# srihari-humbarwadi/retinanet-tensorflow2.x

Measured on AMD Instinct MI355X. Metric: images/sec train, ResNet50-640 RetinaNet data-parallel step (encode + fwd + loss + bwd + clip + all-reduce + SGD/EMA); inference images/s under `infer`, higher is better.
Workload: dtype bf16; 1 GPU; ResNet50-640x640 bf16 training, 32 images/GPU (BASELINE configs[2] shard: global batch 32), resnet_initial frozen, single GPU; global_batch=32, parallelism=dp1, rccl_ranks=1, comm=torch, syncbn_messages=0

## Files before the change

### include/rnet_hip.h

```cpp
#ifndef RNET_HIP_H_
#define RNET_HIP_H_

#include <stddef.h>
#include <stdint.h>

#ifdef __cplusplus
extern "C" {
#endif
#if defined(__GNUC__)
#pragma GCC visibility push(default)
#endif

typedef enum {
  RN_OK = 0,
  RN_EINVAL = -1,
  RN_ENOMEM = -2,
  RN_EHIP = -3,
  RN_ECOMM = -4,
  RN_EUNSUPPORTED = -5
} rn_status;

enum { RN_DT_F32 = 0, RN_DT_BF16 = 1 };
enum { RN_ACT_NONE = 0, RN_ACT_RELU = 1, RN_ACT_RELU6 = 2, RN_ACT_SWISH = 3 };

// ... 16 lines not shown
size_t rn_loss_workspace_bytes(int B, int64_t A, int K);
int rn_retinanet_loss_fwd_bwd(const float* const* class_logits, const float* const* box_preds,
                              float* const* d_class_logits, float* const* d_box_preds,
                              const int64_t* level_offsets, int num_levels, int B, int K,
                              const float* class_targets, const float* box_targets, const float* normalizer,
                              float alpha, float gamma, float label_smoothing, float delta,
                              float box_loss_weight, float class_loss_weight, float grad_scale, float* losses,
                              void* workspace, size_t workspace_bytes, void* stream);
int rn_retinanet_loss_fwd_bwd_bf16(const float* const* class_logits, const float* const* box_preds,
                                   void* const* d_class_bf16, void* const* d_box_bf16, int class_pix_stride,
                                   int box_pix_stride, int anchors_per_location, const int64_t* level_offsets,
                                   int num_levels, int B, int K, const float* class_targets,
                                   const float* box_targets, const float* normalizer, float alpha, float gamma,
                                   float label_smoothing, float delta, float box_loss_weight,
                                   float class_loss_weight, float grad_scale, float* losses, void* workspace,
                                   size_t workspace_bytes, void* stream);

int rn_decode_boxes(const float* const* box_preds, const int64_t* level_offsets, int num_levels, int B,
                    const float* anchors, const float* box_variance, float input_h, float input_w,
                    float* boxes, void* stream);

int rn_sigmoid_scores(const float* const* class_logits, const int64_t* level_offsets, int num_levels, int B,
                      int K, float* scores, void* stream);

size_t rn_topk_workspace_bytes(int B, int64_t A, int K);
int rn_topk_per_class(const float* scores, int B, int64_t A, int K, int top_k, float* topk_scores,
                      int32_t* topk_indices, void* workspace, size_t workspace_bytes, void* stream);

size_t rn_detect_workspace_bytes(int B, int64_t A, int K, int max_det);
int rn_detect_per_class(const float* const* class_logits, const int64_t* level_offsets, int num_levels, int B,
                        int K, const float* boxes, int pre_nms_top_k, float iou_threshold,
                        float score_threshold, float soft_nms_sigma, int max_det, float* det_boxes,
                        float* det_scores, int32_t* det_classes, int32_t* valid, void* workspace,
                        size_t workspace_bytes, void* stream);

size_t rn_nms_workspace_bytes(int B, int n, int K, int max_det);
int rn_nms_per_class(const float* cand_scores, const float* cand_boxes, int B, int n, int K,
                     float iou_threshold, float score_threshold, float soft_nms_sigma, int max_det,
                     float* det_boxes, float* det_scores, int32_t* det_classes,
                     int32_t* det_index ,
                     int32_t* valid, void* workspace, size_t workspace_bytes, void* stream);

int rn_rowmax_argmax(const float* scores, int64_t rows, int K, float* max_out, int32_t* argmax_out, void* stream);

typedef struct {
  int32_t conv_tile;
  int32_t conv_no_halo;
  int32_t conv_big_min_tiles;
  int32_t max_workgroups;
  int32_t reserved_cus;
  int32_t wgrad_kernel;
  int32_t wgrad_target_blocks;
  int32_t ablate;
  int32_t splitk_target_blocks;
} rn_launch_opts;

typedef struct rn_handle rn_handle;
int rn_create(int device_id, rn_handle** out);
int rn_destroy(rn_handle* h);
int rn_handle_device(const rn_handle* h);
int rn_handle_num_cus(const rn_handle* h);
int rn_handle_set_launch_opts(rn_handle* h, const rn_launch_opts* opts);
int rn_handle_get_launch_opts(const rn_handle* h, rn_launch_opts* opts);
int rn_handle_comm_init(rn_handle* h, int slot, const void* unique_id , int rank, int world);
void* rn_handle_comm(const rn_handle* h, int slot);
int rn_handle_comm_destroy(rn_handle* h, int slot);

#define RN_CONV_MAX_SEGMENTS 10

typedef struct {
  const void* x;
  const void* w;
  void* y;
  const float* scale;
  const float* shift;
  const void* residual;
  int32_t N, H, W, Cin, pix_stride, Ho, Wo, Cout;
  float* bn_partial;
  const float* bias;
  int32_t w_terms;
  int32_t w_pair;
  const void* bn_bwd_y;
  const float* bn_bwd_fwd;
} rn_conv_segment;

typedef struct {
  int32_t R, S, stride_h, stride_w, pad_top, pad_left;
  int32_t act;
  int32_t out_dtype;
  int32_t num_segments;
  rn_conv_segment seg[RN_CONV_MAX_SEGMENTS];
  rn_launch_opts opts;
  void* splitk_ws;
  int64_t splitk_ws_bytes;
} rn_conv_problem;

int rn_conv2d_nhwc_fwd(const rn_conv_problem* problem , void* stream);
size_t rn_conv_splitk_workspace_bytes(const rn_conv_problem* problem );
size_t rn_conv_splitk_workspace_max_bytes(void);

int rn_conv_cout_pad(int Cout);
int rn_conv_tile_rows(const rn_conv_problem* problem);
int rn_conv_bn_row_blocks(const rn_conv_problem* problem, int segment);
int rn_conv_kernel_id(const rn_conv_problem* problem);
int rn_conv_cin_pad(int Cin);
int rn_pack_conv_weight(const float* w_hwio, int R, int S, int Cin, int Cout, int Cin_pad, void* w_packed,
                        void* stream);
int rn_pack_conv_weight_split(const float* w, int layout_ohwi, int R, int S, int Cin, int Cout, int Cin_pad, int terms,
                              void* w_packed, void* stream);
int rn_conv_pair_rows(int Cout);
int rn_pack_conv_weight_pair(const float* w, int layout_ohwi, int R, int S, int Cin, int Cout, int Cin_pad,
                             void* w_packed, void* stream);
int rn_pack_conv_weight_ohwi(const float* w_ohwi, int R, int S, int Cin, int Cout, int Cin_pad, void* w_packed,
                             void* stream);
int rn_pack_stem_weight(const float* w_hwio, int Cout, void* w_packed, void* stream);
int rn_stem_padded_width(int W);
int rn_pack_stem_input(const float* images, int N, int H, int W, void* packed, void* stream);
int rn_pack_stem_weight_rs(const float* w_hwio, int R, int S, int Cout, void* w_packed, void* stream);
int rn_pack_image_nhwc4(const float* images, int N, int H, int W, int pad_top, int pad_left, int Hp, int Wp,
                        void* packed, void* stream);

typedef struct {
  const void* x;
  const void* dy;
  int32_t N, H, W, Cin, Ho, Wo, Cout;
  int32_t dy_pix_stride;
  int32_t x_pix_stride;
} rn_wgrad_segment;

typedef struct {
  int32_t R, S, stride_h, stride_w, pad_top, pad_left;
  int32_t num_segments;
  rn_wgrad_segment seg[RN_CONV_MAX_SEGMENTS];
  rn_launch_opts opts;
} rn_wgrad_problem;

size_t rn_wgrad_workspace_bytes(const rn_wgrad_problem* problem );
int rn_wgrad_kernel_id(const rn_wgrad_problem* problem );
int rn_conv2d_nhwc_wgrad(const rn_wgrad_problem* problem , float* dw, float beta, void* workspace,
                         size_t workspace_bytes, void* stream);
size_t rn_wgrad_group_workspace_bytes(const rn_wgrad_problem* const* problems , int n);
int rn_wgrad_group_fused(const rn_wgrad_problem* const* problems , int n);
int rn_conv2d_nhwc_wgrad_group(const rn_wgrad_problem* const* problems , int n, float* const* dws ,
                               float beta, void* workspace, size_t workspace_bytes, void* stream);

int rn_pack_conv_weight_dgrad(const float* w_ohwi, int R, int S, int Cin, int Cout, int Cout_pad, void* w_packed,
                              void* stream);
#define RN_DGRAD_PACK_MAX 64
typedef struct {
  const float* w_ohwi;
  void* w_packed;
  int32_t R, S, Cin, Cout, Cout_pad;
  int32_t pad_;
} rn_dgrad_pack;
int rn_pack_conv_weight_dgrad_batch(const rn_dgrad_pack* items , int n, void* stream);
int rn_cast_pad_f32_to_bf16(const float* x, void* y, int64_t P, int C, int Cpad, void* stream);
int rn_reduce_rows_f32(const float* src, int rows, int64_t row_stride, int n, float add, float* dst, void* stream);
int rn_upsample_zero2x(const void* x, void* y, int N, int H, int W, int C, int Ho, int Wo, void* stream);
int rn_scatter_add2x(const void* x, void* y, int N, int H, int W, int C, int Ho, int Wo, int accumulate, void* stream);
int rn_depth_to_space2x(const void* x, void* y, int N, int H, int W, int C, int accumulate, void* stream);
int rn_cast_f32_to_bf16(const float* x, void* y, int64_t n, void* stream);
int rn_act_bwd(const void* dz, const void* z, void* dy, int64_t n, int act, void* stream);

typedef struct {
  const void* y;
  void* z;
  const void* residual;
  const void* dz;
  void* dy;
  void* dres;
  float* sums;
  float* fwd;
  float* bsums;
  const float* gamma;
  const float* beta;
  float* moving_mean;
  float* moving_var;
  float* dgamma;
  float* dbeta;
  int64_t P;
  int32_t C;
  int32_t dres_accumulate;
  const float* sample_scale;
  int64_t rows_per_sample;
  int32_t ext_chunks;
  int32_t ext_chunks_bwd;
  void* act_mask;
  float* dy_colsum_partial;
} rn_bn_segment;

typedef struct {
  int32_t num_segments;
  int32_t act;
  int32_t bessel;
  float eps;
  float momentum;
  float count_scale;
  rn_bn_segment seg[RN_CONV_MAX_SEGMENTS];
} rn_bn_problem;

size_t rn_bn_workspace_bytes(const rn_bn_problem* problem );
int rn_bn_workspace_init(const rn_bn_problem* problem, void* workspace, size_t workspace_bytes, void* stream);
size_t rn_bn_partial_offset_bytes(const rn_bn_problem* problem, int segment);
size_t rn_bn_bwd_partial_offset_bytes(const rn_bn_problem* problem, int segment);
int rn_bn_stats(const rn_bn_problem* problem, void* workspace, size_t workspace_bytes, void* stream);
int rn_bn_stats_finalize(const rn_bn_problem* problem, void* workspace, size_t workspace_bytes, void* stream);
int rn_bn_finalize(const rn_bn_problem* problem, void* stream);
int rn_bn_apply(const rn_bn_problem* problem, void* stream);
int rn_bn_bwd_reduce(const rn_bn_problem* problem, void* workspace, size_t workspace_bytes, void* stream);
int rn_bn_bwd_apply(const rn_bn_problem* problem, void* stream);
int rn_bn_bwd_colsum_chunks(const rn_bn_problem* problem, int segment);

int rn_maxpool2d_nhwc_bwd(const void* x, const void* dy, void* dx, int N, int H, int W, int C, int k, int stride,
                          int pad_top, int pad_left, int Ho, int Wo, int accumulate, void* stream);
int rn_fpn_topdown_bwd_level(const void* dout, const void* din_finer, const void* out, void* din, int N, int H,
                             int W, int C, int act, void* stream);
size_t rn_balance_features_bwd_scratch_bytes(int num_levels, int mid, int N, int H0, int W0, int C);
int rn_balance_features_bwd(void* const* dout, void* const* in, void* const* din, const void* avg,
                            void* davg_scratch, size_t scratch_bytes, int num_levels, int mid, int N, int H0, int W0,
                            int C, void* stream);

int rn_optim_chunk(void);
size_t rn_optim_workspace_bytes(int num_blocks, int num_segments);
int rn_optim_clip(float* grads, const float* params, const void* segs_dev, int num_segments,
                  const int32_t* block_seg_dev, int num_blocks, float wd_coeff, float wd_alpha, float grad_unscale,
                  float clipnorm, float* metrics, void* workspace, size_t workspace_bytes, void* stream);
int rn_optim_clip_prepare(float* grads, const float* params, const void* segs_dev, const int32_t* block_seg_dev,
                          int num_blocks, int block_begin, int block_count, float wd_coeff, float grad_unscale,
                          float* local_copy ,
                          void* workspace, size_t workspace_bytes, void* stream);
int rn_optim_clip_factors(const void* segs_dev, int num_segments, int num_blocks, float clipnorm, float wd_alpha,
                          float* metrics, float* flags, void* workspace, size_t workspace_bytes, void* stream);
int rn_optim_clip_apply(float* grads, float* correction, const void* segs_dev, const int32_t* block_seg_dev,
                        int num_blocks, void* workspace, size_t workspace_bytes, void* stream);
int rn_optim_sgd_step(float* params, const float* grads, float* momentum_buf, float* ema, void* params_bf16,
                      const void* segs_dev, const int32_t* block_seg_dev, int num_blocks, float lr, float momentum,
                      float ema_decay, int nesterov, const float* skip_flag, void* stream);

int rn_comm_available(void);
int rn_comm_unique_id_bytes(void);
int rn_comm_unique_id(void* out );
int rn_comm_init(const void* unique_id , int rank, int world, void** comm_out);
int rn_comm_destroy(void* comm);
int rn_allreduce_bucket(void* comm, void* ptr , int64_t count, int dtype, void* stream);
int rn_allreduce_small(void* comm, float* ptr , int count, void* stream);

long long rn_probe_mfma_flops(int iters);
int rn_probe_spin(int microseconds, void* stream);
int rn_probe_mfma(const float* table, float* out, int iters, unsigned long long* clocks, void* stream);

int rn_maxpool2d_nhwc(const void* x, void* y, int N, int H, int W, int C, int k, int stride, int pad_top,
                      int pad_left, int Ho, int Wo, void* stream);

int rn_stem_conv_bn_relu_pool(const void* x, const void* w_packed, const float* scale, const float* shift, void* y,
                              int N, int Hp, int Wp, int Hs, int Ws, int R, int Cout, int act, int pool_k,
                              int pool_stride, int pool_pad_top, int pool_pad_left, int Po, int Qo, void* stream);

typedef struct {
  const void* x;
  void* y;
  const void* w_packed;
  const float* affine;
  int32_t N, H, W, Cx;
  rn_launch_opts opts;
} rn_bottleneck64_problem;
int rn_bottleneck64_supported(int N, int H, int W, int Cx);
size_t rn_bottleneck64_packed_bytes(int Cx);
int rn_bottleneck64_pack(const float* wa_hwio, const float* wb_hwio, const float* wo_hwio, const float* wsc_hwio, int Cx,
                         void* packed, void* stream);
int rn_bottleneck64_fwd(const rn_bottleneck64_problem* problem, void* stream);

int rn_fpn_topdown(void* const* p_in , void* const* p_out, int num_levels,
                   int N, int H0, int W0, int C, int act, void* stream);

int rn_balance_features(void* const* p_in, void* const* p_out, int num_levels, int mid, int N, int H0, int W0,
                        int C, void* scratch, void* stream);

typedef struct {
  const void* x;
  const void* w;
  void* y;
  const float* scale;
  const float* shift;
  const void* residual;
  int32_t N, H, W, C, Ho, Wo;
} rn_dw_segment;

typedef struct {
  int32_t k, stride, pad_top, pad_left, act, num_segments;
  rn_dw_segment seg[RN_CONV_MAX_SEGMENTS];
} rn_dw_problem;

int rn_depthwise_conv2d_nhwc_fwd(const rn_dw_problem* problem , void* stream);
int rn_pack_depthwise_weight(const float* w_kkc1, int k, int C, void* w_packed, void* stream);
int rn_pack_depthwise_weight_flip(const float* w_kkc, int k, int C, void* w_packed, void* stream);
// ... 50 lines not shown
```

### retinanet-tensorflow2.x_amd/csrc/rn_conv.hip

```cpp
#include <map>
#include <mutex>
#include <tuple>

#include <algorithm>
#include "rn_conv_dev.h"

template <int BM, int BN, int BK, bool OUT_F32, int ABL = 0, int WM = 2, int WN = 2, int STAGES = 2, bool SPLIT = false>
__global__ void __launch_bounds__(64 * WM * WN, 2) conv_fwd_kernel(const ConvArgs args) {
  constexpr int NWAVES = WM * WN;
  constexpr int NTHREADS = 64 * NWAVES;
  constexpr int SLOTS = BK / 8;
  constexpr int RPI = 64 / SLOTS;
  constexpr int A_INSTR = BM / RPI / NWAVES;
  constexpr int B_INSTR = BN / RPI / NWAVES;
  constexpr int WTM = BM / WM, WTN = BN / WN;
  constexpr int TM = WTM / 32, TN = WTN / 32;
  constexpr int KSUB = BK / 16;
  constexpr int A_BYTES = BM * BK * 2, B_BYTES = BN * BK * 2;
  constexpr int STAGE_BYTES = A_BYTES + B_BYTES;
  static_assert(A_INSTR >= 1 && B_INSTR >= 1, "tile too small for the wave count");

  extern __shared__ __attribute__((aligned(16))) char smem[];

  int tile, part = 0;
// ... 741 lines not shown
  const int kid = conv_pick(p);
  return kid == 3 ? 512 : (kid ? 256 : 128);
}

extern "C" int rn_conv2d_nhwc_fwd(const rn_conv_problem* p, void* stream) {
  RN_CHECK_ARG(p != nullptr, "rn_conv2d_nhwc_fwd: null problem");
  RN_CHECK_ARG(p->num_segments >= 1 && p->num_segments <= RN_CONV_MAX_SEGMENTS,
               "rn_conv2d_nhwc_fwd: num_segments=%d", p->num_segments);
  RN_CHECK_ARG(p->R >= 1 && p->S >= 1 && p->R * p->S <= 32, "rn_conv2d_nhwc_fwd: R*S=%d > 32", p->R * p->S);
  RN_CHECK_ARG(p->stride_h >= 1 && p->stride_w >= 1, "rn_conv2d_nhwc_fwd: bad stride");
  RN_CHECK_ARG(p->out_dtype == RN_DT_BF16 || p->out_dtype == RN_DT_F32, "rn_conv2d_nhwc_fwd: bad out_dtype");
  if (const int orc = rn_validate_launch_opts(p->opts, "rn_conv2d_nhwc_fwd")) return orc;
  ConvArgs a;
  a.R = p->R; a.S = p->S; a.sh = p->stride_h; a.sw = p->stride_w; a.pt = p->pad_top; a.pl = p->pad_left;
  a.act = p->act; a.nseg = p->num_segments; a.pad_ = 0;
  const int cout_pad0 = rn_conv_cout_pad(seg_cols(p->seg[0]));
  int BN = cout_pad0 <= 64 ? 64 : 128;
  const int BK = conv128_bk(p);
  const int kid = conv_pick(p);
  const bool big = kid == 1 || kid == 2;
  const bool halo512 = kid == 3;
  const int BM = big ? 256 : (halo512 ? 512 : 128);
  if (!big && !halo512) {
    int bk_;
    conv128_shape(p, &BN, &bk_);
  }
  const int BNT = big ? 256 : BN;
  const int bal_rows = kid == 1 ? conv_big_balanced_rows(p) : 0;
  int tiles = 0;
  int order[RN_CONV_MAX_SEGMENTS];
  for (int i = 0; i < p->num_segments; ++i) order[i] = i;
  bool deal = false;
  if (kid == 1 && p->num_segments > 1) {
    long long dmin = 1ll << 60, dmax = 0;
    bool one_col = true;
    for (int i = 0; i < p->num_segments; ++i) {
      const long long depth = (long long)p->R * p->S * rn_conv_cin_pad(p->seg[i].Cin) * (p->seg[i].w_terms > 1 ? p->seg[i].w_terms : 1);
      dmin = depth < dmin ? depth : dmin;
      dmax = depth > dmax ? depth : dmax;
      one_col = one_col && rn_conv_cout_pad(seg_cols(p->seg[i])) <= 256;
    }
    deal = one_col && dmax >= 2 * dmin;
    if (deal)
      std::stable_sort(order, order + p->num_segments, [&](int x, int y) {
        return rn_conv_cin_pad(p->seg[x].Cin) * (p->seg[x].w_terms > 1 ? p->seg[x].w_terms : 1) >
               rn_conv_cin_pad(p->seg[y].Cin) * (p->seg[y].w_terms > 1 ? p->seg[y].w_terms : 1);
      });
  }
  for (int ii = 0; ii < p->num_segments; ++ii) {
    const int i = order[ii];
    const rn_conv_segment& s = p->seg[i];
    RN_CHECK_ARG(s.x && s.w && s.y, "rn_conv2d_nhwc_fwd: segment %d has a null tensor", i);
    RN_CHECK_ARG(s.N > 0 && s.H > 0 && s.W > 0 && s.Ho > 0 && s.Wo > 0 && s.Cout > 0 && s.Cin > 0,
                 "rn_conv2d_nhwc_fwd: segment %d bad shape", i);
    RN_CHECK_ARG(s.Cin % 8 == 0 && rn_conv_cin_pad(s.Cin) % BK == 0,
                 "rn_conv2d_nhwc_fwd: segment %d Cin=%d must be a multiple of 8 (K step %d)", i, s.Cin, BK);
    RN_CHECK_ARG(s.pix_stride % 4 == 0 && s.pix_stride > 0,
                 "rn_conv2d_nhwc_fwd: segment %d pix_stride=%d must be a positive multiple of 4", i, s.pix_stride);
    RN_CHECK_ARG(s.Cout % 4 == 0, "rn_conv2d_nhwc_fwd: segment %d Cout=%d not a multiple of 4", i, s.Cout);
    const int cp = rn_conv_cout_pad(seg_cols(s));
    RN_CHECK_ARG((cp <= 64) == (cout_pad0 <= 64), "rn_conv2d_nhwc_fwd: segments mix Cout tile widths");
    RN_CHECK_ARG(!s.w_pair || ((big || halo512) && p->out_dtype == RN_DT_F32 && s.w_terms <= 1 && !s.scale && !s.shift &&
                               !s.residual && !s.bn_partial),
                 "rn_conv2d_nhwc_fwd: segment %d: w_pair needs an f32 launch without scale / shift / residual that the 256- / "
                 "512-row kernels take (rn_conv_kernel_id() != 0)", i);
    RN_CHECK_ARG(((uintptr_t)s.x | (uintptr_t)s.w | (uintptr_t)s.y | (uintptr_t)s.residual) % 16 == 0,
                 "rn_conv2d_nhwc_fwd: segment %d tensors must be 16-byte aligned", i);
    const long long M = (long long)s.N * s.Ho * s.Wo;
    RN_CHECK_ARG(M < (1ll << 31) && (long long)s.N * s.H * s.W * s.pix_stride * 2 < (1ll << 31),
                 "rn_conv2d_nhwc_fwd: segment %d input exceeds the 2 GiB buffer-addressing limit", i);
    ConvSegDev& d = a.seg[ii];
    d.x = (const uint16_t*)s.x; d.w = (const uint16_t*)s.w; d.y = s.y;
    d.scale = s.scale; d.shift = s.shift; d.residual = (const uint16_t*)s.residual;
    d.bn_partial = s.bn_partial;
    d.bn_y = (const uint16_t*)s.bn_bwd_y;
    d.bn_fwd = s.bn_bwd_fwd;
    if (s.bn_bwd_y) {
      RN_CHECK_ARG(s.bn_partial && s.bn_bwd_fwd && p->out_dtype == RN_DT_BF16 && !s.scale && !s.shift && !s.bias &&
                       !s.residual && p->act == RN_ACT_NONE && s.Cout % 8 == 0 && (uintptr_t)s.bn_bwd_y % 16 == 0,
                   "rn_conv2d_nhwc_fwd: segment %d: bn_bwd_y needs bn_partial + bn_bwd_fwd on a plain bf16 launch", i);
    }
    RN_CHECK_ARG((s.bn_bwd_y != nullptr) == (p->seg[0].bn_bwd_y != nullptr),
                 "rn_conv2d_nhwc_fwd: bn_bwd_y must be set on all segments or none");
    d.bias = s.bias;
    d.N = s.N; d.H = s.H; d.W = s.W; d.Cin = s.Cin; d.pix_stride = s.pix_stride;
    d.Ho = s.Ho; d.Wo = s.Wo; d.Cout = seg_cols(s);
    d.pair_cout = s.w_pair ? s.Cout : 0;
    d.rows = kid == 1 ? bal_rows : 0;
    d.M = (int)M;
    d.tile_begin = tiles;
    d.n_tiles = (int)rn_cdiv(cp, BNT);
    const int terms = s.w_terms > 1 ? s.w_terms : 1;
    RN_CHECK_ARG(terms <= 3, "rn_conv2d_nhwc_fwd: segment %d w_terms=%d (1..3)", i, s.w_terms);
    d.cwrap = rn_conv_cin_pad(s.Cin);
    d.CinP = terms * d.cwrap;
    d.halo_pitch = s.W + 1;
    if (rn_conv_halo_patch_pixels(s.N, s.H, s.W, rn_conv_halo_pitch(s.W), halo512 ? 512 : 256) <= rn_conv_halo_capacity(halo512 ? 512 : 256))
      d.halo_pitch = rn_conv_halo_pitch(s.W);
    tiles += (int)rn_cdiv(M, d.rows ? d.rows : BM) * d.n_tiles;
  }
  a.total_tiles = tiles;
  a.split_f = a.vtotal = tiles; a.split_s = 1; a.pad2_ = 0; a.ws = nullptr;
  RN_CHECK_ARG(p->splitk_ws == nullptr || ((uintptr_t)p->splitk_ws % 16 == 0 && p->splitk_ws_bytes >= 0),
               "rn_conv2d_nhwc_fwd: splitk_ws must be 16-byte aligned");
  hipStream_t st = (hipStream_t)stream;
  const bool f32 = p->out_dtype == RN_DT_F32;
  if (p->opts.ablate && BM == 128 && BN == 128 && BK == 64 && !f32) {
    switch (p->opts.ablate) {
      case 1: return launch_ablate<1>(a, st);
      case 2: return launch_ablate<2>(a, st);
      case 3: return launch_ablate<3>(a, st);
      case 4: return launch_ablate<4>(a, st);
      case 5: return launch_ablate<5>(a, st);
      case 6: return launch_ablate<6>(a, st);
      case 7: return launch_ablate<7>(a, st);
      case 8: return launch_ablate<8>(a, st);
      case 16: return launch_ablate<16>(a, st);
      case 32: return launch_ablate<32>(a, st);
      case 48: return launch_ablate<48>(a, st);
      default: break;
    }
  }
  if (halo512) return rn_launch_conv_halo(a, f32, p->opts, st, 4);
  if (kid == 2) {
    rn_splitk_plan(a, conv_splitk_min_chunks(p), p->splitk_ws, p->splitk_ws_bytes, p->opts);
    return rn_launch_conv_halo(a, f32, p->opts, st);
  }
  if (big) {
    a.pad_ = 1;
    for (int i = 0; i < a.nseg; ++i)
      if (a.seg[i].M >= (1 << 22)) a.pad_ = 0;
    if (deal) a.pad_ |= 2;
    return rn_launch_conv_big(a, f32, p->opts, st);
  }
  a.pad_ = 1;
  for (int i = 0; i < a.nseg; ++i)
    if (a.seg[i].M >= (1 << 22)) a.pad_ = 0;
  const int S128 = conv128_split_parts(p, tiles, BN, BK);
  if (S128 >= 2) {
    a.split_s = S128; a.vtotal = tiles * S128; a.ws = (float*)p->splitk_ws;
    return launch_conv128<true>(a, BN, BK, f32, st);
  }
  return launch_conv128<false>(a, BN, BK, f32, st);
}

__global__ void pack_weight_kernel(const float* __restrict__ w, int R, int S, int Cin, int Cout, int Cin_pad,
                                   int Cout_pad, uint16_t* __restrict__ out) {
  const long long total = (long long)Cout_pad * R * S * Cin_pad;
  for (long long i = blockIdx.x * (long long)blockDim.x + threadIdx.x; i < total;
       i += (long long)gridDim.x * blockDim.x) {
    const int c = (int)(i % Cin_pad);
    long long t = i / Cin_pad;
    const int s = (int)(t % S);
    t /= S;
    const int r = (int)(t % R);
    const int o = (int)(t / R);
    float v = 0.0f;
    if (o < Cout && c < Cin) v = w[(((long long)r * S + s) * Cin + c) * Cout + o];
    out[i] = rn_f32_to_bf16(v);
  }
}

extern "C" int rn_pack_conv_weight(const float* w_hwio, int R, int S, int Cin, int Cout, int Cin_pad,
                                   void* w_packed, void* stream) {
  RN_CHECK_ARG(w_hwio && w_packed && R > 0 && S > 0 && Cin > 0 && Cout > 0 && Cin_pad >= Cin,
               "rn_pack_conv_weight: bad argument");
  const int Cout_pad = rn_conv_cout_pad(Cout);
  const long long total = (long long)Cout_pad * R * S * Cin_pad;
  int blocks = (int)(rn_cdiv(total, 256) < 4096 ? rn_cdiv(total, 256) : 4096);
  hipLaunchKernelGGL(pack_weight_kernel, dim3(blocks), dim3(256), 0, (hipStream_t)stream, w_hwio, R, S, Cin,
                     Cout, Cin_pad, Cout_pad, (uint16_t*)w_packed);
  RN_CHECK_LAUNCH();
  return RN_OK;
}

__global__ void pack_weight_ohwi_kernel(const float* __restrict__ w, int RS, int Cin, int Cout, int Cin_pad,
                                        int Cout_pad, uint16_t* __restrict__ out) {
  const long long total = (long long)Cout_pad * RS * Cin_pad;
  for (long long i = blockIdx.x * (long long)blockDim.x + threadIdx.x; i < total;
       i += (long long)gridDim.x * blockDim.x) {
    const int c = (int)(i % Cin_pad);
    const long long t = i / Cin_pad;
    float v = 0.0f;
    if (t < (long long)Cout * RS && c < Cin) v = w[t * Cin + c];
    out[i] = rn_f32_to_bf16(v);
  }
}

extern "C" int rn_pack_conv_weight_ohwi(const float* w_ohwi, int R, int S, int Cin, int Cout, int Cin_pad,
                                        void* w_packed, void* stream) {
  RN_CHECK_ARG(w_ohwi && w_packed && R > 0 && S > 0 && Cin > 0 && Cout > 0 && Cin_pad >= Cin,
               "rn_pack_conv_weight_ohwi: bad argument");
  const int Cout_pad = rn_conv_cout_pad(Cout);
  const long long total = (long long)Cout_pad * R * S * Cin_pad;
  int blocks = (int)(rn_cdiv(total, 256) < 4096 ? rn_cdiv(total, 256) : 4096);
  hipLaunchKernelGGL(pack_weight_ohwi_kernel, dim3(blocks), dim3(256), 0, (hipStream_t)stream, w_ohwi, R * S, Cin,
                     Cout, Cin_pad, Cout_pad, (uint16_t*)w_packed);
  RN_CHECK_LAUNCH();
  return RN_OK;
}

__global__ void pack_weight_split_kernel(const float* __restrict__ w, int ohwi, int RS, int Cin, int Cout, int Cin_pad,
                                         int Cout_pad, int terms, uint16_t* __restrict__ out) {
  const long long total = (long long)Cout_pad * RS * Cin_pad;
  for (long long i = blockIdx.x * (long long)blockDim.x + threadIdx.x; i < total;
       i += (long long)gridDim.x * blockDim.x) {
    const int c = (int)(i % Cin_pad);
    const long long t = i / Cin_pad;
    const int tap = (int)(t % RS), o = (int)(t / RS);
    float v = 0.0f;
    if (o < Cout && c < Cin) v = ohwi ? w[t * Cin + c] : w[((long long)tap * Cin + c) * Cout + o];
    uint16_t* dst = out + (t * terms) * Cin_pad + c;
    for (int k = 0; k < terms; ++k) {
      const uint16_t b = rn_f32_to_bf16(v);
      dst[(long long)k * Cin_pad] = b;
// ... 112 lines not shown
```

### retinanet-tensorflow2.x_amd/csrc/rn_conv_big.hip

```cpp
#include "rn_conv_big_epi.h"

namespace {

constexpr int BM = 256, BN = 256, BK = 32, NW = 8, STAGES = 4;
constexpr int A_BYTES = BM * BK * 2, STAGE_BYTES = (BM + BN) * BK * 2;
constexpr int RING_BYTES = STAGES * STAGE_BYTES, PATCH_BYTES = 4096;
constexpr int LDS_BYTES = RING_BYTES + NW * PATCH_BYTES;

template <bool OUT_F32, bool HAS_RES, bool BN_BWD = false>
__global__ void __launch_bounds__(512) conv_big_kernel(const ConvArgs args) {
  extern __shared__ __attribute__((aligned(16))) char smem[];
  const int total = args.total_tiles;
  const int G = gridDim.x;
  const int tid = threadIdx.x;
  const int lane = tid & 63;
  const int wave = __builtin_amdgcn_readfirstlane(tid >> 6);
  const int wave_m = wave >> 2, wave_n = wave & 3;
  const int R = args.R, S = args.S, RS = R * S;

  int i_v = blockIdx.x;
  int i_tap = 0, i_c0 = 0;
  int i_r = 0, i_s = 0;
  int g_iss = 0;
  int i_W = 0, i_PS = 0, i_Cin = 0, i_cw = 0;
  __amdgpu_buffer_rsrc_t rs_x, rs_w;
  unsigned a_off[2], a_mask[2], b_off[2];
  const int d_row = lane >> 2, d_pos = lane & 3;

#define BIG_SETUP_ISSUE()                                                                             \
  do {                                                                                                \
    const int tile__ = (args.pad_ & 2) ? i_v : tile_of(i_v, total);      \
    int si__ = 0;                                                                                     \
    _Pragma("unroll 1") for (int i = 1; i < args.nseg; ++i)                                           \
      if (tile__ >= args.seg[i].tile_begin) si__ = i;                                                 \
    const ConvSegDev& sg__ = args.seg[si__];                                                          \
    const int lt__ = tile__ - sg__.tile_begin;                                                        \
    const int mt__ = rn_fdiv(lt__, sg__.n_tiles, rn_rcp((float)sg__.n_tiles));   \
    const int rows_t__ = sg__.rows ? sg__.rows : BM;      \
    const int m0__ = mt__ * rows_t__, n0__ = (lt__ - mt__ * sg__.n_tiles) * BN;                       \
    const int mend__ = m0__ + rows_t__ < sg__.M ? m0__ + rows_t__ : sg__.M;                           \
    i_W = sg__.W; i_PS = sg__.pix_stride; i_Cin = sg__.CinP; i_cw = sg__.cwrap;                       \
    const int H__ = sg__.H, Ktot__ = RS * i_Cin;                                                      \
    const int rows__ = sg__.Cout <= 64 ? 64 : ((sg__.Cout + 127) / 128) * 128;  \
    rs_x = __builtin_amdgcn_make_buffer_rsrc((void*)sg__.x, 0,                                        \
                                             (int)((long long)sg__.N * H__ * i_W * i_PS * 2), 0x00020000); \
    rs_w = __builtin_amdgcn_make_buffer_rsrc((void*)sg__.w, 0, (int)((long long)rows__ * Ktot__ * 2), \
                                             0x00020000);                                             \
    const float rWo__ = rn_rcp((float)sg__.Wo), rHo__ = rn_rcp((float)sg__.Ho);                 \
    _Pragma("unroll") for (int j = 0; j < 2; ++j) {                                                   \
      const int row = (j * NW + wave) * 16 + d_row;                                                   \
      const int chunk = d_pos ^ lds_swz<BK>(row);                                                     \
      const int m = m0__ + row;                                                                       \
      const int mm = m < mend__ ? m : 0;                                                              \
      int ox, oy, n;                                                                                  \
      if (args.pad_ & 1) {    \
        const int t2 = rn_fdiv(mm, sg__.Wo, rWo__);                                                   \
        ox = mm - t2 * sg__.Wo;                                                                       \
        n = rn_fdiv(t2, sg__.Ho, rHo__);                                                              \
        oy = t2 - n * sg__.Ho;                                                                        \
      } else {                                                                                        \
        ox = mm % sg__.Wo;                                                                            \
        const int t2 = mm / sg__.Wo;                                                                  \
        oy = t2 % sg__.Ho;                                                                            \
        n = t2 / sg__.Ho;                                                                             \
      }                                                                                               \
      const int iy0 = oy * args.sh - args.pt, ix0 = ox * args.sw - args.pl;                           \
      a_off[j] = (unsigned)(((((long long)n * H__ + iy0) * i_W + ix0) * i_PS + chunk * 8) * 2);       \
      unsigned mask = 0;                                                                              \
      if (m < mend__) {                                                                               \
        for (int r = 0; r < R; ++r)                                                                   \
          for (int s = 0; s < S; ++s) {                                                               \
            const bool ok = (unsigned)(iy0 + r) < (unsigned)H__ && (unsigned)(ix0 + s) < (unsigned)i_W; \
            mask |= (ok ? 1u : 0u) << (r * S + s);                                                    \
          }                                                                                           \
      }                                                                                               \
      a_mask[j] = mask;                                                                               \
      const int nrow = n0__ + row;                                                                    \
      b_off[j] = nrow < rows__ ? (unsigned)(((long long)nrow * Ktot__ + chunk * 8) * 2) : RN_OOB;     \
    }                                                                                                 \
  } while (0)

#define BIG_ISSUE_STEP()                                                                              \
  do {                                                                                                \
    const int cw__ = i_c0 < i_cw ? i_c0 : (i_c0 < 2 * i_cw ? i_c0 - i_cw : i_c0 - 2 * i_cw);          \
    const unsigned tap_off__ = (unsigned)((((long long)i_r * i_W + i_s) * i_PS + cw__) * 2);          \
    const unsigned koff__ = (unsigned)(((long long)i_tap * i_Cin + i_c0) * 2);                        \
    char* st__ = smem + (g_iss & 3) * STAGE_BYTES;                                                    \
    _Pragma("unroll") for (int j = 0; j < 2; ++j) {                                                   \
      const unsigned v__ = ((a_mask[j] >> i_tap) & 1u) ? a_off[j] + tap_off__ : RN_OOB;               \
      dma16(rs_x, st__ + (j * NW + wave) * 1024, v__);                                                \
    }                                                                                                 \
    _Pragma("unroll") for (int j = 0; j < 2; ++j)                                                     \
// ... 10 lines not shown
      if (__builtin_expect(i_tap == RS, 0)) {                                                         \
        i_tap = i_r = i_s = 0;                                                                        \
        i_v += G;                                                                                     \
        if (i_v < total) BIG_SETUP_ISSUE();                                                           \
      }                                                                                               \
    }                                                                                                 \
  } while (0)

  int off_p0, off_w0;
  {
    const int fr = lane & 31, fh = lane >> 5;
    const int sw = (fr >> 2) & 3;
    off_p0 = (wave_m * 128 + fr) * 64 + ((0 + fh) ^ sw) * 16;
    off_w0 = A_BYTES + (wave_n * 64 + fr) * 64 + ((0 + fh) ^ sw) * 16;
  }

  f32x16_t acc[4][2];
#pragma unroll
  for (int i = 0; i < 4; ++i)
#pragma unroll
    for (int j = 0; j < 2; ++j)
#pragma unroll
      for (int r = 0; r < 16; ++r) acc[i][j][r] = 0.0f;

  bf16x8_t px0[4], wt0[2], px1[4], wt1[2];
#define BIG_READ(stage_)                                                                              \
  do {                                                                                                \
    const char* b__ = smem + (stage_) * STAGE_BYTES;                                                  \
    _Pragma("unroll") for (int j = 0; j < 2; ++j) wt0[j] = *(const bf16x8_t*)(b__ + off_w0 + j * 2048); \
    _Pragma("unroll") for (int i = 0; i < 4; ++i) px0[i] = *(const bf16x8_t*)(b__ + off_p0 + i * 2048); \
    _Pragma("unroll") for (int j = 0; j < 2; ++j) wt1[j] = *(const bf16x8_t*)(b__ + (off_w0 ^ 32) + j * 2048); \
    _Pragma("unroll") for (int i = 0; i < 4; ++i) px1[i] = *(const bf16x8_t*)(b__ + (off_p0 ^ 32) + i * 2048); \
  } while (0)
#define BIG_LOADSEG(stage_)                                                                           \
  do {                                                                                                \
    BIG_READ(stage_);                                                                                 \
    if (i_v < total) {                                                                                \
      BIG_ISSUE_STEP();                                                                               \
      asm volatile("s_waitcnt vmcnt(8)" ::: "memory");                                                \
    } else {                                                                                          \
      asm volatile("s_waitcnt vmcnt(0)" ::: "memory");                                                \
    }                                                                                                 \
    asm volatile("s_waitcnt lgkmcnt(0)" ::: "memory");                                                \
  } while (0)
#define BIG_COMPUTESEG()                                                                              \
  do {                                                                                                \
    __builtin_amdgcn_sched_barrier(0);                                                                \
    _Pragma("unroll") for (int i = 0; i < 4; ++i)                                                     \
      _Pragma("unroll") for (int j = 0; j < 2; ++j)                                                   \
        acc[i][j] = RN_MFMA_32x32x16(wt0[j], px0[i], acc[i][j], 0, 0, 0);      \
    _Pragma("unroll") for (int i = 0; i < 4; ++i)                                                     \
      _Pragma("unroll") for (int j = 0; j < 2; ++j)                                                   \
        acc[i][j] = RN_MFMA_32x32x16(wt1[j], px1[i], acc[i][j], 0, 0, 0);      \
    __builtin_amdgcn_sched_barrier(0);                                                                \
  } while (0)
#define BIG_BARRIER()                       \
  do {                                      \
    __builtin_amdgcn_s_barrier();           \
    asm volatile("" ::: "memory");          \
  } while (0)

  int c_v = blockIdx.x;
  int c_k = 0;
  int c_ksteps, c_m0, c_n0, c_si, c_mend, c_chunk0;
#define BIG_SETUP_COMPUTE()                                                                           \
  do {                                                                                                \
    const int tile__ = (args.pad_ & 2) ? c_v : tile_of(c_v, total);                                   \
    c_si = 0;                                                                                         \
    _Pragma("unroll 1") for (int i = 1; i < args.nseg; ++i)                                           \
      if (tile__ >= args.seg[i].tile_begin) c_si = i;                                                 \
    const ConvSegDev& sg__ = args.seg[c_si];                                                          \
    const int lt__ = tile__ - sg__.tile_begin;                                                        \
    const int mt__ = rn_fdiv(lt__, sg__.n_tiles, rn_rcp((float)sg__.n_tiles));   \
    const int rows_t__ = sg__.rows ? sg__.rows : BM;                                                  \
    c_m0 = mt__ * rows_t__;                                                                           \
    c_mend = c_m0 + rows_t__ < sg__.M ? c_m0 + rows_t__ : sg__.M;                                     \
    c_chunk0 = mt__ * 2;                                                                              \
    c_n0 = (lt__ - mt__ * sg__.n_tiles) * BN;                                                         \
    c_ksteps = RS * (sg__.CinP / BK);                                                                 \
    c_k = 0;                                                                                          \
  } while (0)

  auto epilogue = [&]() __attribute__((always_inline)) {
    big_epilogue<OUT_F32, HAS_RES, BN_BWD>(acc, args, c_si, c_m0, c_n0, wave, smem + RING_BYTES + wave * PATCH_BYTES,
                                           BigEpiSrc(), c_mend, c_chunk0);
  };

  BIG_SETUP_ISSUE();
  BIG_SETUP_COMPUTE();
  big_acc_init<OUT_F32, HAS_RES>(acc, args, c_si, c_n0, wave);
#pragma unroll 1
  for (int t = 0; t < 3 && i_v < total; ++t) BIG_ISSUE_STEP();
  if (g_iss >= 3) asm volatile("s_waitcnt vmcnt(4)" ::: "memory");
  else asm volatile("s_waitcnt vmcnt(0)" ::: "memory");
  BIG_BARRIER();
  BIG_LOADSEG(0);
  if (wave_m == 1) BIG_BARRIER();

#define BIG_TILE_END()                                       \
  if (__builtin_expect(c_k == c_ksteps, 0)) {               \
    epilogue();                                             \
    if (c_v + G >= total) break;                            \
    c_v += G;                                               \
    BIG_SETUP_COMPUTE();                                    \
    big_acc_init<OUT_F32, HAS_RES>(acc, args, c_si, c_n0, wave); \
  }
  int g = 0;
#pragma unroll 1
  while (true) {
    BIG_COMPUTESEG();
    ++c_k;
    if (wave_m == 0) BIG_BARRIER();
    BIG_TILE_END();
    if (wave_m == 1) BIG_BARRIER();
    ++g;
    BIG_LOADSEG(g & 3);
    BIG_BARRIER();
  }
#undef BIG_TILE_END
#undef BIG_SETUP_COMPUTE
#undef BIG_BARRIER
#undef BIG_COMPUTESEG
#undef BIG_LOADSEG
#undef BIG_READ
#undef BIG_ISSUE_STEP
#undef BIG_SETUP_ISSUE
}

}

int rn_launch_conv_big(const ConvArgs& a, bool out_f32, const rn_launch_opts& opts, hipStream_t st) {
  static unsigned long long attr_set = 0;
  if (RN_ATTRS_NEEDED(attr_set)) {
    RN_CHECK_HIP(hipFuncSetAttribute((const void*)conv_big_kernel<false, false>,
                                     hipFuncAttributeMaxDynamicSharedMemorySize, LDS_BYTES));
    RN_CHECK_HIP(hipFuncSetAttribute((const void*)conv_big_kernel<false, true>,
                                     hipFuncAttributeMaxDynamicSharedMemorySize, LDS_BYTES));
    RN_CHECK_HIP(hipFuncSetAttribute((const void*)conv_big_kernel<true, false>,
                                     hipFuncAttributeMaxDynamicSharedMemorySize, LDS_BYTES));
    RN_CHECK_HIP(hipFuncSetAttribute((const void*)conv_big_kernel<true, true>,
                                     hipFuncAttributeMaxDynamicSharedMemorySize, LDS_BYTES));
    RN_CHECK_HIP(hipFuncSetAttribute((const void*)conv_big_kernel<false, false, true>,
                                     hipFuncAttributeMaxDynamicSharedMemorySize, LDS_BYTES));
    RN_ATTRS_DONE(attr_set);
  }
  const int grid = rn_persistent_grid(a.total_tiles, rn_num_cus(), opts);
  bool has_res = false;
  for (int i = 0; i < a.nseg; ++i) has_res = has_res || a.seg[i].residual != nullptr;
  const dim3 g3(grid), b3(512);
  if (a.seg[0].bn_y) {
    hipLaunchKernelGGL((conv_big_kernel<false, false, true>), g3, b3, LDS_BYTES, st, a);
  } else if (out_f32) {
    if (has_res) hipLaunchKernelGGL((conv_big_kernel<true, true>), g3, b3, LDS_BYTES, st, a);
    else hipLaunchKernelGGL((conv_big_kernel<true, false>), g3, b3, LDS_BYTES, st, a);
  } else {
    if (has_res) hipLaunchKernelGGL((conv_big_kernel<false, true>), g3, b3, LDS_BYTES, st, a);
    else hipLaunchKernelGGL((conv_big_kernel<false, false>), g3, b3, LDS_BYTES, st, a);
  }
  RN_CHECK_LAUNCH();
  return RN_OK;
}
```

### retinanet-tensorflow2.x_amd/csrc/rn_conv_big_epi.h

```cpp
#ifndef RN_CONV_BIG_EPI_H_
#define RN_CONV_BIG_EPI_H_
#include <type_traits>

#include "rn_conv_dev.h"

#ifdef HALO_PROF
__device__ unsigned long long g_halo_clk[48];
#define EPI_STAMP(k_) if (blockIdx.x == 0 && threadIdx.x == 0) g_halo_clk[k_] = clock64();
#else
#define EPI_STAMP(k_)
#endif

#ifdef HALO_ABLATE
#define EPI_ABLATE HALO_ABLATE
#else
#define EPI_ABLATE 0
#endif

typedef rn_h16 bf16x2_t __attribute__((ext_vector_type(2)));
typedef float f32x2_t __attribute__((ext_vector_type(2)));

__device__ __forceinline__ uint32_t pack2(float lo, float hi) {
  f32x2_t v = {lo, hi};
  bf16x2_t b = __builtin_convertvector(v, bf16x2_t);
// ... 28 lines not shown
    typedef const float __attribute__((address_space(4))) cfloat;
    const cfloat* b = (const cfloat*)(unsigned long long)sg.bias;
    const int cw0 = (c_n0 + (wave % (8 / WM)) * 64) >> 1;
    const int C = sg.pair_cout;
    const int lane = (int)__builtin_amdgcn_mbcnt_hi(~0u, __builtin_amdgcn_mbcnt_lo(~0u, 0u));
    const bool hi = lane >= 32;
#pragma unroll
    for (int g = 0; g < 4; ++g)
#pragma unroll
      for (int q = 0; q < 4; ++q) {
        const int ca = cw0 + g * 8 + q, cb = ca + 4;
        const float lo_v = b[ca < C ? ca : 0], hi_v = b[cb < C ? cb : 0];
        const float v = hi ? hi_v : lo_v;
#pragma unroll
        for (int i = 0; i < 4; ++i) { acc[i][0][g * 4 + q] = v; acc[i][1][g * 4 + q] = 0.0f; }
      }
    return;
  }
  if (with_bias && big_bias_in_acc<OUT_F32, HAS_RES>(args, sg)) {
    typedef const float __attribute__((address_space(4))) cfloat;
    const cfloat* b = (const cfloat*)(unsigned long long)sg.bias;
    const int nw0 = c_n0 + (wave % (8 / WM)) * 64;
    const int Cout = sg.Cout;
    const int lane = (int)__builtin_amdgcn_mbcnt_hi(~0u, __builtin_amdgcn_mbcnt_lo(~0u, 0u));
    const bool hi = lane >= 32;
#pragma unroll
    for (int j = 0; j < 2; ++j)
#pragma unroll
      for (int g = 0; g < 4; ++g) {
        int c0 = nw0 + j * 32 + g * 8;
        c0 = c0 + 8 <= Cout ? c0 : Cout - 8;
        c0 = c0 < 0 ? 0 : c0;
#pragma unroll
        for (int q = 0; q < 4; ++q) {
          const float lo_v = b[c0 + q], hi_v = b[c0 + 4 + q];
          const float v = hi ? hi_v : lo_v;
#pragma unroll
          for (int i = 0; i < 4; ++i) acc[i][j][g * 4 + q] = v;
        }
      }
  } else {
#pragma unroll
    for (int i = 0; i < 4; ++i)
#pragma unroll
      for (int j = 0; j < 2; ++j)
#pragma unroll
        for (int r = 0; r < 16; ++r) acc[i][j][r] = 0.0f;
  }
}

struct BigEpiSrc {
  const char* slots;
  int nparts, voff;
};
template <int NJ>
__device__ __forceinline__ void big_epi_rebuild(f32x16_t* t, const BigEpiSrc& src, int i, int j0) {
  typedef unsigned u32x4_t_ __attribute__((ext_vector_type(4)));
  const __amdgpu_buffer_rsrc_t rs = __builtin_amdgcn_make_buffer_rsrc(
      (void*)src.slots, 0, src.nparts * RN_SPLITK_SLOT_BYTES, 0x00020000);
  u32x4_t_ v[4][NJ][4];
#pragma unroll
  for (int p = 0; p < 4; ++p)
#pragma unroll
    for (int j = 0; j < NJ; ++j)
#pragma unroll
      for (int q = 0; q < 4; ++q)
        v[p][j][q] = __builtin_amdgcn_raw_buffer_load_b128(rs, src.voff + p * RN_SPLITK_SLOT_BYTES,
                                                           ((i * 2 + j0 + j) * 4 + q) * 1024, 16);
#pragma unroll
  for (int j = 0; j < NJ; ++j)
#pragma unroll
    for (int q = 0; q < 4; ++q) {
      float a0 = __uint_as_float(v[0][j][q].x), a1 = __uint_as_float(v[0][j][q].y);
      float a2 = __uint_as_float(v[0][j][q].z), a3 = __uint_as_float(v[0][j][q].w);
#pragma unroll
      for (int p = 1; p < 4; ++p) {
        a0 += __uint_as_float(v[p][j][q].x); a1 += __uint_as_float(v[p][j][q].y);
        a2 += __uint_as_float(v[p][j][q].z); a3 += __uint_as_float(v[p][j][q].w);
      }
      t[j][q * 4] = a0; t[j][q * 4 + 1] = a1; t[j][q * 4 + 2] = a2; t[j][q * 4 + 3] = a3;
    }
}

template <bool OUT_F32, bool HAS_RES, bool BN_BWD = false, bool FROM_WS = false, int WM = 2>
__device__ __forceinline__ void big_epilogue(f32x16_t (&acc)[4][2], const ConvArgs& args, int c_si, int c_m0,
                                             int c_n0, int wave, char* patch, const BigEpiSrc src = BigEpiSrc(),
                                             int m_end = -1, int chunk0 = -1) {
  static_assert(!(BN_BWD && (OUT_F32 || HAS_RES)), "BN_BWD: plain bf16 launches only");
  constexpr bool LOADS = HAS_RES || BN_BWD;
  const int wave_m = wave / (8 / WM), wave_n = wave % (8 / WM);
  const ConvSegDev& sg = args.seg[c_si];
  const int Cout = sg.Cout, M = m_end >= 0 ? m_end : sg.M;
  const int nw0 = c_n0 + wave_n * 64;
  const int mw0 = c_m0 + wave_m * 128;
  const int elane = (int)__builtin_amdgcn_mbcnt_hi(~0u, __builtin_amdgcn_mbcnt_lo(~0u, 0u));
  const int fr = elane & 31, fh = elane >> 5;
  const int rrow = elane >> 3, ru = elane & 7;
  if (!OUT_F32) {
    const int nr = nw0 + ru * 8;
    const bool nok = nr < Cout;
    float sc[8], sf[8];
#pragma unroll
    for (int q = 0; q < 8; ++q) { sc[q] = 1.0f; sf[q] = 0.0f; }
    if (nok && sg.scale) {
      const float4 a = *(const float4*)(sg.scale + nr), b = *(const float4*)(sg.scale + nr + 4);
      sc[0] = a.x; sc[1] = a.y; sc[2] = a.z; sc[3] = a.w; sc[4] = b.x; sc[5] = b.y; sc[6] = b.z; sc[7] = b.w;
    }
    if (nok && sg.shift) {
      const float4 a = *(const float4*)(sg.shift + nr), b = *(const float4*)(sg.shift + nr + 4);
      sf[0] = a.x; sf[1] = a.y; sf[2] = a.z; sf[3] = a.w; sf[4] = b.x; sf[5] = b.y; sf[6] = b.z; sf[7] = b.w;
    }
    float mu[BN_BWD ? 8 : 1], is[BN_BWD ? 8 : 1];
    if (BN_BWD) {
#pragma unroll
      for (int q = 0; q < 8; ++q) { mu[q] = 0.0f; is[q] = 0.0f; }
    }
    if (BN_BWD && nok) {
      const float* f0 = sg.bn_fwd + nr;
      const float* f1 = sg.bn_fwd + Cout + nr;
      {
        const float4 a = *(const float4*)f0, b = *(const float4*)(f0 + 4), c = *(const float4*)f1, d = *(const float4*)(f1 + 4);
        mu[0] = a.x; mu[1] = a.y; mu[2] = a.z; mu[3] = a.w; mu[4] = b.x; mu[5] = b.y; mu[6] = b.z; mu[7] = b.w;
        is[0] = c.x; is[1] = c.y; is[2] = c.z; is[3] = c.w; is[4] = d.x; is[5] = d.y; is[6] = d.z; is[7] = d.w;
      }
      const float* f2 = sg.bn_fwd + 2 * Cout + nr;
      const float* f3 = sg.bn_fwd + 3 * Cout + nr;
      const float4 a = *(const float4*)f2, b = *(const float4*)(f2 + 4), c = *(const float4*)f3, d = *(const float4*)(f3 + 4);
      sc[0] = a.x; sc[1] = a.y; sc[2] = a.z; sc[3] = a.w; sc[4] = b.x; sc[5] = b.y; sc[6] = b.z; sc[7] = b.w;
      sf[0] = c.x; sf[1] = c.y; sf[2] = c.z; sf[3] = c.w; sf[4] = d.x; sf[5] = d.y; sf[6] = d.z; sf[7] = d.w;
    }
#pragma unroll
    for (int q = 0; q < 8; ++q) asm volatile("" : "+v"(sc[q]), "+v"(sf[q]));
    if (BN_BWD) {
#pragma unroll
      for (int q = 0; q < 8; ++q) asm volatile("" : "+v"(mu[q]), "+v"(is[q]));
    }
    EPI_STAMP(12);
    const bool has_res = HAS_RES && sg.residual != nullptr;
    const uint16_t* const side = BN_BWD ? sg.bn_y : sg.residual;
    const bool has_side = BN_BWD ? true : has_res;
    const bool stats = sg.bn_partial != nullptr;
    float st0[8], st1[8];
#pragma unroll
    for (int q = 0; q < 8; ++q) st0[q] = st1[q] = 0.0f;
    char* const ybase = (char*)sg.y + ((long long)(mw0 + rrow) * Cout + nr) * 2;
    const long long row_bytes = (long long)Cout * 2;
    const int act = args.act;
    const bool clamp_lo = act == RN_ACT_RELU || act == RN_ACT_RELU6, clamp_hi = act == RN_ACT_RELU6;
    const bool affine = !BN_BWD && (sg.scale != nullptr || sg.shift != nullptr);
    const bool plain = BN_BWD || (!affine && !has_res && act != RN_ACT_SWISH);
    const bool round2 = affine && has_res;
    uint4 rv[2][LOADS ? 4 : 1];
#define BIG_RES_PREFETCH(buf_, i_)                                                                    \
_Pragma("unroll") for (int pass = 0; pass < (LOADS ? 4 : 0); ++pass) {                              \
  const int m = mw0 + (i_) * 32 + pass * 8 + rrow;                                                  \
  rv[buf_][pass] = make_uint4(0u, 0u, 0u, 0u);                                                      \
  if (has_side && nok && m < M) rv[buf_][pass] = *(const uint4*)(side + (long long)m * Cout + nr);  \
}
    const uint32_t lo2 = clamp_lo ? 0u : 0x80008000u, hi2 = clamp_hi ? RN_SIX_X2 : 0x7fff7fffu;
    auto blocks = [&](auto plain_c, auto stats_c, auto round2_c, auto swish_c) __attribute__((always_inline)) {
      constexpr bool PLAIN = decltype(plain_c)::value;
      constexpr int STATS = decltype(stats_c)::value, ROUND2 = decltype(round2_c)::value, SWISH = decltype(swish_c)::value;
      BIG_RES_PREFETCH(0, 0);
#pragma unroll
      for (int i = 0; i < 4; ++i) {
        EPI_STAMP(13 + 2 * i);
        if (i + 1 < 4) BIG_RES_PREFETCH((i + 1) & 1, i + 1);
        if (FROM_WS) big_epi_rebuild<2>(&acc[i][0], src, i, 0);
#pragma unroll
        for (int j = 0; j < 2; ++j)
#pragma unroll
          for (int g = 0; g < 4; ++g) {
            const int nl = j * 32 + g * 8 + fh * 4;
            uint2 pk;
            pk.x = pack2(acc[i][j][g * 4 + 0], acc[i][j][g * 4 + 1]);
            pk.y = pack2(acc[i][j][g * 4 + 2], acc[i][j][g * 4 + 3]);
            *(uint2*)(patch + fr * 128 + (((nl >> 3) ^ (fr & 7)) << 4) + ((((nl >> 2) ^ (fr >> 3)) & 1) << 3)) = pk;
          }
        EPI_STAMP(14 + 2 * i);
        uint4 vb[4];
#pragma unroll
        for (int pass = 0; pass < 4; ++pass) {
          const int row = pass * 8 + rrow;
          const uint4 t = *(const uint4*)(patch + row * 128 + ((ru ^ (row & 7)) << 4));
          vb[pass] = (pass & 1) ? make_uint4(t.z, t.w, t.x, t.y) : t;
        }
#pragma unroll
        for (int pass = 0; pass < 4; ++pass) {
          const int row = pass * 8 + rrow;
          const uint4 v = vb[pass];
          const int m = mw0 + i * 32 + row;
          if (m < M && nok) {
            uint4 ov;
            if (PLAIN) {
              ov.x = pk_min_i16(pk_max_i16(v.x, lo2), hi2); ov.y = pk_min_i16(pk_max_i16(v.y, lo2), hi2);
              ov.z = pk_min_i16(pk_max_i16(v.z, lo2), hi2); ov.w = pk_min_i16(pk_max_i16(v.w, lo2), hi2);
            } else {
              const uint4 r4 = HAS_RES ? rv[i & 1][LOADS ? pass : 0] : make_uint4(0u, 0u, 0u, 0u);
              float f[8] = {bf_lo(v.x), bf_hi(v.x), bf_lo(v.y), bf_hi(v.y), bf_lo(v.z), bf_hi(v.z), bf_lo(v.w), bf_hi(v.w)};
              const float rr[8] = {bf_lo(r4.x), bf_hi(r4.x), bf_lo(r4.y), bf_hi(r4.y),
                                   bf_lo(r4.z), bf_hi(r4.z), bf_lo(r4.w), bf_hi(r4.w)};
#pragma unroll
              for (int q = 0; q < 8; ++q) f[q] = f[q] * sc[q] + sf[q];
              if (ROUND2 == 1 || (ROUND2 == 2 && round2)) {
#pragma unroll
                for (int q = 0; q < 8; q += 2) {
                  const uint32_t pq = pack2(f[q], f[q + 1]);
                  f[q] = bf_lo(pq); f[q + 1] = bf_hi(pq);
                }
              }
#pragma unroll
              for (int q = 0; q < 8; ++q) f[q] += rr[q];
              if (SWISH == 1 || (SWISH == 2 && act == RN_ACT_SWISH)) {
#pragma unroll
                for (int q = 0; q < 8; ++q) f[q] = rn_swish(rn_rb(f[q]));
              }
              ov.x = pack2(f[0], f[1]); ov.y = pack2(f[2], f[3]); ov.z = pack2(f[4], f[5]); ov.w = pack2(f[6], f[7]);
              ov.x = pk_min_i16(pk_max_i16(ov.x, lo2), hi2); ov.y = pk_min_i16(pk_max_i16(ov.y, lo2), hi2);
              ov.z = pk_min_i16(pk_max_i16(ov.z, lo2), hi2); ov.w = pk_min_i16(pk_max_i16(ov.w, lo2), hi2);
            }
            if (!(EPI_ABLATE & 16) || ov.x == 0x12345678u) *(uint4*)(ybase + (long long)(i * 32 + pass * 8) * row_bytes) = ov;
            if (STATS == 1 || (STATS == 2 && stats)) {
              const float w[8] = {bf_lo(ov.x), bf_hi(ov.x), bf_lo(ov.y), bf_hi(ov.y),
                                  bf_lo(ov.z), bf_hi(ov.z), bf_lo(ov.w), bf_hi(ov.w)};
              if (BN_BWD) {
                const uint4 y4 = rv[i & 1][LOADS ? pass : 0];
                const float yy[8] = {bf_lo(y4.x), bf_hi(y4.x), bf_lo(y4.y), bf_hi(y4.y),
                                     bf_lo(y4.z), bf_hi(y4.z), bf_lo(y4.w), bf_hi(y4.w)};
#pragma unroll
                for (int q = 0; q < 8; ++q) {
                  const float g = (yy[q] * sc[q] + sf[q]) > 0.0f ? w[q] : 0.0f;
                  st0[q] += g;
                  st1[q] += g * ((yy[q] - mu[BN_BWD ? q : 0]) * is[BN_BWD ? q : 0]);
                }
              } else {
#pragma unroll
                for (int q = 0; q < 8; ++q) { st0[q] += w[q]; st1[q] += w[q] * w[q]; }
              }
            }
          }
        }
      }
    };
    typedef std::integral_constant<int, 0> off_t;
    typedef std::integral_constant<int, 1> on_t;
    typedef std::integral_constant<int, 2> runtime_t;
    if constexpr (BN_BWD) {
      blocks(std::true_type{}, on_t{}, off_t{}, off_t{});
    } else if (plain) {
      if (stats) blocks(std::true_type{}, on_t{}, off_t{}, off_t{});
      else blocks(std::true_type{}, off_t{}, off_t{}, off_t{});
    } else if (!stats && act != RN_ACT_SWISH) {
      if (round2) blocks(std::false_type{}, off_t{}, on_t{}, off_t{});
      else blocks(std::false_type{}, off_t{}, off_t{}, off_t{});
    } else {
      blocks(std::false_type{}, runtime_t{}, runtime_t{}, runtime_t{});
    }
    EPI_STAMP(21);
    if (stats) {
#pragma unroll
      for (int q = 0; q < 8; ++q) {
#pragma unroll
        for (int o = 8; o < 64; o <<= 1) {
          st0[q] += __shfl_xor(st0[q], o, 64);
          st1[q] += __shfl_xor(st1[q], o, 64);
        }
      }
      if (rrow == 0 && nok) {
        float* dst = sg.bn_partial + ((long long)(chunk0 >= 0 ? chunk0 : c_m0 / 128) + wave_m) * 2 * Cout + nr;
        *(float4*)(dst) = make_float4(st0[0], st0[1], st0[2], st0[3]);
        *(float4*)(dst + 4) = make_float4(st0[4], st0[5], st0[6], st0[7]);
        *(float4*)(dst + Cout) = make_float4(st1[0], st1[1], st1[2], st1[3]);
        *(float4*)(dst + Cout + 4) = make_float4(st1[4], st1[5], st1[6], st1[7]);
      }
    }
#undef BIG_RES_PREFETCH
  } else {
    const int pairC = sg.pair_cout;
    const int CoutY = pairC ? pairC : Cout;
    auto half = [&](auto j_c) __attribute__((always_inline)) {
      constexpr int j = decltype(j_c)::value;
      const int nr = (pairC ? (nw0 >> 1) : nw0 + j * 32) + ru * 4;
      const bool nok = nr < CoutY;
      float4 sc = make_float4(1.f, 1.f, 1.f, 1.f), sf = make_float4(0.f, 0.f, 0.f, 0.f);
      if (nok && sg.scale) sc = *(const float4*)(sg.scale + nr);
      if (nok && sg.shift) sf = *(const float4*)(sg.shift + nr);
      asm volatile("" : "+v"(sc.x), "+v"(sc.y), "+v"(sc.z), "+v"(sc.w), "+v"(sf.x), "+v"(sf.y), "+v"(sf.z), "+v"(sf.w));
#pragma unroll
      for (int i = 0; i < 4; ++i) {
        if (FROM_WS) big_epi_rebuild<1>(&acc[i][j], src, i, j);
        if (j == 0 && pairC) {
          if (FROM_WS) big_epi_rebuild<1>(&acc[i][1], src, i, 1);
#pragma unroll
          for (int r = 0; r < 16; ++r) acc[i][0][r] += acc[i][1][r];
        }
#pragma unroll
        for (int g = 0; g < 4; ++g) {
          float4 v;
          v.x = acc[i][j][g * 4 + 0]; v.y = acc[i][j][g * 4 + 1]; v.z = acc[i][j][g * 4 + 2]; v.w = acc[i][j][g * 4 + 3];
          *(float4*)(patch + fr * 128 + (((g * 2 + fh) ^ (fr & 7)) << 4)) = v;
        }
#pragma unroll
        for (int pass = 0; pass < 4; ++pass) {
          const int row = pass * 8 + rrow;
          float4 v = *(const float4*)(patch + row * 128 + ((ru ^ (row & 7)) << 4));
          const int m = mw0 + i * 32 + row;
          if (m < M && nok) {
            const long long o = (long long)m * CoutY + nr;
            v.x = v.x * sc.x + sf.x; v.y = v.y * sc.y + sf.y; v.z = v.z * sc.z + sf.z; v.w = v.w * sc.w + sf.w;
            if (sg.residual) {
              const uint2 r2 = *(const uint2*)(sg.residual + o);
              v.x += bf_lo(r2.x); v.y += bf_hi(r2.x); v.z += bf_lo(r2.y); v.w += bf_hi(r2.y);
            }
            {
              float f4[4] = {v.x, v.y, v.z, v.w};
              rn_apply_act_n<4>(f4, args.act);
              v = make_float4(f4[0], f4[1], f4[2], f4[3]);
            }
            *(float4*)((float*)sg.y + o) = v;
          }
        }
      }
    };
    half(std::integral_constant<int, 0>{});
    if (!pairC) half(std::integral_constant<int, 1>{});
  }
}
#endif
```

### retinanet-tensorflow2.x_amd/csrc/rn_core.hip

```cpp
#include "rn_common.h"
#include <string.h>
#include <new>

static thread_local char g_rn_err[512] = "";

void rn_set_error(const char* fmt, ...) {
  va_list ap;
  va_start(ap, fmt);
  vsnprintf(g_rn_err, sizeof(g_rn_err), fmt, ap);
  va_end(ap);
}

extern "C" const char* rn_last_error(void) { return g_rn_err; }

extern "C" int rn_abi_version(void) { return 8; }

extern "C" int rn_storage_dtype(void) {
#ifdef RN_F16
  return 1;
#else
  return 0;
#endif
}

extern "C" int rn_device_ok(void) {
  int n = 0;
  if (hipGetDeviceCount(&n) != hipSuccess || n <= 0) {
    (void)hipGetLastError();
    return 0;
  }
  hipDeviceProp_t p;
  if (hipGetDeviceProperties(&p, 0) != hipSuccess) return 0;
  return strncmp(p.gcnArchName, "gfx950", 6) == 0 ? 1 : 0;
}

struct rn_handle {
  int device;
  int num_cus;
  rn_launch_opts opts;
  void* comm[4];
};

static int rn_check_opts(const rn_launch_opts& o, const char* who) {
  RN_CHECK_ARG(o.conv_tile >= 0 && o.conv_tile <= 3, "%s: conv_tile=%d (0..3)", who, o.conv_tile);
  RN_CHECK_ARG(o.wgrad_kernel >= 0 && o.wgrad_kernel <= 3, "%s: wgrad_kernel=%d (0..3)", who, o.wgrad_kernel);
  RN_CHECK_ARG(o.reserved_cus >= 0 && o.reserved_cus <= 128, "%s: reserved_cus=%d out of range (0..128)", who,
               o.reserved_cus);
  RN_CHECK_ARG(o.max_workgroups >= 0 && o.conv_big_min_tiles >= 0 && o.wgrad_target_blocks >= 0 && o.splitk_target_blocks >= 0,
               "%s: negative max_workgroups / conv_big_min_tiles / wgrad_target_blocks / splitk_target_blocks", who);
  return RN_OK;
}
int rn_validate_launch_opts(const rn_launch_opts& o, const char* who) { return rn_check_opts(o, who); }

extern "C" int rn_create(int device_id, rn_handle** out) {
  RN_CHECK_ARG(out != nullptr, "rn_create: null out");
  *out = nullptr;
  int n = 0;
  RN_CHECK_HIP(hipGetDeviceCount(&n));
  RN_CHECK_ARG(device_id >= 0 && device_id < n, "rn_create: device %d of %d", device_id, n);
  hipDeviceProp_t p;
  RN_CHECK_HIP(hipGetDeviceProperties(&p, device_id));
  RN_CHECK_ARG(strncmp(p.gcnArchName, "gfx950", 6) == 0, "rn_create: device %d is %s, this library is gfx950 only",
               device_id, p.gcnArchName);
  rn_handle* h = new (std::nothrow) rn_handle();
  if (!h) {
    rn_set_error("rn_create: out of host memory");
    return RN_ENOMEM;
  }
  h->device = device_id;
  h->num_cus = p.multiProcessorCount;
  memset(&h->opts, 0, sizeof(h->opts));
  for (auto& c : h->comm) c = nullptr;
  *out = h;
  return RN_OK;
}

extern "C" int rn_destroy(rn_handle* h) {
  if (!h) return RN_OK;
  int rc = RN_OK;
  for (auto& c : h->comm)
    if (c) {
      const int r = rn_comm_destroy(c);
      if (r != RN_OK) rc = r;
      c = nullptr;
    }
  delete h;
  return rc;
}

extern "C" int rn_handle_device(const rn_handle* h) { return h ? h->device : RN_EINVAL; }
extern "C" int rn_handle_num_cus(const rn_handle* h) { return h ? h->num_cus : RN_EINVAL; }

extern "C" int rn_handle_set_launch_opts(rn_handle* h, const rn_launch_opts* opts) {
  RN_CHECK_ARG(h && opts, "rn_handle_set_launch_opts: null argument");
  const int rc = rn_check_opts(*opts, "rn_handle_set_launch_opts");
  if (rc != RN_OK) return rc;
  h->opts = *opts;
  return RN_OK;
// ... 51 lines not shown
```

### retinanet-tensorflow2.x_amd/csrc/rn_optim.hip

```cpp
#include "rn_common.h"

#define OPT_THREADS 256
#define OPT_CHUNK 8192

struct OptSeg { long long offset, size; int wd, block_begin, nblocks, pad_; long long bf16_offset; };

__global__ void __launch_bounds__(OPT_THREADS)
optim_sqnorm_kernel(float* __restrict__ g, const float* __restrict__ w, const OptSeg* __restrict__ segs,
                    const int* __restrict__ block_seg, int block0, float wdc, float unscale,
                    double* __restrict__ partial, double* __restrict__ partial_w, float* __restrict__ local_copy) {
  const int blk = block0 + blockIdx.x;
  const int si = block_seg[blk];
  const OptSeg s = segs[si];
  const long long b0 = (long long)(blk - s.block_begin) * OPT_CHUNK;
  long long b1 = b0 + OPT_CHUNK;
  if (b1 > s.size) b1 = s.size;
  float acc = 0.0f, accw = 0.0f;
  const bool touch = s.wd || unscale != 1.0f;
#define SQNORM_ELEM(gv_, wv_)                 \
  do {                                        \
    float v__ = (gv_) * unscale;              \
    if (s.wd) {                               \
      v__ += wdc * (wv_);                     \
      accw += (wv_) * (wv_);                  \
// ... 210 lines not shown
                                     float wd_alpha, float* metrics, float* flags, void* workspace,
                                     size_t workspace_bytes, void* stream) {
  RN_CHECK_ARG(segs_dev && metrics && num_segments > 0 && num_blocks > 0, "rn_optim_clip_factors: bad argument");
  if (!workspace || workspace_bytes < rn_optim_workspace_bytes(num_blocks, num_segments)) {
    rn_set_error("rn_optim_clip_factors: workspace too small");
    return RN_ENOMEM;
  }
  const OptWs w = opt_ws(workspace, num_blocks);
  hipLaunchKernelGGL(optim_factors_kernel, dim3(1), dim3(256), 0, (hipStream_t)stream, (const OptSeg*)segs_dev,
                     num_segments, w.partial, w.partial_w, clipnorm, wd_alpha, w.factor, metrics, flags);
  RN_CHECK_LAUNCH();
  return RN_OK;
}

extern "C" int rn_optim_clip_apply(float* grads, float* correction, const void* segs_dev,
                                   const int32_t* block_seg_dev, int num_blocks, void* workspace,
                                   size_t workspace_bytes, void* stream) {
  RN_CHECK_ARG(grads && segs_dev && block_seg_dev && num_blocks > 0 && workspace, "rn_optim_clip_apply: bad argument");
  const OptWs w = opt_ws(workspace, num_blocks);
  hipLaunchKernelGGL(optim_scale_kernel, dim3(num_blocks), dim3(OPT_THREADS), 0, (hipStream_t)stream, grads, correction,
                     (const OptSeg*)segs_dev, block_seg_dev, w.factor);
  RN_CHECK_LAUNCH();
  return RN_OK;
}

extern "C" int rn_optim_clip(float* grads, const float* params, const void* segs_dev, int num_segments,
                             const int32_t* block_seg_dev, int num_blocks, float wd_coeff, float wd_alpha,
                             float grad_unscale, float clipnorm, float* metrics , void* workspace,
                             size_t workspace_bytes, void* stream) {
  RN_CHECK_ARG(grads && params && segs_dev && block_seg_dev && metrics && num_segments > 0 && num_blocks > 0,
               "rn_optim_clip: bad argument");
  int rc = rn_optim_clip_prepare(grads, params, segs_dev, block_seg_dev, num_blocks, 0, num_blocks, wd_coeff,
                                 grad_unscale, nullptr, workspace, workspace_bytes, stream);
  if (rc) return rc;
  rc = rn_optim_clip_factors(segs_dev, num_segments, num_blocks, clipnorm, wd_alpha, metrics, nullptr, workspace,
                             workspace_bytes, stream);
  if (rc) return rc;
  return rn_optim_clip_apply(grads, nullptr, segs_dev, block_seg_dev, num_blocks, workspace, workspace_bytes, stream);
}

extern "C" int rn_optim_sgd_step(float* params, const float* grads, float* momentum_buf, float* ema,
                                 void* params_bf16, const void* segs_dev, const int32_t* block_seg_dev,
                                 int num_blocks, float lr, float momentum, float ema_decay, int nesterov,
                                 const float* skip_flag, void* stream) {
  RN_CHECK_ARG(params && grads && momentum_buf && segs_dev && block_seg_dev && num_blocks > 0,
               "rn_optim_sgd_step: bad argument");
  hipLaunchKernelGGL(optim_sgd_kernel, dim3(num_blocks), dim3(OPT_THREADS), 0, (hipStream_t)stream, params, grads,
                     momentum_buf, ema, (uint16_t*)params_bf16, (const OptSeg*)segs_dev, block_seg_dev, lr, momentum,
                     ema_decay, ema ? 1 : 0, nesterov, skip_flag);
  RN_CHECK_LAUNCH();
  return RN_OK;
}

__global__ void __launch_bounds__(256)
pack_dgrad_kernel(const float* __restrict__ w, int R, int S, int Cin, int Cout, int Cin_pad, int Cout_pad,
                  uint16_t* __restrict__ out) {
  const long long total = (long long)Cin_pad * R * S * Cout_pad;
  for (long long i = blockIdx.x * (long long)blockDim.x + threadIdx.x; i < total;
       i += (long long)gridDim.x * blockDim.x) {
    const int co = (int)(i % Cout_pad);
    long long t = i / Cout_pad;
    const int s = (int)(t % S);
    t /= S;
    const int r = (int)(t % R);
    const int ci = (int)(t / R);
    float v = 0.0f;
    if (ci < Cin && co < Cout) v = w[(((long long)co * R + (R - 1 - r)) * S + (S - 1 - s)) * Cin + ci];
    out[i] = rn_f32_to_bf16(v);
  }
}
struct DgradPackArgs {
  int n;
  rn_dgrad_pack item[RN_DGRAD_PACK_MAX];
};
__device__ __forceinline__ float dgrad_s2_weight(const float* __restrict__ w, int Cin, int Cout, int n, int u, int v, int co) {
  if (n >= 4 * Cin || co >= Cout) return 0.0f;
  const int ph = n / Cin, ci = n - ph * Cin, a = ph >> 1, b = ph & 1;
  const int r = a == 0 ? (u == 0 ? 1 : -1) : (u == 0 ? 2 : 0);
  const int s = b == 0 ? (v == 0 ? 1 : -1) : (v == 0 ? 2 : 0);
  if (r < 0 || s < 0) return 0.0f;
  return w[(((long long)co * 3 + r) * 3 + s) * Cin + ci];
}

__global__ void __launch_bounds__(256) pack_dgrad_batch_kernel(const DgradPackArgs a) {
  const rn_dgrad_pack& it = a.item[blockIdx.y];
  if (it.pad_ == 1) {
    const int Cin = it.Cin, Cout = it.Cout, Cout_pad = it.Cout_pad;
    const int rows = 4 * Cin <= 64 ? 64 : ((4 * Cin + 127) / 128) * 128;
    const long long total = (long long)rows * 4 * Cout_pad;
    uint16_t* __restrict__ out = (uint16_t*)it.w_packed;
    for (long long i = blockIdx.x * (long long)blockDim.x + threadIdx.x; i < total;
         i += (long long)gridDim.x * blockDim.x) {
      const int co = (int)(i % Cout_pad);
      const long long t = i / Cout_pad;
      const int v = (int)(t & 1), u = (int)((t >> 1) & 1), n = (int)(t >> 2);
      out[i] = rn_f32_to_bf16(dgrad_s2_weight(it.w_ohwi, Cin, Cout, n, u, v, co));
    }
    return;
  }
  const int R = it.R, S = it.S, Cin = it.Cin, Cout = it.Cout, Cout_pad = it.Cout_pad;
  const int Cin_pad = Cin <= 64 ? 64 : ((Cin + 127) / 128) * 128;
  const long long total = (long long)Cin_pad * R * S * Cout_pad;
  const float* __restrict__ w = it.w_ohwi;
  uint16_t* __restrict__ out = (uint16_t*)it.w_packed;
  for (long long i = blockIdx.x * (long long)blockDim.x + threadIdx.x; i < total;
       i += (long long)gridDim.x * blockDim.x) {
    const int co = (int)(i % Cout_pad);
    long long t = i / Cout_pad;
    const int s = (int)(t % S);
    t /= S;
    const int r = (int)(t % R);
    const int ci = (int)(t / R);
    float v = 0.0f;
    if (ci < Cin && co < Cout) v = w[(((long long)co * R + (R - 1 - r)) * S + (S - 1 - s)) * Cin + ci];
    out[i] = rn_f32_to_bf16(v);
  }
}
extern "C" int rn_pack_conv_weight_dgrad_batch(const rn_dgrad_pack* items, int n, void* stream) {
  RN_CHECK_ARG(items && n >= 0, "rn_pack_conv_weight_dgrad_batch: bad argument");
  for (int base = 0; base < n; base += RN_DGRAD_PACK_MAX) {
    DgradPackArgs a;
    a.n = n - base < RN_DGRAD_PACK_MAX ? n - base : RN_DGRAD_PACK_MAX;
    long long most = 0;
    for (int i = 0; i < a.n; ++i) {
      const rn_dgrad_pack& it = items[base + i];
      RN_CHECK_ARG(it.w_ohwi && it.w_packed && it.R > 0 && it.S > 0 && it.Cin > 0 && it.Cout > 0 &&
                       it.Cout_pad >= it.Cout, "rn_pack_conv_weight_dgrad_batch: bad item %d", base + i);
      RN_CHECK_ARG(it.pad_ == 0 || (it.pad_ == 1 && it.R == 3 && it.S == 3),
                   "rn_pack_conv_weight_dgrad_batch: item %d: the sub-pixel form is for 3x3 kernels", base + i);
      a.item[i] = it;
      const long long total = it.pad_ == 1 ? (long long)rn_conv_cout_pad(4 * it.Cin) * 4 * it.Cout_pad
                                           : (long long)rn_conv_cout_pad(it.Cin) * it.R * it.S * it.Cout_pad;
      if (total > most) most = total;
    }
    const int bx = (int)(rn_cdiv(most, 256) < 256 ? rn_cdiv(most, 256) : 256);
    hipLaunchKernelGGL(pack_dgrad_batch_kernel, dim3(bx, a.n), dim3(256), 0, (hipStream_t)stream, a);
    RN_CHECK_LAUNCH();
  }
  return RN_OK;
}

extern "C" int rn_pack_conv_weight_dgrad(const float* w_ohwi, int R, int S, int Cin, int Cout, int Cout_pad,
                                         void* out, void* stream) {
  RN_CHECK_ARG(w_ohwi && out && R > 0 && S > 0 && Cin > 0 && Cout > 0 && Cout_pad >= Cout,
               "rn_pack_conv_weight_dgrad: bad argument");
  const int Cin_pad = rn_conv_cout_pad(Cin);
  const long long total = (long long)Cin_pad * R * S * Cout_pad;
  int blocks = (int)(rn_cdiv(total, 256) < 4096 ? rn_cdiv(total, 256) : 4096);
  hipLaunchKernelGGL(pack_dgrad_kernel, dim3(blocks), dim3(256), 0, (hipStream_t)stream, w_ohwi, R, S, Cin, Cout,
                     Cin_pad, Cout_pad, (uint16_t*)out);
  RN_CHECK_LAUNCH();
  return RN_OK;
}
```

### retinanet-tensorflow2.x_amd/csrc/rn_train.hip

```cpp
#include "rn_common.h"

#define TR_THREADS 256

struct bf8 { float v[8]; };
__device__ __forceinline__ bf8 unpack8(uint4 u) {
  bf8 r;
  r.v[0] = rn_bf16_to_f32((uint16_t)(u.x & 0xffffu)); r.v[1] = rn_bf16_to_f32((uint16_t)(u.x >> 16));
  r.v[2] = rn_bf16_to_f32((uint16_t)(u.y & 0xffffu)); r.v[3] = rn_bf16_to_f32((uint16_t)(u.y >> 16));
  r.v[4] = rn_bf16_to_f32((uint16_t)(u.z & 0xffffu)); r.v[5] = rn_bf16_to_f32((uint16_t)(u.z >> 16));
  r.v[6] = rn_bf16_to_f32((uint16_t)(u.w & 0xffffu)); r.v[7] = rn_bf16_to_f32((uint16_t)(u.w >> 16));
  return r;
}
__device__ __forceinline__ uint4 pack8(const bf8& r) {
  uint4 u;
  u.x = rn_pack_bf16x2(r.v[0], r.v[1]); u.y = rn_pack_bf16x2(r.v[2], r.v[3]);
  u.z = rn_pack_bf16x2(r.v[4], r.v[5]); u.w = rn_pack_bf16x2(r.v[6], r.v[7]);
  return u;
}
__device__ __forceinline__ float act_mask(float z, int act) {
  if (act == RN_ACT_RELU) return z > 0.0f ? 1.0f : 0.0f;
  if (act == RN_ACT_RELU6) return (z > 0.0f && z < 6.0f) ? 1.0f : 0.0f;
  return 1.0f;
}
__device__ __forceinline__ float act_mask_u(float u, int act) {
  if (act == RN_ACT_RELU) return u > 0.0f ? 1.0f : 0.0f;
  if (act == RN_ACT_RELU6) {
    const float ub = rn_rb(u);
    return (ub > 0.0f && ub < 6.0f) ? 1.0f : 0.0f;
  }
  return 1.0f;
}
__device__ __forceinline__ float act_deriv(float z, float u, int act) {
  if (act == RN_ACT_SWISH) {
    const float sg = 1.0f / (1.0f + __expf(-u));
    return sg + u * sg * (1.0f - sg);
  }
  return act_mask(z, act);
}

enum { G_GENERIC = 0, G_NONE = 1, G_U_RELU = 2, G_U_RELU6 = 3, G_Z_RELU = 4, G_Z_RELU6 = 5, G_SWISH = 6, G_MASK = 7 };
template <int G>
__device__ __forceinline__ float grad_gate(float dz, float z, float u, int act, bool from_u) {
  if (G == G_NONE || G == G_MASK) return dz;
  if (G == G_U_RELU) return u > 0.0f ? dz : 0.0f;
  if (G == G_U_RELU6) {
    const float ub = rn_rb(u);
    return (ub > 0.0f && ub < 6.0f) ? dz : 0.0f;
  }
  if (G == G_Z_RELU) return z > 0.0f ? dz : 0.0f;
  if (G == G_Z_RELU6) return (z > 0.0f && z < 6.0f) ? dz : 0.0f;
  if (G == G_SWISH) {
    const float sg = __builtin_amdgcn_rcpf(1.0f + __expf(-u));
    return dz * (sg + u * sg * (1.0f - sg));
  }
  return act == RN_ACT_NONE ? dz : dz * (from_u ? act_mask_u(u, act) : act_deriv(z, u, act));
}
static int bn_gate_mode(const rn_bn_problem* p) {
  if (p->act == RN_ACT_NONE) return G_NONE;
  if (p->act == RN_ACT_SWISH) return G_SWISH;
  int with_res = 0;
  for (int i = 0; i < p->num_segments; ++i) with_res += p->seg[i].residual ? 1 : 0;
  if (with_res != 0 && with_res != p->num_segments) return G_GENERIC;
  if (with_res == 0) return p->act == RN_ACT_RELU ? G_U_RELU : (p->act == RN_ACT_RELU6 ? G_U_RELU6 : G_GENERIC);
  int with_mask = 0;
  for (int i = 0; i < p->num_segments; ++i) with_mask += p->seg[i].act_mask ? 1 : 0;
  if (with_mask == p->num_segments && (p->act == RN_ACT_RELU || p->act == RN_ACT_RELU6)) return G_MASK;
  return p->act == RN_ACT_RELU ? G_Z_RELU : (p->act == RN_ACT_RELU6 ? G_Z_RELU6 : G_GENERIC);
}
#define BN_DISPATCH_GATE(mode_, CALL_)                  \
  switch (mode_) {                                      \
    case G_NONE: CALL_(G_NONE); break;                  \
    case G_U_RELU: CALL_(G_U_RELU); break;              \
    case G_U_RELU6: CALL_(G_U_RELU6); break;            \
    case G_Z_RELU: CALL_(G_Z_RELU); break;              \
    case G_Z_RELU6: CALL_(G_Z_RELU6); break;            \
    case G_SWISH: CALL_(G_SWISH); break;                \
    case G_MASK: CALL_(G_MASK); break;                  \
    default: CALL_(G_GENERIC); break;                   \
  }

static int tr_blocks(long long items, int cap = 8192) {
  long long b = rn_cdiv(items, TR_THREADS);
  if (b > cap) b = cap;
// ... 67 lines not shown
        const bool from_u = !s.residual && (a.act == RN_ACT_RELU || a.act == RN_ACT_RELU6);
        constexpr bool need_z = G == G_Z_RELU || G == G_Z_RELU6 || G == G_GENERIC;
        bf8 z;
        if (need_z && (G != G_GENERIC || (a.act != RN_ACT_NONE && !from_u))) z = unpack8(s.z[o]);
        unsigned bits = 0xffu;
        if (G == G_MASK) bits = s.mask[o];
        float m = 1.0f;
        if (s.sample_scale) m = s.sample_scale[(int)r / (int)s.rows_per_sample];
#pragma unroll
        for (int q = 0; q < 8; ++q) {
          const float u = y.v[q] * scq[q] + shq[q];
          float g = grad_gate<G < 0 ? 0 : G>(dz.v[q], z.v[q], u, a.act, from_u) * m;
          if (G == G_MASK) g = ((bits >> q) & 1u) ? g : 0.0f;
          s0[q] += g;
          s1[q] += g * ((y.v[q] - mean[q]) * istd[q]);
        }
      }
    }
  }
  __shared__ float red[SGT == 8 ? 2 * 32 * 65 : 2 * (TR_THREADS * 8 + TR_THREADS)];
  const int W = SG * 8 + 1;
  if (rl < RL) {
#pragma unroll
    for (int q = 0; q < 8; ++q) {
      red[rl * W + cg * 8 + q] = s0[q];
      red[RL * W + rl * W + cg * 8 + q] = s1[q];
    }
  }
  __syncthreads();
  for (int t = threadIdx.x; t < 2 * SG * 8; t += TR_THREADS) {
    const int which = t >= SG * 8 ? 1 : 0, c = t - which * SG * 8;
    float v = 0.0f;
    for (int r = 0; r < RL; ++r) v += red[which * RL * W + r * W + c];
    const int ch = slab * SG * 8 + c;
    if (ch < s.C) a.ws[a.ws_off[blockIdx.z] + ((long long)chunk * 2 + which) * s.C + ch] = v;
  }
}

static void bn_slab_plan(int C8, int chunks, int* slab_groups, int* nslab) {
  const int old_n = (C8 + 7) / 8;
  auto score = [&](int n) {
    const int g = (C8 + n - 1) / n;
    return (double)C8 * (TR_THREADS / g) / ((double)n * TR_THREADS);
  };
  *slab_groups = C8 < 8 ? C8 : 8;
  *nslab = old_n;
  if (C8 >= 8 && (double)C8 / (8.0 * old_n) >= 0.95) return;
  double best = 0.0;
  for (int n = 1; n <= old_n; ++n) {
    const int g = (C8 + n - 1) / n;
    if (g > 64 || (g < 8 && n > 1)) continue;
    if (score(n) > best) best = score(n);
  }
  for (int n = 1; n <= old_n; ++n) {
    const int g = (C8 + n - 1) / n;
    if (g > 64 || (g < 8 && n > 1) || score(n) < best - 0.01) continue;
    if ((long long)chunks * n >= 512 || C8 < 8) {
      *slab_groups = g;
      *nslab = n;
      return;
    }
  }
}

__device__ __forceinline__ void bn_finalize_channel(const BnArgs& a, const BnSegDev& s, int c, double sum, double sumsq) {
  const double n = (double)s.P * (double)a.count_scale;
  const double mean = sum / n;
  double var = sumsq / n - mean * mean;
  if (var < 0.0) var = 0.0;
  const float istd = (float)(1.0 / sqrt(var + (double)a.eps));
  const float sc = s.gamma[c] * istd;
  s.fwd[0 * s.C + c] = (float)mean;
  s.fwd[1 * s.C + c] = istd;
  s.fwd[2 * s.C + c] = sc;
  s.fwd[3 * s.C + c] = s.beta[c] - (float)mean * sc;
  if (s.moving_mean) {
    const double vm = a.bessel && n > 1.0 ? var * n / (n - 1.0) : var;
    s.moving_mean[c] = s.moving_mean[c] * a.momentum + (float)mean * (1.0f - a.momentum);
    s.moving_var[c] = s.moving_var[c] * a.momentum + (float)vm * (1.0f - a.momentum);
  }
}

template <int CH>
__global__ void __launch_bounds__(1024) bn_colreduce_final_kernel(const BnArgs a) {
  constexpr int LANES = 1024 / CH, PER = LANES / 16;
  const BnSegDev& s = a.seg[blockIdx.y];
  __shared__ double red[2][LANES][CH + 1];
  __shared__ double red2[2][16][CH + 1];
  const int cl = threadIdx.x & (CH - 1), lane = threadIdx.x / CH;
  const int c = blockIdx.x * CH + cl;
  double t0 = 0.0, t1 = 0.0;
  if (c < s.C) {
    const float* p = a.ws + a.ws_off[blockIdx.y];
#pragma unroll 8
    for (int k = lane; k < s.chunks; k += LANES) {
      t0 += (double)p[((long long)k * 2 + 0) * s.C + c];
      t1 += (double)p[((long long)k * 2 + 1) * s.C + c];
    }
  }
  red[0][lane][cl] = t0;
  red[1][lane][cl] = t1;
  __syncthreads();
  if (threadIdx.x < 2 * 16 * CH) {
    const int which = threadIdx.x / (16 * CH), rem = threadIdx.x - which * (16 * CH);
    const int grp = rem / CH, ch = rem - grp * CH;
    double t = 0.0;
#pragma unroll
    for (int j = 0; j < PER; ++j) t += red[which][grp * PER + j][ch];
    red2[which][grp][ch] = t;
  }
  __syncthreads();
  if (threadIdx.x < 2 * CH) {
    const int which = threadIdx.x / CH, ch = threadIdx.x - which * CH;
    const int cc = blockIdx.x * CH + ch;
    if (cc < s.C) {
      double t = 0.0;
#pragma unroll
      for (int j = 0; j < 16; ++j) t += red2[which][j][ch];
      float* out = a.mode == 0 ? s.sums : s.bsums;
      out[which * s.C + cc] = (float)t;
      if (a.mode == 1) {
        float* gp = which == 0 ? s.dbeta : s.dgamma;
        if (gp) gp[cc] = (float)t;
      }
      red2[which][0][ch] = (double)(float)t;
    }
  }
  if (a.fuse_finalize) {
    __syncthreads();
    if (threadIdx.x < CH && c < s.C) bn_finalize_channel(a, s, c, red2[0][0][cl], red2[1][0][cl]);
  }
}

typedef unsigned bn_u32x2_t __attribute__((ext_vector_type(2)));
__global__ void __launch_bounds__(1024) bn_colreduce_final_split_kernel(const BnArgs a) {
  const BnSegDev& s = a.seg[blockIdx.y];
  const int ks = a.ks[blockIdx.y], part = blockIdx.z;
  if (part >= ks || (int)blockIdx.x * 16 >= s.C) return;
  __shared__ double red[16][2][16];
  __shared__ unsigned s_old;
  const int col = threadIdx.x & 3, lane = threadIdx.x >> 2, wave = threadIdx.x >> 6;
  const int c = blockIdx.x * 16 + col * 4;
  double t[8];
#pragma unroll
  for (int q = 0; q < 8; ++q) t[q] = 0.0;
  if (c < s.C) {
    const float* p = a.ws + a.ws_off[blockIdx.y] + c;
    const int per = (s.chunks + ks - 1) / ks;
    const int k1 = (part + 1) * per < s.chunks ? (part + 1) * per : s.chunks;
#pragma unroll 2
    for (int k = part * per + lane; k < k1; k += 256) {
      const float4 v0 = *(const float4*)(p + ((long long)k * 2 + 0) * s.C);
      const float4 v1 = *(const float4*)(p + ((long long)k * 2 + 1) * s.C);
      t[0] += (double)v0.x; t[1] += (double)v0.y; t[2] += (double)v0.z; t[3] += (double)v0.w;
      t[4] += (double)v1.x; t[5] += (double)v1.y; t[6] += (double)v1.z; t[7] += (double)v1.w;
    }
  }
#pragma unroll
  for (int m = 4; m < 64; m <<= 1)
#pragma unroll
    for (int q = 0; q < 8; ++q) t[q] += __shfl_xor(t[q], m, 64);
  if ((threadIdx.x & 63) < 4) {
#pragma unroll
    for (int q = 0; q < 8; ++q) red[wave][q >> 2][col * 4 + (q & 3)] = t[q];
  }
  __syncthreads();
  const int which = (threadIdx.x >> 4) & 1, ch = threadIdx.x & 15;
  double r = 0.0;
  if (threadIdx.x < 32) {
#pragma unroll
    for (int j = 0; j < 16; ++j) r += red[j][which][ch];
  }
  if (ks > 1) {
    char* const slots = (char*)a.ws + a.slot_off[blockIdx.y] + (size_t)blockIdx.x * ks * 256;
    if (threadIdx.x < 64) {
      if (threadIdx.x < 32) {
        const __amdgpu_buffer_rsrc_t rs = __builtin_amdgcn_make_buffer_rsrc((void*)(slots + part * 256), 0, 256, 0x00020000);
        const unsigned long long bits = __builtin_bit_cast(unsigned long long, r);
        __builtin_amdgcn_raw_buffer_store_b64(bn_u32x2_t{(unsigned)bits, (unsigned)(bits >> 32)}, rs, threadIdx.x * 8, 0, 16);
      }
      asm volatile("s_waitcnt vmcnt(0)" ::: "memory");
      if (threadIdx.x == 0) {
        unsigned* const cnt = (unsigned*)((char*)a.ws + a.cnt_off[blockIdx.y]) + blockIdx.x;
        const unsigned old = __hip_atomic_fetch_add(cnt, 1u, __ATOMIC_RELAXED, __HIP_MEMORY_SCOPE_AGENT);
        if (old == (unsigned)(ks - 1)) __hip_atomic_store(cnt, 0u, __ATOMIC_RELAXED, __HIP_MEMORY_SCOPE_AGENT);
        s_old = old;
      }
    }
    __syncthreads();
    if (s_old != (unsigned)(ks - 1)) return;
    if (threadIdx.x < 32) {
      const __amdgpu_buffer_rsrc_t rs = __builtin_amdgcn_make_buffer_rsrc((void*)slots, 0, ks * 256, 0x00020000);
      bn_u32x2_t pv[BN_KS_MAX];
#pragma unroll
      for (int j = 0; j < BN_KS_MAX; ++j) pv[j] = __builtin_amdgcn_raw_buffer_load_b64(rs, j * 256 + threadIdx.x * 8, 0, 16);
      r = 0.0;
#pragma unroll
      for (int j = 0; j < BN_KS_MAX; ++j)
        r += __builtin_bit_cast(double, ((unsigned long long)pv[j].y << 32) | pv[j].x);
    }
  }
  if (threadIdx.x < 32) {
    const int cc = blockIdx.x * 16 + ch;
    if (cc < s.C) {
      float* out = a.mode == 0 ? s.sums : s.bsums;
      out[which * s.C + cc] = (float)r;
      if (a.mode == 1) {
        float* gp = which == 0 ? s.dbeta : s.dgamma;
        if (gp) gp[cc] = (float)r;
      }
    }
    red[0][which][ch] = (double)(float)r;
  }
  if (a.fuse_finalize) {
    __syncthreads();
    const int cc = blockIdx.x * 16 + threadIdx.x;
    if (threadIdx.x < 16 && cc < s.C) bn_finalize_channel(a, s, cc, red[0][0][threadIdx.x], red[0][1][threadIdx.x]);
  }
}

__global__ void bn_finalize_kernel(const BnArgs a) {
  const BnSegDev& s = a.seg[blockIdx.y];
  const int c = blockIdx.x * blockDim.x + threadIdx.x;
  if (c >= s.C) return;
  bn_finalize_channel(a, s, c, (double)s.sums[c], (double)s.sums[s.C + c]);
}

#define BN_ELEMENTWISE_RANGE() BN_ELEMENTWISE_RANGE_(false)
#define BN_ELEMENTWISE_RANGE_(keep_)                                                                  \
  long long first, last, step;                                                                        \
  if (a.chunk_u > 0) {                                                                                \
    const long long span = 256ll * a.chunk_u;                                                         \
    first = blockIdx.x * span + threadIdx.x;                                                          \
    last = (blockIdx.x + 1) * span < total ? (blockIdx.x + 1) * span : total;                         \
    step = 256;                                                                                       \
    if (first >= last) {                                                                              \
      if (!(keep_) || blockIdx.x * span >= total) return;    \
      first = last;                                                                                   \
    }                                                                                                 \
  } else {                                                                                            \
    const long long nthreads = (long long)gridDim.x * blockDim.x;                                     \
    step = nthreads / C8 * C8;                                                                        \
    first = blockIdx.x * (long long)blockDim.x + threadIdx.x;                                         \
    last = total;                                                                                     \
    if (first >= step) return;                                                                        \
  }

__global__ void __launch_bounds__(TR_THREADS) bn_apply_kernel(const BnArgs a) {
  const BnSegDev& s = a.seg[blockIdx.y];
  const int C8 = s.C >> 3;
  const long long total = s.P * C8;
  BN_ELEMENTWISE_RANGE();
  const int c8 = (int)(first % C8);
  float sc[8], sh[8];
#pragma unroll
  for (int q = 0; q < 8; ++q) {
    sc[q] = s.fwd[2 * s.C + c8 * 8 + q];
    sh[q] = s.fwd[3 * s.C + c8 * 8 + q];
  }
  for (long long i = first; i < last; i += step) {
    const bf8 y = unpack8(s.y[i]);
    bf8 o;
    bf8 res;
    if (s.residual) res = unpack8(s.residual[i]);
    const float m = s.sample_scale ? s.sample_scale[(int)(i / C8) / (int)s.rows_per_sample] : 1.0f;
    const bool swish = a.act == RN_ACT_SWISH;
#pragma unroll
    for (int q = 0; q < 8; ++q) o.v[q] = y.v[q] * sc[q] + sh[q];
    if (s.residual != nullptr || s.sample_scale != nullptr || swish) {
#pragma unroll
      for (int q = 0; q < 8; ++q) o.v[q] = rn_rb(o.v[q]);
    }
    if (s.sample_scale) {
#pragma unroll
      for (int q = 0; q < 8; ++q) o.v[q] = rn_rb(o.v[q] * m);
    }
    if (s.residual) {
#pragma unroll
      for (int q = 0; q < 8; ++q) o.v[q] += res.v[q];
      if (swish) {
#pragma unroll
        for (int q = 0; q < 8; ++q) o.v[q] = rn_rb(o.v[q]);
      }
    }
    rn_apply_act_n<8>(o.v, a.act);
    const uint4 zp = pack8(o);
    s.z[i] = zp;
    if (s.mask) {
      const bf8 zs = unpack8(zp);
      unsigned bits = 0u;
      if (a.act == RN_ACT_RELU) {
#pragma unroll
        for (int q = 0; q < 8; ++q) bits |= (zs.v[q] > 0.0f ? 1u : 0u) << q;
      } else if (a.act == RN_ACT_RELU6) {
#pragma unroll
        for (int q = 0; q < 8; ++q) bits |= ((zs.v[q] > 0.0f && zs.v[q] < 6.0f) ? 1u : 0u) << q;
      } else {
        bits = 0xffu;
      }
      s.mask[i] = (unsigned char)bits;
    }
// ... 89 lines not shown
}

static int bn_fill(const rn_bn_problem* p, BnArgs& a, int need_ws, int mode = 1) {
  if (!p || p->num_segments < 1 || p->num_segments > RN_CONV_MAX_SEGMENTS) return -1;
  a.nseg = p->num_segments; a.act = p->act; a.bessel = p->bessel; a.mode = 0; a.fuse_finalize = 0; a.chunk_u = 0;
  a.eps = p->eps; a.momentum = p->momentum; a.count_scale = p->count_scale > 0 ? p->count_scale : 1.0f;
  long long off = 0;
  for (int i = 0; i < p->num_segments; ++i) {
    const rn_bn_segment& s = p->seg[i];
    if (s.P <= 0 || s.C <= 0 || (s.C % 8)) return -1;
    BnSegDev& d = a.seg[i];
    d.y = (const uint4*)s.y; d.z = (uint4*)s.z; d.residual = (const uint4*)s.residual;
    d.dz = (const uint4*)s.dz; d.dy = (uint4*)s.dy; d.dres = (uint4*)s.dres;
    d.sums = s.sums; d.fwd = s.fwd; d.bsums = s.bsums; d.gamma = s.gamma; d.beta = s.beta;
    d.moving_mean = s.moving_mean; d.moving_var = s.moving_var; d.dgamma = s.dgamma; d.dbeta = s.dbeta;
    d.P = s.P; d.C = s.C; d.dres_accumulate = s.dres_accumulate;
    d.sample_scale = s.sample_scale; d.rows_per_sample = s.rows_per_sample > 0 ? s.rows_per_sample : 1;
    d.mask = (unsigned char*)s.act_mask;
    d.colsum = s.dy_colsum_partial;
    if (s.sample_scale && p->act == RN_ACT_SWISH) return -1;
    d.chunks = bn_chunks_of(s, mode, &d.rows_per_chunk);
    bn_slab_plan(s.C / 8, d.chunks, &d.slab_groups, &d.nslab);
    a.ws_off[i] = off;
    off += (long long)d.chunks * 2 * s.C;
  }
  long long other = 0;
  for (int i = 0; i < p->num_segments; ++i) other += (long long)bn_chunks_of(p->seg[i], 1 - mode, nullptr) * 2 * p->seg[i].C;
  long long tail = ((off > other ? off : other) * 4 + 255) / 256 * 256;
  for (int i = 0; i < p->num_segments; ++i) {
    a.cnt_off[i] = tail;
    tail += rn_cdiv(p->seg[i].C, 16) * 4;
  }
  tail = (tail + 255) / 256 * 256;
  for (int i = 0; i < p->num_segments; ++i) {
    const int ch = a.seg[i].chunks;
    int ks = ch > BN_KS_CHUNKS ? (int)rn_cdiv(ch, 256) : 1;
    if (ks > BN_KS_MAX) ks = BN_KS_MAX;
    a.ks[i] = ks;
    a.slot_off[i] = tail;
    if (ks > 1) tail += rn_cdiv(p->seg[i].C, 16) * ks * 256;
  }
  a.total_bytes = tail;
  (void)need_ws;
  return 0;
}

extern "C" size_t rn_bn_workspace_bytes(const rn_bn_problem* p) {
  size_t need = 0;
  for (int mode = 0; mode < 2; ++mode) {
    BnArgs a;
    if (bn_fill(p, a, 1, mode)) return 0;
    if ((size_t)a.total_bytes > need) need = (size_t)a.total_bytes;
  }
  return need;
}

extern "C" int rn_bn_workspace_init(const rn_bn_problem* p, void* ws, size_t ws_bytes, void* stream) {
  BnArgs a;
  RN_CHECK_ARG(p && bn_fill(p, a, 1, 0) == 0, "rn_bn_workspace_init: bad problem (C %% 8 == 0, 1..10 segments)");
  const size_t need = rn_bn_workspace_bytes(p);
  if (!ws || ws_bytes < need) {
    rn_set_error("rn_bn_workspace_init: workspace too small (%zu < %zu)", ws_bytes, need);
    return RN_ENOMEM;
  }
  const long long begin = a.cnt_off[0];
  long long end = begin;
  for (int i = 0; i < p->num_segments; ++i) end = a.cnt_off[i] + rn_cdiv(p->seg[i].C, 16) * 4;
  RN_CHECK_HIP(hipMemsetAsync((char*)ws + begin, 0, (size_t)(end - begin), (hipStream_t)stream));
  return RN_OK;
}

extern "C" size_t rn_bn_partial_offset_bytes(const rn_bn_problem* p, int segment) {
  BnArgs a;
  if (bn_fill(p, a, 1, 0) || segment < 0 || segment >= a.nseg) return 0;
  return (size_t)a.ws_off[segment] * sizeof(float);
}

extern "C" size_t rn_bn_bwd_partial_offset_bytes(const rn_bn_problem* p, int segment) {
  BnArgs a;
  if (bn_fill(p, a, 1, 1) || segment < 0 || segment >= a.nseg) return 0;
  return (size_t)a.ws_off[segment] * sizeof(float);
}

static int bn_colreduce(const rn_bn_problem* p, int mode, void* ws, size_t ws_bytes, hipStream_t st,
                        const char* fn, int fuse_finalize = 0) {
  BnArgs a;
  RN_CHECK_ARG(bn_fill(p, a, 1, mode) == 0, "%s: bad problem (C %% 8 == 0, 1..10 segments)", fn);
  int n_ext = 0;
  for (int i = 0; i < p->num_segments; ++i)
    n_ext += ((mode == 0 && p->seg[i].ext_chunks > 0) || (mode == 1 && p->seg[i].ext_chunks_bwd > 0)) ? 1 : 0;
  RN_CHECK_ARG(n_ext == 0 || n_ext == p->num_segments, "%s: ext_chunks must be set on all segments or none", fn);
  if (mode == 1 && n_ext) {
    RN_CHECK_ARG(bn_gate_mode(p) == G_U_RELU, "%s: ext_chunks_bwd needs act = relu without residual inputs", fn);
    for (int i = 0; i < p->num_segments; ++i)
      RN_CHECK_ARG(!p->seg[i].sample_scale, "%s: ext_chunks_bwd with sample_scale", fn);
  }
  if (!ws || ws_bytes < rn_bn_workspace_bytes(p)) {
    rn_set_error("%s: workspace too small", fn);
    return RN_ENOMEM;
  }
  a.mode = mode;
  a.fuse_finalize = fuse_finalize;
  if (fuse_finalize)
    for (int i = 0; i < a.nseg; ++i)
      RN_CHECK_ARG(a.seg[i].fwd && a.seg[i].gamma && a.seg[i].beta, "%s: null tensor", fn);
  a.ws = (float*)ws;
  int max_chunks = 0, max_slabs = 0, max_c = 0;
  for (int i = 0; i < a.nseg; ++i) {
    const BnSegDev& s = a.seg[i];
    RN_CHECK_ARG(s.y && (mode == 0 ? s.sums != nullptr : (s.dz && s.bsums && s.fwd)), "%s: null tensor", fn);
    RN_CHECK_ARG(mode == 0 || a.act == RN_ACT_NONE || s.z || s.mask, "%s: z needed for the activation mask", fn);
    if (s.chunks > max_chunks) max_chunks = s.chunks;
    if (s.nslab > max_slabs) max_slabs = s.nslab;
    if (s.C > max_c) max_c = s.C;
  }
  if (n_ext == 0) {
    const dim3 grid(max_chunks, max_slabs, a.nseg), block(TR_THREADS);
    bool all8 = true;
    for (int i = 0; i < a.nseg; ++i) all8 = all8 && a.seg[i].slab_groups == 8;
    if (mode == 0) {
      if (all8) hipLaunchKernelGGL((bn_colreduce_kernel<-1, 8>), grid, block, 0, st, a);
      else hipLaunchKernelGGL((bn_colreduce_kernel<-1, 0>), grid, block, 0, st, a);
    } else {
#define BN_CALL_(G_)                                                                       \
  if (all8) hipLaunchKernelGGL((bn_colreduce_kernel<G_, 8>), grid, block, 0, st, a);       \
  else hipLaunchKernelGGL((bn_colreduce_kernel<G_, 0>), grid, block, 0, st, a)
      BN_DISPATCH_GATE(bn_gate_mode(p), BN_CALL_)
#undef BN_CALL_
    }
    RN_CHECK_LAUNCH();
  }
  int max_ks = 1;
  for (int i = 0; i < a.nseg; ++i) max_ks = a.ks[i] > max_ks ? a.ks[i] : max_ks;
  static const int final_form = getenv("RNET_BN_FINAL") ? atoi(getenv("RNET_BN_FINAL")) : 0;
  if (max_ks > 1 && final_form != 1 && (((uintptr_t)a.ws) & 15) == 0)
    hipLaunchKernelGGL(bn_colreduce_final_split_kernel, dim3((max_c + 15) / 16, a.nseg, max_ks), dim3(1024), 0, st, a);
  else
    hipLaunchKernelGGL(bn_colreduce_final_kernel<16>, dim3((max_c + 15) / 16, a.nseg), dim3(1024), 0, st, a);
  RN_CHECK_LAUNCH();
  return RN_OK;
}

extern "C" int rn_bn_stats(const rn_bn_problem* p, void* ws, size_t ws_bytes, void* stream) {
  return bn_colreduce(p, 0, ws, ws_bytes, (hipStream_t)stream, "rn_bn_stats");
}
extern "C" int rn_bn_stats_finalize(const rn_bn_problem* p, void* ws, size_t ws_bytes, void* stream) {
  return bn_colreduce(p, 0, ws, ws_bytes, (hipStream_t)stream, "rn_bn_stats_finalize", 1);
}
extern "C" int rn_bn_bwd_reduce(const rn_bn_problem* p, void* ws, size_t ws_bytes, void* stream) {
  return bn_colreduce(p, 1, ws, ws_bytes, (hipStream_t)stream, "rn_bn_bwd_reduce");
}

extern "C" int rn_bn_finalize(const rn_bn_problem* p, void* stream) {
  BnArgs a;
  RN_CHECK_ARG(bn_fill(p, a, 0) == 0, "rn_bn_finalize: bad problem");
  int max_c = 0;
  for (int i = 0; i < a.nseg; ++i) {
    RN_CHECK_ARG(a.seg[i].sums && a.seg[i].fwd && a.seg[i].gamma && a.seg[i].beta, "rn_bn_finalize: null tensor");
    if (a.seg[i].C > max_c) max_c = a.seg[i].C;
  }
  hipLaunchKernelGGL(bn_finalize_kernel, dim3((max_c + 255) / 256, a.nseg), dim3(256), 0, (hipStream_t)stream, a);
  RN_CHECK_LAUNCH();
  return RN_OK;
}

#ifndef RN_BN_CHUNK_U
#define RN_BN_CHUNK_U 8
#endif
static int bn_elementwise_grid(BnArgs& a, long long max_units) {
  static_assert(TR_THREADS == 256, "BN_ELEMENTWISE_RANGE assumes 256 threads");
  bool chunk = RN_BN_CHUNK_U > 0;
  for (int i = 0; i < a.nseg; ++i) chunk = chunk && 256 % (a.seg[i].C >> 3) == 0;
  const long long blocks = rn_cdiv(max_units, 256ll * (RN_BN_CHUNK_U > 0 ? RN_BN_CHUNK_U : 1));
  if (chunk && blocks < (1ll << 31)) {
    a.chunk_u = RN_BN_CHUNK_U;
    return (int)blocks;
  }
  a.chunk_u = 0;
  return tr_blocks(max_units, 4096);
}

extern "C" int rn_bn_apply(const rn_bn_problem* p, void* stream) {
  BnArgs a;
  RN_CHECK_ARG(bn_fill(p, a, 0) == 0, "rn_bn_apply: bad problem");
  long long mx = 0;
  for (int i = 0; i < a.nseg; ++i) {
    RN_CHECK_ARG(a.seg[i].y && a.seg[i].z && a.seg[i].fwd, "rn_bn_apply: null tensor");
    const long long t = a.seg[i].P * (a.seg[i].C / 8);
    if (t > mx) mx = t;
  }
  hipLaunchKernelGGL(bn_apply_kernel, dim3(bn_elementwise_grid(a, mx), a.nseg), dim3(TR_THREADS), 0, (hipStream_t)stream, a);
  RN_CHECK_LAUNCH();
  return RN_OK;
}

extern "C" int rn_bn_bwd_colsum_chunks(const rn_bn_problem* p, int segment) {
  BnArgs a;
  if (bn_fill(p, a, 0) || segment < 0 || segment >= a.nseg) return 0;
  long long mx = 0;
  for (int i = 0; i < a.nseg; ++i) {
    const long long t = a.seg[i].P * (a.seg[i].C / 8);
    if (t > mx) mx = t;
  }
  bn_elementwise_grid(a, mx);
  if (a.chunk_u <= 0) return 0;
  return (int)rn_cdiv(a.seg[segment].P * (a.seg[segment].C / 8), 256ll * a.chunk_u);
}

extern "C" int rn_bn_bwd_apply(const rn_bn_problem* p, void* stream) {
  BnArgs a;
  RN_CHECK_ARG(bn_fill(p, a, 0) == 0, "rn_bn_bwd_apply: bad problem");
  long long mx = 0;
  for (int i = 0; i < a.nseg; ++i) {
    RN_CHECK_ARG(a.seg[i].y && a.seg[i].dz && a.seg[i].dy && a.seg[i].fwd && a.seg[i].bsums,
                 "rn_bn_bwd_apply: null tensor");
    RN_CHECK_ARG(a.act == RN_ACT_NONE || a.seg[i].z || a.seg[i].mask, "rn_bn_bwd_apply: z needed for the activation mask");
    const long long t = a.seg[i].P * (a.seg[i].C / 8);
    if (t > mx) mx = t;
  }
  {
    const dim3 grid(bn_elementwise_grid(a, mx), a.nseg), block(TR_THREADS);
    for (int i = 0; i < a.nseg; ++i)
      RN_CHECK_ARG(!a.seg[i].colsum || a.chunk_u > 0,
                   "rn_bn_bwd_apply: dy_colsum_partial needs the chunked form (rn_bn_bwd_colsum_chunks() > 0)");
#define BN_CALL_(G_) hipLaunchKernelGGL(bn_bwd_apply_kernel<G_>, grid, block, 0, (hipStream_t)stream, a)
    BN_DISPATCH_GATE(bn_gate_mode(p), BN_CALL_)
#undef BN_CALL_
  }
  RN_CHECK_LAUNCH();
  return RN_OK;
}

__global__ void __launch_bounds__(TR_THREADS)
act_bwd_kernel(const uint4* __restrict__ dz, const uint4* __restrict__ z, uint4* __restrict__ dy, long long n8,
               int act) {
  for (long long i = blockIdx.x * (long long)blockDim.x + threadIdx.x; i < n8;
       i += (long long)gridDim.x * blockDim.x) {
    bf8 g = unpack8(dz[i]);
    const bf8 zz = unpack8(z[i]);
#pragma unroll
    for (int q = 0; q < 8; ++q) g.v[q] *= act_mask(zz.v[q], act);
    dy[i] = pack8(g);
  }
}

__global__ void __launch_bounds__(TR_THREADS)
cast_f32_bf16_kernel(const float4* __restrict__ x, uint2* __restrict__ y, long long n4) {
  for (long long i = blockIdx.x * (long long)blockDim.x + threadIdx.x; i < n4;
       i += (long long)gridDim.x * blockDim.x) {
    const float4 v = x[i];
    uint2 o;
    o.x = rn_pack_bf16x2(v.x, v.y);
    o.y = rn_pack_bf16x2(v.z, v.w);
    y[i] = o;
  }
}
__global__ void __launch_bounds__(TR_THREADS)
cast_pad_kernel(const float* __restrict__ x, uint2* __restrict__ y, long long P, int C, int Cpad) {
  const int q = Cpad / 4;
  const long long total = P * q;
  for (long long i = blockIdx.x * (long long)blockDim.x + threadIdx.x; i < total;
       i += (long long)gridDim.x * blockDim.x) {
    const long long r = i / q;
    const int c = (int)(i - r * q) * 4;
    float v[4];
#pragma unroll
    for (int u = 0; u < 4; ++u) v[u] = (c + u) < C ? x[r * C + c + u] : 0.0f;
    uint2 o;
    o.x = rn_pack_bf16x2(v[0], v[1]);
    o.y = rn_pack_bf16x2(v[2], v[3]);
    y[i] = o;
  }
}
extern "C" int rn_cast_pad_f32_to_bf16(const float* x, void* y, int64_t P, int C, int Cpad, void* stream) {
  RN_CHECK_ARG(x && y && P > 0 && C > 0 && Cpad >= C && Cpad % 4 == 0, "rn_cast_pad_f32_to_bf16: bad argument");
  hipLaunchKernelGGL(cast_pad_kernel, dim3(tr_blocks(P * (Cpad / 4))), dim3(TR_THREADS), 0, (hipStream_t)stream, x,
                     (uint2*)y, (long long)P, C, Cpad);
  RN_CHECK_LAUNCH();
  return RN_OK;
}
extern "C" int rn_cast_f32_to_bf16(const float* x, void* y, int64_t n, void* stream) {
  RN_CHECK_ARG(x && y && n > 0 && n % 4 == 0, "rn_cast_f32_to_bf16: bad argument (n %% 4 == 0)");
  hipLaunchKernelGGL(cast_f32_bf16_kernel, dim3(tr_blocks(n / 4)), dim3(TR_THREADS), 0, (hipStream_t)stream,
                     (const float4*)x, (uint2*)y, (long long)(n / 4));
  RN_CHECK_LAUNCH();
  return RN_OK;
}

__global__ void __launch_bounds__(TR_THREADS)
reduce_rows_kernel(const float* __restrict__ src, int rows, long long row_stride, int n, float add, float* __restrict__ dst) {
  const int c = blockIdx.x * blockDim.x + threadIdx.x;
  if (c >= n) return;
  float s = 0.0f;
  for (int r = 0; r < rows; ++r) s += src[r * row_stride + c];
  dst[c] = s + add;
}
extern "C" int rn_reduce_rows_f32(const float* src, int rows, int64_t row_stride, int n, float add, float* dst, void* stream) {
  RN_CHECK_ARG(src && dst && rows > 0 && n > 0 && row_stride >= 0, "rn_reduce_rows_f32: bad argument");
  hipLaunchKernelGGL(reduce_rows_kernel, dim3((n + TR_THREADS - 1) / TR_THREADS), dim3(TR_THREADS), 0, (hipStream_t)stream,
                     src, rows, (long long)row_stride, n, add, dst);
  RN_CHECK_LAUNCH();
  return RN_OK;
}

__global__ void __launch_bounds__(TR_THREADS)
upsample_zero_kernel(const uint4* __restrict__ x, uint4* __restrict__ y, int N, int H, int W, int C8, int Ho,
                     int Wo) {
  const long long total = (long long)N * Ho * Wo * C8;
  for (long long i = blockIdx.x * (long long)blockDim.x + threadIdx.x; i < total;
       i += (long long)gridDim.x * blockDim.x) {
    const RnIdx4 d_ = rn_decode4(i, C8, Wo, Ho, rn_decode_mode(total, C8));
    const int c = d_.c, ox = d_.x, oy = d_.y, n = d_.n;
    uint4 v = make_uint4(0u, 0u, 0u, 0u);
    if (!(ox & 1) && !(oy & 1) && (oy >> 1) < H && (ox >> 1) < W)
      v = x[(((long long)n * H + (oy >> 1)) * W + (ox >> 1)) * C8 + c];
    y[i] = v;
  }
}
extern "C" int rn_upsample_zero2x(const void* x, void* y, int N, int H, int W, int C, int Ho, int Wo,
                                  void* stream) {
  RN_CHECK_ARG(x && y && N > 0 && H > 0 && W > 0 && C % 8 == 0 && Ho >= 2 * H - 1 && Wo >= 2 * W - 1,
               "rn_upsample_zero2x: bad argument");
  hipLaunchKernelGGL(upsample_zero_kernel, dim3(tr_blocks((long long)N * Ho * Wo * (C / 8))), dim3(TR_THREADS), 0,
                     (hipStream_t)stream, (const uint4*)x, (uint4*)y, N, H, W, C / 8, Ho, Wo);
  RN_CHECK_LAUNCH();
  return RN_OK;
}

__global__ void __launch_bounds__(TR_THREADS)
scatter_add2x_kernel(const uint4* __restrict__ x, uint4* __restrict__ y, int N, int H, int W, int C8, int Ho, int Wo) {
  const long long total = (long long)N * H * W * C8;
  for (long long i = blockIdx.x * (long long)blockDim.x + threadIdx.x; i < total;
       i += (long long)gridDim.x * blockDim.x) {
    const RnIdx4 d_ = rn_decode4(i, C8, W, H, rn_decode_mode(total, C8));
    const int c = d_.c, w = d_.x, h = d_.y, n = d_.n;
    if (2 * h >= Ho || 2 * w >= Wo) continue;
    const long long o = (((long long)n * Ho + 2 * h) * Wo + 2 * w) * C8 + c;
    const bf8 a = unpack8(x[i]), b = unpack8(y[o]);
    bf8 r;
#pragma unroll
    for (int q = 0; q < 8; ++q) r.v[q] = a.v[q] + b.v[q];
    y[o] = pack8(r);
  }
}
extern "C" int rn_scatter_add2x(const void* x, void* y, int N, int H, int W, int C, int Ho, int Wo, int accumulate,
                                void* stream) {
  RN_CHECK_ARG(x && y && N > 0 && H > 0 && W > 0 && C % 8 == 0 && Ho >= 2 * H - 1 && Wo >= 2 * W - 1,
               "rn_scatter_add2x: bad argument");
  if (!accumulate) return rn_upsample_zero2x(x, y, N, H, W, C, Ho, Wo, stream);
  hipLaunchKernelGGL(scatter_add2x_kernel, dim3(tr_blocks((long long)N * H * W * (C / 8))), dim3(TR_THREADS), 0,
                     (hipStream_t)stream, (const uint4*)x, (uint4*)y, N, H, W, C / 8, Ho, Wo);
  RN_CHECK_LAUNCH();
  return RN_OK;
}

__global__ void __launch_bounds__(TR_THREADS)
depth_to_space2x_kernel(const uint4* __restrict__ x, uint4* __restrict__ y, int N, int H, int W, int C8, int accumulate) {
  const long long total = (long long)N * H * W * 4 * C8;
  for (long long i = blockIdx.x * (long long)blockDim.x + threadIdx.x; i < total;
       i += (long long)gridDim.x * blockDim.x) {
    const RnIdx4 d_ = rn_decode4(i, C8, 4 * W, H, rn_decode_mode(total, C8));
    const int c = d_.c, ph = d_.x & 3, w = d_.x >> 2, h = d_.y, n = d_.n;
    const long long o = (((long long)n * 2 * H + 2 * h + (ph >> 1)) * 2 * W + 2 * w + (ph & 1)) * C8 + c;
    uint4 v = x[i];
    if (accumulate) {
      const bf8 a = unpack8(v), b = unpack8(y[o]);
      bf8 r;
#pragma unroll
      for (int q = 0; q < 8; ++q) r.v[q] = a.v[q] + b.v[q];
      v = pack8(r);
    }
    y[o] = v;
  }
}
extern "C" int rn_depth_to_space2x(const void* x, void* y, int N, int H, int W, int C, int accumulate, void* stream) {
  RN_CHECK_ARG(x && y && N > 0 && H > 0 && W > 0 && C > 0 && C % 8 == 0, "rn_depth_to_space2x: bad argument");
  hipLaunchKernelGGL(depth_to_space2x_kernel, dim3(tr_blocks((long long)N * H * W * 4 * (C / 8))), dim3(TR_THREADS), 0,
                     (hipStream_t)stream, (const uint4*)x, (uint4*)y, N, H, W, C / 8, accumulate);
  RN_CHECK_LAUNCH();
  return RN_OK;
}

extern "C" int rn_act_bwd(const void* dz, const void* z, void* dy, int64_t n, int act, void* stream) {
// ... 319 lines not shown
```

### retinanet-tensorflow2.x_amd/retinanet/_C.py

```python
from __future__ import annotations

import ctypes
import logging
import os
from ctypes import (POINTER, Structure, c_char_p, c_float, c_int, c_int32, c_int64, c_longlong, c_size_t, c_uint32,
                    c_uint64, c_void_p)

_HERE = os.path.dirname(os.path.abspath(__file__))
LIB_PATH = os.environ.get("RNET_HIP_LIB") or os.path.join(_HERE, "librnet_hip.so")
LIB_PATH_F16 = os.environ.get("RNET_HIP_LIB_F16") or os.path.join(_HERE, "librnet_hip_f16.so")

RN_DT_F32, RN_DT_BF16 = 0, 1
RN_OK, RN_EINVAL, RN_ENOMEM, RN_EHIP, RN_ECOMM, RN_EUNSUPPORTED = 0, -1, -2, -3, -4, -5
RN_ACT_NONE, RN_ACT_RELU, RN_ACT_RELU6, RN_ACT_SWISH = 0, 1, 2, 3
RN_CONV_MAX_SEGMENTS = 10
ABI_VERSION = 8
PRED_W_TERMS = int(os.environ.get("RNET_PRED_W_TERMS", "2"))
ACT_IDS = {None: RN_ACT_NONE, "none": RN_ACT_NONE, "relu": RN_ACT_RELU, "relu6": RN_ACT_RELU6,
           "swish": RN_ACT_SWISH}


class RnetError(RuntimeError):
    pass


class DgradPack(Structure):
    _fields_ = [("w_ohwi", c_void_p), ("w_packed", c_void_p), ("R", c_int32), ("S", c_int32), ("Cin", c_int32),
                ("Cout", c_int32), ("Cout_pad", c_int32), ("pad_", c_int32)]


class ExampleInfo(Structure):
    _fields_ = [("image_offset", c_uint64), ("image_length", c_uint64), ("image_id", c_int64),
                ("n_xmins", c_int32), ("n_ymins", c_int32), ("n_xmaxs", c_int32), ("n_ymaxs", c_int32),
                ("n_classes", c_int32), ("pad_", c_int32)]


class LaunchOpts(Structure):
    _fields_ = [("conv_tile", c_int32), ("conv_no_halo", c_int32), ("conv_big_min_tiles", c_int32),
                ("max_workgroups", c_int32), ("reserved_cus", c_int32), ("wgrad_kernel", c_int32),
                ("wgrad_target_blocks", c_int32), ("ablate", c_int32), ("splitk_target_blocks", c_int32)]

    def __init__(self, **kw):
        super().__init__()
        for k, v in kw.items():
            if k not in dict(self._fields_):
                raise TypeError(f"rn_launch_opts has no field {k!r}")
            setattr(self, k, int(v))

    def copy(self, **kw):
        o = LaunchOpts(**{k: getattr(self, k) for k, _ in self._fields_})
        for k, v in kw.items():
            setattr(o, k, int(v))
        return o


class Bottleneck64Problem(Structure):
    _fields_ = [("x", c_void_p), ("y", c_void_p), ("w_packed", c_void_p), ("affine", c_void_p), ("N", c_int32), ("H", c_int32),
                ("W", c_int32), ("Cx", c_int32), ("opts", LaunchOpts)]


class ConvSegment(Structure):
    _fields_ = [("x", c_void_p), ("w", c_void_p), ("y", c_void_p), ("scale", c_void_p), ("shift", c_void_p),
                ("residual", c_void_p), ("N", c_int32), ("H", c_int32), ("W", c_int32), ("Cin", c_int32),
                ("pix_stride", c_int32), ("Ho", c_int32), ("Wo", c_int32), ("Cout", c_int32), ("bn_partial", c_void_p),
                ("bias", c_void_p), ("w_terms", c_int32), ("w_pair", c_int32), ("bn_bwd_y", c_void_p),
                ("bn_bwd_fwd", c_void_p)]


class ConvProblem(Structure):
    _fields_ = [("R", c_int32), ("S", c_int32), ("stride_h", c_int32), ("stride_w", c_int32),
                ("pad_top", c_int32), ("pad_left", c_int32), ("act", c_int32), ("out_dtype", c_int32),
                ("num_segments", c_int32), ("seg", ConvSegment * RN_CONV_MAX_SEGMENTS), ("opts", LaunchOpts),
                ("splitk_ws", c_void_p), ("splitk_ws_bytes", c_int64)]


class WgradSegment(Structure):
    _fields_ = [("x", c_void_p), ("dy", c_void_p), ("N", c_int32), ("H", c_int32), ("W", c_int32),
                ("Cin", c_int32), ("Ho", c_int32), ("Wo", c_int32), ("Cout", c_int32),
                ("dy_pix_stride", c_int32), ("x_pix_stride", c_int32)]


class WgradProblem(Structure):
    _fields_ = [("R", c_int32), ("S", c_int32), ("stride_h", c_int32), ("stride_w", c_int32),
                ("pad_top", c_int32), ("pad_left", c_int32), ("num_segments", c_int32),
                ("seg", WgradSegment * RN_CONV_MAX_SEGMENTS), ("opts", LaunchOpts)]


class DwSegment(Structure):
    _fields_ = [("x", c_void_p), ("w", c_void_p), ("y", c_void_p), ("scale", c_void_p), ("shift", c_void_p),
                ("residual", c_void_p),
                ("N", c_int32), ("H", c_int32), ("W", c_int32), ("C", c_int32), ("Ho", c_int32), ("Wo", c_int32)]


class DwProblem(Structure):
    _fields_ = [("k", c_int32), ("stride", c_int32), ("pad_top", c_int32), ("pad_left", c_int32), ("act", c_int32),
                ("num_segments", c_int32), ("seg", DwSegment * RN_CONV_MAX_SEGMENTS)]


class BnSegment(Structure):
    _fields_ = [("y", c_void_p), ("z", c_void_p), ("residual", c_void_p), ("dz", c_void_p), ("dy", c_void_p),
                ("dres", c_void_p), ("sums", c_void_p), ("fwd", c_void_p), ("bsums", c_void_p),
                ("gamma", c_void_p), ("beta", c_void_p), ("moving_mean", c_void_p), ("moving_var", c_void_p),
                ("dgamma", c_void_p), ("dbeta", c_void_p), ("P", c_int64), ("C", c_int32),
                ("dres_accumulate", c_int32), ("sample_scale", c_void_p), ("rows_per_sample", c_int64),
                ("ext_chunks", c_int32), ("ext_chunks_bwd", c_int32), ("act_mask", c_void_p),
                ("dy_colsum_partial", c_void_p)]


class BnProblem(Structure):
    _fields_ = [("num_segments", c_int32), ("act", c_int32), ("bessel", c_int32), ("eps", c_float),
                ("momentum", c_float), ("count_scale", c_float), ("seg", BnSegment * RN_CONV_MAX_SEGMENTS)]


_PP = POINTER(c_void_p)
_SIGNATURES = {
    "rn_last_error": (c_char_p, []),
    "rn_abi_version": (c_int, []),
    "rn_storage_dtype": (c_int, []),
    "rn_device_ok": (c_int, []),
    "rn_anchors_generate": (c_int, [c_void_p, c_int64, c_int, c_int, c_int, c_int, POINTER(c_float),
                                    POINTER(c_float), c_int, POINTER(c_float), c_int, POINTER(c_int64),
                                    c_void_p]),
    "rn_match_workspace_bytes": (c_size_t, [c_int, c_int]),
    "rn_anchor_match_encode": (c_int, [c_void_p, c_int64, c_void_p, c_void_p, c_void_p, c_int, c_int, c_float,
                                       c_float, POINTER(c_float), c_void_p, c_void_p, c_void_p, c_void_p,
                                       c_void_p, c_size_t, c_void_p]),
    "rn_loss_workspace_bytes": (c_size_t, [c_int, c_int64, c_int]),
    "rn_retinanet_loss_fwd_bwd": (c_int, [_PP, _PP, _PP, _PP, POINTER(c_int64), c_int, c_int, c_int, c_void_p,
                                          c_void_p, c_void_p, c_float, c_float, c_float, c_float, c_float,
                                          c_float, c_float, c_void_p, c_void_p, c_size_t, c_void_p]),
    "rn_retinanet_loss_fwd_bwd_bf16": (c_int, [_PP, _PP, _PP, _PP, c_int, c_int, c_int, POINTER(c_int64), c_int, c_int,
                                               c_int, c_void_p, c_void_p, c_void_p, c_float, c_float, c_float, c_float,
                                               c_float, c_float, c_float, c_void_p, c_void_p, c_size_t, c_void_p]),
    "rn_decode_boxes": (c_int, [_PP, POINTER(c_int64), c_int, c_int, c_void_p, POINTER(c_float), c_float,
                                c_float, c_void_p, c_void_p]),
    "rn_sigmoid_scores": (c_int, [_PP, POINTER(c_int64), c_int, c_int, c_int, c_void_p, c_void_p]),
    "rn_topk_workspace_bytes": (c_size_t, [c_int, c_int64, c_int]),
    "rn_topk_per_class": (c_int, [c_void_p, c_int, c_int64, c_int, c_int, c_void_p, c_void_p, c_void_p,
                                  c_size_t, c_void_p]),
    "rn_detect_workspace_bytes": (c_size_t, [c_int, c_int64, c_int, c_int]),
    "rn_detect_per_class": (c_int, [_PP, POINTER(c_int64), c_int, c_int, c_int, c_void_p, c_int, c_float,
                                    c_float, c_float, c_int, c_void_p, c_void_p, c_void_p, c_void_p, c_void_p,
                                    c_size_t, c_void_p]),
    "rn_nms_workspace_bytes": (c_size_t, [c_int, c_int, c_int, c_int]),
    "rn_nms_per_class": (c_int, [c_void_p, c_void_p, c_int, c_int, c_int, c_float, c_float, c_float, c_int,
                                 c_void_p, c_void_p, c_void_p, c_void_p, c_void_p, c_void_p, c_size_t, c_void_p]),
    "rn_rowmax_argmax": (c_int, [c_void_p, c_int64, c_int, c_void_p, c_void_p, c_void_p]),
    "rn_conv2d_nhwc_fwd": (c_int, [POINTER(ConvProblem), c_void_p]),
    "rn_conv_cout_pad": (c_int, [c_int]),
    "rn_conv_tile_rows": (c_int, [POINTER(ConvProblem)]),
    "rn_conv_bn_row_blocks": (c_int, [POINTER(ConvProblem), c_int]),
    "rn_probe_spin": (c_int, [c_int, c_void_p]),
    "rn_conv_kernel_id": (c_int, [POINTER(ConvProblem)]),
    "rn_conv_splitk_workspace_bytes": (c_size_t, [POINTER(ConvProblem)]),
    "rn_conv_splitk_workspace_max_bytes": (c_size_t, []),
    "rn_conv_cin_pad": (c_int, [c_int]),
    "rn_depthwise_conv2d_nhwc_fwd": (c_int, [POINTER(DwProblem), c_void_p]),
    "rn_pack_depthwise_weight": (c_int, [c_void_p, c_int, c_int, c_void_p, c_void_p]),
    "rn_pack_depthwise_weight_flip": (c_int, [c_void_p, c_int, c_int, c_void_p, c_void_p]),
    "rn_depthwise_wgrad_workspace_bytes": (c_size_t, [POINTER(DwProblem)]),
    "rn_depthwise_conv2d_nhwc_wgrad": (c_int, [POINTER(DwProblem), c_void_p, c_void_p, c_size_t, c_void_p]),
    "rn_squeeze_excite_fwd": (c_int, [c_void_p, c_void_p, c_int, c_int, c_int, c_void_p, c_void_p, c_void_p, c_void_p,
                                      c_int, c_void_p, c_size_t, c_void_p]),
    "rn_squeeze_excite_bwd": (c_int, [c_void_p, c_void_p, c_void_p, c_int, c_int, c_int, c_void_p, c_void_p, c_int,
                                      c_void_p, c_void_p, c_void_p, c_void_p, c_void_p, c_void_p, c_size_t, c_void_p]),
    "rn_coco_accumulate": (c_int, [c_void_p, c_void_p, c_void_p, c_void_p, c_float, c_float, c_void_p, c_int, c_int, c_int,
                                   c_int, c_void_p, c_void_p, c_void_p]),
    "rn_pack_conv_weight_ohwi": (c_int, [c_void_p, c_int, c_int, c_int, c_int, c_int, c_void_p, c_void_p]),
    "rn_se_workspace_bytes": (c_size_t, [c_int, c_int]),
    "rn_squeeze_excite_inplace": (c_int, [c_void_p, c_int, c_int, c_int, c_void_p, c_void_p, c_void_p, c_void_p,
                                          c_int, c_void_p, c_size_t, c_void_p]),
    "rn_pack_conv_weight": (c_int, [c_void_p, c_int, c_int, c_int, c_int, c_int, c_void_p, c_void_p]),
    "rn_conv_pair_rows": (c_int, [c_int]),
    "rn_pack_conv_weight_pair": (c_int, [c_void_p, c_int, c_int, c_int, c_int, c_int, c_int, c_void_p, c_void_p]),
    "rn_pack_conv_weight_split": (c_int, [c_void_p, c_int, c_int, c_int, c_int, c_int, c_int, c_int, c_void_p,
                                          c_void_p]),
    "rn_pack_stem_weight": (c_int, [c_void_p, c_int, c_void_p, c_void_p]),
    "rn_stem_padded_width": (c_int, [c_int]),
    "rn_pack_stem_input": (c_int, [c_void_p, c_int, c_int, c_int, c_void_p, c_void_p]),
    "rn_pack_stem_weight_rs": (c_int, [c_void_p, c_int, c_int, c_int, c_void_p, c_void_p]),
    "rn_pack_image_nhwc4": (c_int, [c_void_p, c_int, c_int, c_int, c_int, c_int, c_int, c_int, c_void_p, c_void_p]),
    "rn_wgrad_workspace_bytes": (c_size_t, [POINTER(WgradProblem)]),
    "rn_wgrad_kernel_id": (c_int, [POINTER(WgradProblem)]),
    "rn_conv2d_nhwc_wgrad": (c_int, [POINTER(WgradProblem), c_void_p, c_float, c_void_p, c_size_t, c_void_p]),
    "rn_wgrad_group_workspace_bytes": (c_size_t, [POINTER(POINTER(WgradProblem)), c_int]),
    "rn_wgrad_group_fused": (c_int, [POINTER(POINTER(WgradProblem)), c_int]),
    "rn_conv2d_nhwc_wgrad_group": (c_int, [POINTER(POINTER(WgradProblem)), c_int, _PP, c_float, c_void_p, c_size_t,
                                           c_void_p]),
    "rn_pack_conv_weight_dgrad": (c_int, [c_void_p, c_int, c_int, c_int, c_int, c_int, c_void_p, c_void_p]),
    "rn_pack_conv_weight_dgrad_batch": (c_int, [POINTER(DgradPack), c_int, c_void_p]),
    "rn_cast_pad_f32_to_bf16": (c_int, [c_void_p, c_void_p, c_int64, c_int, c_int, c_void_p]),
    "rn_reduce_rows_f32": (c_int, [c_void_p, c_int, c_int64, c_int, c_float, c_void_p, c_void_p]),
    "rn_upsample_zero2x": (c_int, [c_void_p, c_void_p, c_int, c_int, c_int, c_int, c_int, c_int, c_void_p]),
    "rn_scatter_add2x": (c_int, [c_void_p, c_void_p, c_int, c_int, c_int, c_int, c_int, c_int, c_int, c_void_p]),
    "rn_depth_to_space2x": (c_int, [c_void_p, c_void_p, c_int, c_int, c_int, c_int, c_int, c_void_p]),
    "rn_cast_f32_to_bf16": (c_int, [c_void_p, c_void_p, c_int64, c_void_p]),
    "rn_act_bwd": (c_int, [c_void_p, c_void_p, c_void_p, c_int64, c_int, c_void_p]),
    "rn_bn_workspace_bytes": (c_size_t, [POINTER(BnProblem)]),
    "rn_bn_workspace_init": (c_int, [POINTER(BnProblem), c_void_p, c_size_t, c_void_p]),
    "rn_bn_partial_offset_bytes": (c_size_t, [POINTER(BnProblem), c_int]),
    "rn_bn_bwd_partial_offset_bytes": (c_size_t, [POINTER(BnProblem), c_int]),
    "rn_bn_stats": (c_int, [POINTER(BnProblem), c_void_p, c_size_t, c_void_p]),
    "rn_bn_stats_finalize": (c_int, [POINTER(BnProblem), c_void_p, c_size_t, c_void_p]),
    "rn_bn_finalize": (c_int, [POINTER(BnProblem), c_void_p]),
    "rn_bn_apply": (c_int, [POINTER(BnProblem), c_void_p]),
    "rn_bn_bwd_reduce": (c_int, [POINTER(BnProblem), c_void_p, c_size_t, c_void_p]),
    "rn_bn_bwd_apply": (c_int, [POINTER(BnProblem), c_void_p]),
    "rn_bn_bwd_colsum_chunks": (c_int, [POINTER(BnProblem), c_int]),
    "rn_maxpool2d_nhwc_bwd": (c_int, [c_void_p, c_void_p, c_void_p, c_int, c_int, c_int, c_int, c_int, c_int,
                                      c_int, c_int, c_int, c_int, c_int, c_void_p]),
    "rn_fpn_topdown_bwd_level": (c_int, [c_void_p, c_void_p, c_void_p, c_void_p, c_int, c_int, c_int, c_int,
                                         c_int, c_void_p]),
    "rn_balance_features_bwd_scratch_bytes": (c_size_t, [c_int, c_int, c_int, c_int, c_int, c_int]),
    "rn_balance_features_bwd": (c_int, [_PP, _PP, _PP, c_void_p, c_void_p, c_size_t, c_int, c_int, c_int, c_int, c_int,
                                        c_int, c_void_p]),
    "rn_optim_chunk": (c_int, []),
    "rn_optim_workspace_bytes": (c_size_t, [c_int, c_int]),
    "rn_optim_clip": (c_int, [c_void_p, c_void_p, c_void_p, c_int, c_void_p, c_int, c_float, c_float, c_float, c_float,
                              c_void_p, c_void_p, c_size_t, c_void_p]),
    "rn_optim_clip_prepare": (c_int, [c_void_p, c_void_p, c_void_p, c_void_p, c_int, c_int, c_int, c_float, c_float,
                                      c_void_p, c_void_p, c_size_t, c_void_p]),
    "rn_optim_clip_factors": (c_int, [c_void_p, c_int, c_int, c_float, c_float, c_void_p, c_void_p, c_void_p, c_size_t,
                                      c_void_p]),
    "rn_optim_clip_apply": (c_int, [c_void_p, c_void_p, c_void_p, c_void_p, c_int, c_void_p, c_size_t, c_void_p]),
    "rn_optim_sgd_step": (c_int, [c_void_p, c_void_p, c_void_p, c_void_p, c_void_p, c_void_p, c_void_p, c_int,
                                  c_float, c_float, c_float, c_int, c_void_p, c_void_p]),
    "rn_prepare_image": (c_int, [c_void_p, c_int, c_int, c_int, c_int, c_void_p, c_int, c_int, POINTER(c_float),
                                 POINTER(c_float), c_float, c_void_p]),
    "rn_bottleneck64_supported": (c_int, [c_int, c_int, c_int, c_int]),
    "rn_bottleneck64_packed_bytes": (c_size_t, [c_int]),
    "rn_bottleneck64_pack": (c_int, [c_void_p, c_void_p, c_void_p, c_void_p, c_int, c_void_p, c_void_p]),
# ... 45 lines not shown
def lib(f16=False):
    f16 = bool(f16)
    if f16 not in _libs:
        path = LIB_PATH_F16 if f16 else LIB_PATH
        if not os.path.exists(path):
            raise RnetError(
                f"{path} is missing: build it with `python -c 'import __graft_entry__ as g; g.build()'` "
                "(hipcc --offload-arch=gfx950).  There is no CPU fallback.")
        import torch
        handle = ctypes.CDLL(path)
        for name, (res, args) in _SIGNATURES.items():
            fn = getattr(handle, name)
            fn.restype = res
            fn.argtypes = args
        if handle.rn_abi_version() != ABI_VERSION:
            raise RnetError(f"{path}: ABI version {handle.rn_abi_version()}, this binding needs {ABI_VERSION}: rebuild")
        if handle.rn_storage_dtype() != (1 if f16 else 0):
            raise RnetError(f"{path}: built for the other 16-bit storage type: rebuild")
        _libs[f16] = handle
    return _libs[f16]


class Handle:

    def __init__(self, library, device_id, opts=None):
        self.lib = library
        self.h = c_void_p()
        check(library.rn_create(int(device_id), ctypes.byref(self.h)), "rn_create")
        if opts is not None:
            self.set_launch_opts(opts)

    def set_launch_opts(self, opts):
        check(self.lib.rn_handle_set_launch_opts(self.h, ctypes.byref(opts)), "rn_handle_set_launch_opts")

    def launch_opts(self):
        o = LaunchOpts()
        check(self.lib.rn_handle_get_launch_opts(self.h, ctypes.byref(o)), "rn_handle_get_launch_opts")
        return o

    @property
    def device(self):
        return self.lib.rn_handle_device(self.h)

    @property
    def num_cus(self):
        return self.lib.rn_handle_num_cus(self.h)

    def comm_init(self, slot, unique_id, rank, world):
        check(self.lib.rn_handle_comm_init(self.h, int(slot), unique_id, int(rank), int(world)), "rn_handle_comm_init")
        return c_void_p(self.lib.rn_handle_comm(self.h, int(slot)))

    def close(self):
        if self.h:
            self.lib.rn_destroy(self.h)
            self.h = c_void_p()

    def __del__(self):
        try:
            self.close()
        except Exception:
            pass


def check(status: int, what: str = ""):
    if status != 0:
        msgs = [h.rn_last_error() for h in _libs.values()]
        msg = b" | ".join(m for m in msgs if m)
        raise RnetError(f"{what} failed with status {status}: {msg.decode() if msg else ''}")


def ptr(t):
    return None if t is None else c_void_p(t.data_ptr())


def ptr_array(tensors):
    if tensors is None:
        return None
    arr = (c_void_p * len(tensors))()
    for i, t in enumerate(tensors):
        arr[i] = None if t is None else t.data_ptr()
    return ctypes.cast(arr, _PP)


def f32_array(values):
    if values is None:
        return None
    return (c_float * len(values))(*[float(v) for v in values])


def i64_array(values):
    return (c_int64 * len(values))(*[int(v) for v in values])


def current_stream():
    import torch
    return c_void_p(torch.cuda.current_stream().cuda_stream)


def wait_blocks(lib_, a, probe, main, helper, spin_us=600, pre=None):
    import time
    import torch
    t0 = time.perf_counter()
    if pre is not None:
        pre()
    probe()
    host_us = (time.perf_counter() - t0) * 1e6
    torch.cuda.synchronize(a.device)
    t0 = time.perf_counter()
    if pre is not None:
        pre()
    probe()
    host_us = min(host_us, (time.perf_counter() - t0) * 1e6)
    spin_us = int(min(max(spin_us, 8.0 * host_us), 20000))
    torch.cuda.synchronize(a.device)
    gate = torch.cuda.Event()
    check(lib_.rn_probe_spin(int(spin_us), c_void_p(helper.cuda_stream)), "rn_probe_spin")
    gate.record(helper)
    e0, e1 = torch.cuda.Event(enable_timing=True), torch.cuda.Event(enable_timing=True)
    e0.record(main)
    a.wait_event(gate)
    if pre is not None:
        pre()
    probe()
    e1.record(main)
    torch.cuda.synchronize(a.device)
    took_us = e0.elapsed_time(e1) * 1e3
    blocked = took_us > 0.5 * spin_us
    logging.getLogger("retinanet").debug("wait_blocks: spin %d us, host enqueue %.0f us, probe took %.0f us -> %s",
                                         spin_us, host_us, took_us, "blocked" if blocked else "free")
    return blocked


def concurrent_stream(lib_, device, others, attempts=12, probes=(), agree=None):
    import torch
    if os.environ.get("RNET_STREAM_PROBE", "1") == "0" or not others:
        return torch.cuda.Stream(device), None
    held, s = [], None
    with torch.cuda.device(device):
        helper = torch.cuda.Stream(device)
        held.append(helper)
        main = others[0]
        for _ in range(attempts):
            s = torch.cuda.Stream(device)
            ok = True
            for o in others:
                kern_o = lambda o=o: check(lib_.rn_probe_spin(1, c_void_p(o.cuda_stream)), "rn_probe_spin")
                kern_s = lambda s=s: check(lib_.rn_probe_spin(1, c_void_p(s.cuda_stream)), "rn_probe_spin")
                ok = ok and not wait_blocks(lib_, s, kern_o, o, helper) and not wait_blocks(lib_, o, kern_s, s, helper)
                if not ok:
                    break
            for pr in probes:
                blocked = wait_blocks(lib_, s, pr, main, helper)
                ok = ok and not blocked
            if agree is not None:
                ok = bool(agree(ok))
            if ok:
                return s, True
            held.append(s)
    return s, False


def new_splitk_workspace(lib_, device, default_on=False):
    import torch
    on = os.environ.get("RNET_SPLITK", "1" if default_on else "0") == "1"
    if not on:
        return None
# ... 25 lines not shown
```

### retinanet-tensorflow2.x_amd/retinanet/model/train_engine.py

```python
from __future__ import annotations

import ctypes
import os
from typing import NamedTuple

import numpy as np
import torch

from retinanet import _C
from .bottleneck import Bottleneck64, fused_blocks
from .forward import (FoldedConvs, conv_launch_name, conv_problem, dw_problem, half_activations, maxpool_step, split_by_depth,
                      stem_input, stem_pool_partner, stem_pool_step, stem_problem, tensor_readers, topdown_step)

_DT = {"bf16": torch.bfloat16, "f32": torch.float32}
_SEG_DTYPE = np.dtype([("offset", "<i8"), ("size", "<i8"), ("wd", "<i4"), ("bb", "<i4"), ("nb", "<i4"),
                       ("pad", "<i4"), ("bf", "<i8")])


def _hwio_to_ohwi(w):
    return w.permute(3, 0, 1, 2).contiguous()


def _ohwi_to_hwio(w):
    return w.permute(1, 2, 3, 0).contiguous()


class BnGroup(NamedTuple):
    problem: _C.BnProblem
    sums: torch.Tensor
    bsums: torch.Tensor
    ws: torch.Tensor
    dys: list
    ops: list


class TrainEngine:
    def __init__(self, model, batch_size, frozen_regexes=(), process_group=None, world_size=None, frozen_names=(),
                 launch_opts=None, wide_pred_terms=None, force_dp=None):
        self.model = model
        self.g = model.graph
        self.params_cfg = model.params
        self.B = int(batch_size)
        self.dev = model.device
        env = os.environ.get
        if force_dp is None:
            force_dp = env("RNET_FORCE_DP", "0") == "1"
        if wide_pred_terms is None:
            wide_pred_terms = env("RNET_TRAIN_PRED_W_TERMS") or \
                getattr(getattr(model.params, "training", None), "prediction_weight_planes", None) or 2
        comm_cus = int(env("RNET_COMM_CUS", "8"))
        self.fuse_bn_stats = env("RNET_FUSE_BN_STATS", "1") != "0"
        self.fuse_bn_bwd = env("RNET_FUSE_BN_BWD", "1") != "0"
        self.fuse_bn_bwd_groups = env("RNET_FUSE_BN_BWD", "1") == "2"
        self.side_stream_on = env("RNET_WGRAD_STREAM", "1") != "0"
        cus = env("RNET_WGRAD_CUS", "160,208")
        self._wgrad_cap = tuple(int(v) for v in cus.split(",")) if cus not in ("0", "") else None
        if not self.side_stream_on:
            self._wgrad_cap = None
        if self._wgrad_cap and len(self._wgrad_cap) == 1:
            self._wgrad_cap = (self._wgrad_cap[0], 2 * self._wgrad_cap[0])
        self._wgrad_group_mode = env("RNET_WGRAD_GROUP", "halo")
        self._ab_workspaces = env("RNET_AB_WORKSPACES") == "1"
        self._stream_probe = env("RNET_STREAM_PROBE", "1") != "0"
        self._bucket_bytes = int(env("RNET_C1_BUCKET_MB", "25")) << 20
        self.f16 = half_activations(model.params)
        self.h16 = torch.float16 if self.f16 else torch.bfloat16
        self._DT = {"bf16": self.h16, "f32": torch.float32}
        self.lib = _C.lib(self.f16)
        self.pg = process_group
        if world_size is None:
            import torch.distributed as dist
            world_size = dist.get_world_size(process_group) if dist.is_available() and dist.is_initialized() else 1
        self.world = int(world_size)
        bn = self.params_cfg.architecture.batch_norm
        self.eps, self.momentum_bn = float(bn.epsilon), float(bn.momentum)
        self.dp_active = self.world > 1 or bool(force_dp)
        self.sync_bn = bool(bn.use_sync) and self.dp_active
        if isinstance(launch_opts, dict):
            launch_opts = _C.LaunchOpts(**launch_opts)
        self.launch_opts = launch_opts.copy() if launch_opts is not None else _C.LaunchOpts()
        if self.dp_active and not self.launch_opts.reserved_cus:
            self.launch_opts.reserved_cus = comm_cus
        self.handle = _C.Handle(self.lib, self.dev.index if self.dev.index is not None else torch.cuda.current_device(),
                                self.launch_opts)
        self.wide_pred_terms = max(1, min(int(wide_pred_terms), _C.PRED_W_TERMS))
        self.frozen = set(frozen_names)
        for k in model.variables:
            if any(rx.search(k) for rx in frozen_regexes):
                self.frozen.add(k)
        self._keep = []
        self._algo = {}
        self.conv_launches = []
        self._launch_names = {}
        self.wgrad_launches = []
        self.dw_launches = []
        self.dw_wgrad_launches = []
        self.se_launches = []
        self._wgrad_capped = []
        self.stem_packed = None
        self._bn_of_tensor = {}
        self.bn_bwd_ws = {}
        self._bn_bwd_pending = {}
        self.bn_bwd_fused = []
        self.dy_of = {}
        self._loss_dy = None
        self._dgrad_pack_items = None
        self.drop_connect = True
        self.dc_masks = {}
        self.dc_all = self.dc_p = None
        self.dc_generator = torch.Generator(device=self.dev)
        self.dc_generator.manual_seed(1337)
        self.step_count = 0
        self.loss_scale = None
        self._ls_host = self._ls_event = None
        self._ls_pending = False
        self._train_step_active = False
        self._images_ref = None
        self._step_args = dict(wdc=0.0, alpha=0.0, unscale=1.0, clip=0.0)
        self._side_stream = None
        self._side_events = []
        self.side_stream_probed = None
        self._dgrad_prepacked = False
        self.conv_profile = None
        self.wgrad_profile = None
        self.layer_profile = None
        self.hbm_profile = None
        self._c2_local, self._c2_sent, self.c2_normalizer = None, False, None
        self.native_comm = None
        self.native_comm_buckets = None
        self._small_msgs = 0
        self.syncbn_messages_per_step = None
        self._overlap_on = False
        self._overlap_done = 0
        self._overlap_works = []
        self._buckets = None
        self._bucket_at = {}
        self._comm_events = []
        self._bucket_stream = None
        self._overlap_last_event = None
        self.L = None
        self.pg_c1 = None
        self._probe_bucket_group = False
        self._overlap_unsafe = False
        self._flag_host = self._flag_event = None
        self.clip_fired = False
        self.bucket_host_ms = 0.0
        self.price_without_flag_read = False
        self._prepare_graph()
        with torch.cuda.device(self.dev):
            self.splitk_ws = _C.new_splitk_workspace(self.lib, self.dev)
            self.folded = FoldedConvs(self.lib, self.g, self.B, self.dev, self.h16, self.launch_opts, self.splitk_ws,
                                      self.eps, eligible=self._inference_form)
            self._analyse()
            self._alloc_params()
            self._alloc_tensors()
            self._fold_frozen()
            self._build_forward()
            self._build_backward()
            self._group_wgrad_steps()
            for name, cp in self.conv_launches:
                marks = {bool(cp.seg[i].bn_bwd_y) for i in range(cp.num_segments)}
                if name.startswith("dgrad:") and len(marks) != 1:
                    raise RuntimeError(f"{name}: BatchNorm backward fusion covers only part of the launch's segments")

    def _prepare_graph(self):
        g = self.g
        self.tensors = dict(g.tensors)
        self.ops = []
        alias = {}
        for op in g.ops:
            o = dict(op)
            for key in ("inp", "residual"):
                if o.get(key) in alias:
                    o[key] = alias[o[key]]
            if o["op"] == "se":
                t = o["tensor"]
                o["inp"], o["out"] = alias.get(t, t), t + ":se"
                self.tensors[o["out"]] = g.tensors[t]
                alias[t] = o["out"]
            if o["op"] in ("topdown",):
                o["ins"] = [alias.get(n, n) for n in o["ins"]]
            self.ops.append(o)
        self.readers = tensor_readers(self.ops)
        self.var_kind = {}
        for cname, c in g.convs.items():
            self.var_kind[c.get("kvar", cname + "/kernel")] = ("conv", cname)
        for dname, d in getattr(g, "dws", {}).items():
            self.var_kind[d["kvar"]] = ("dw", dname)
        for sname in getattr(g, "ses", {}):
            self.var_kind[sname + "/conv2d/kernel"] = ("se1", sname)
            self.var_kind[sname + "/conv2d_1/kernel"] = ("se2", sname)

    def _kvar(self, op):
        if op["op"] == "dwconv":
            return self.g.dws[op["dw"]]["kvar"]
        c = self.g.convs[op["conv"]]
        return c.get("kvar", op["conv"] + "/kernel")

    def _conv_trainable(self, op):
        return self._kvar(op) not in self.frozen

    def _bn_trainable(self, op):
        return op.get("bn") and (op["bn"] + "/gamma") not in self.frozen

    def _inference_form(self, op):
        return not self._conv_trainable(op) and not self._bn_trainable(op) and not self.requires.get(op["inp"])

    def _analyse(self):
        self.requires = {"images": False}
        for op in self.ops:
            kind = op["op"]
            if kind in ("conv", "stem"):
                tr = self._conv_trainable(op) or bool(self._bn_trainable(op))
                ins = [op["inp"]] + ([op["residual"]] if op.get("residual") else [])
                self.requires[op["out"]] = tr or any(self.requires[i] for i in ins)
            elif kind == "maxpool":
                self.requires[op["out"]] = self.requires[op["inp"]]
            elif kind == "topdown":
                r = any(self.requires[i] for i in op["ins"])
                for o in op["outs"]:
                    self.requires[o] = r or self.requires.get(o, False)
            elif kind == "balance":
                pass
            elif kind == "dwconv":
                if not self._conv_trainable(op):
                    raise NotImplementedError("frozen depthwise layers are not a shipped configuration")
                self.requires[op["out"]] = True
            elif kind == "se":
                if any((op["se"] + sfx) in self.frozen for sfx in ("/conv2d/kernel", "/conv2d_1/kernel")):
                    raise NotImplementedError("frozen squeeze-excite layers are not a shipped configuration")
                self.requires[op["out"]] = True
            else:
                raise NotImplementedError(f"training through '{kind}' ops is not built")
        for op in self.ops:
            if op["op"] in ("conv", "stem", "dwconv") and op.get("bn") and \
                    self._conv_trainable(op) != bool(self._bn_trainable(op)):
                raise NotImplementedError(f"{self._kvar(op)}: conv and its BatchNorm must be frozen together")

    def _alloc_params(self):
        lib = self.lib
        chunk = lib.rn_optim_chunk()
        v = self.model.variables
# ... 717 lines not shown
    @staticmethod
    def _wgrad_bytes(p):
        b = 0
        for i in range(p.num_segments):
            s = p.seg[i]
            b += 2 * s.N * s.H * s.W * s.Cin + 2 * s.N * s.Ho * s.Wo * s.Cout
        return b + 4 * p.R * p.S * p.seg[0].Cin * p.seg[0].Cout

    def _wgrad_kernel_name(self, p):
        return ("wgrad_kernel (128x128 per-tap tiles)", "wgrad_big_kernel (256x256 per-tap tiles)",
                "wgrad_halo_kernel")[max(self.lib.rn_wgrad_kernel_id(ctypes.byref(p)), 0)]

    def _wgrad_workspace(self, problems, size):
        def largest(field, values):
            old = [getattr(p.opts, field) for p in problems]
            n = 0
            for v in values:
                for p in problems:
                    setattr(p.opts, field, v)
                n = max(n, size())
            for p, v in zip(problems, old):
                setattr(p.opts, field, v)
            return n
        nws = size()
        if any(p.opts.wgrad_target_blocks for p in problems):
            nws = max(nws, largest("wgrad_target_blocks", (0,)))
        if self._ab_workspaces:
            nws = max(nws, largest("wgrad_kernel", (1, 3)))
        return torch.empty((max(nws, 256),), dtype=torch.uint8, device=self.dev)

    def _wgrad_step(self, call, args, what, flops, byts, kname, lname, writes):
        def wgrad(st):
            prof, lprof = self.wgrad_profile, self.layer_profile
            if prof is None and lprof is None:
                _C.check(call(*args, st), what)
                return
            self._timed(lambda: _C.check(call(*args, st), what), (prof, (flops, kname)), (lprof, (lname, flops, byts, kname)))
        return self._side(wgrad, writes=writes)

    def _group_wgrad_steps(self):
        lib = self.lib
        self.wgrad_groups = []
        if self._wgrad_group_mode == "0":
            return
        by_sig = {}
        for i, fn in enumerate(self.bwd_steps):
            item = getattr(fn, "wgrad_item", None)
            if item is None:
                continue
            p = item[0]
            sig = (p.R, p.S, p.stride_h, p.stride_w, p.pad_top, p.pad_left, p.num_segments, bytes(p.opts),
                   tuple((s.N, s.H, s.W, s.Cin, s.Ho, s.Wo, s.Cout, s.dy_pix_stride, s.x_pix_stride)
                         for s in (p.seg[k] for k in range(p.num_segments))))
            by_sig.setdefault(sig, []).append(i)
        drop, replace = set(), {}
        for sig, idxs in by_sig.items():
            for lo in range(0, len(idxs), 8):
                grp = idxs[lo:lo + 8]
                if len(grp) < 2:
                    continue
                items = [self.bwd_steps[i].wgrad_item for i in grp]
                probs = [it[0] for it in items]
                arr = (ctypes.POINTER(_C.WgradProblem) * len(grp))(*[ctypes.pointer(p) for p in probs])
                if lib.rn_wgrad_group_fused(arr, len(grp)) != 1:
                    continue
                if self._wgrad_group_mode != "all" and lib.rn_wgrad_kernel_id(ctypes.byref(probs[0])) != 2:
                    continue
                ws = self._wgrad_workspace(probs, lambda: lib.rn_wgrad_group_workspace_bytes(arr, len(grp)))
                dws = _C.ptr_array([it[1] for it in items])
                wname = f"{self._wgrad_kernel_name(probs[0])} ({len(grp)} layers per launch) + wgrad_reduce_kernel"
                lname = "wgrad:" + "+".join(n[len("wgrad:"):] for n, q in self.wgrad_launches
                                            if any(q is p for p in probs))
                self._keep += [arr, dws, ws]
                old_ws = {id(it[2]) for it in items}
                self._keep = [k for k in self._keep if id(k) not in old_ws]
                replace[grp[-1]] = self._wgrad_step(
                    lib.rn_conv2d_nhwc_wgrad_group, (arr, len(grp), dws, 0.0, ws.data_ptr(), ws.numel()),
                    "rn_conv2d_nhwc_wgrad_group", sum(it[3] for it in items), sum(self._wgrad_bytes(p) for p in probs),
                    wname, lname, [w for i in grp for w in self.bwd_steps[i].writes])
                drop.update(grp[:-1])
                self.wgrad_groups.append(probs)
        self.bwd_steps = [replace.get(i, fn) for i, fn in enumerate(self.bwd_steps) if i not in drop]

    def _bn_bwd_step(self, grp, ws, profiled=True):
        lib, pb, prb, bsums = self.lib, grp.problem, ctypes.byref(grp.problem), grp.bsums
        bracket = self._bn_pass if profiled else (lambda kind, pb, fn: fn())

        def run(st):
            bracket("bn_bwd_reduce", pb, lambda: _C.check(lib.rn_bn_bwd_reduce(prb, _C.ptr(ws), ws.numel(), st),
                                                           "rn_bn_bwd_reduce"))
            if self.sync_bn:
                self._allreduce_small(bsums)
            bracket("bn_bwd_apply", pb, lambda: _C.check(lib.rn_bn_bwd_apply(prb, st), "rn_bn_bwd_apply"))
        run.writes = [op["bn"] + sfx for op in grp.ops for sfx in ("/gamma", "/beta")]
        return run

    @staticmethod
    def _distinct_inputs(ops):
        launches = []
        for op in ops:
            for sub in launches:
                if all(o["inp"] != op["inp"] for o in sub):
                    sub.append(op)
                    break
            else:
                launches.append([op])
        return launches

    def _plan_conv_backward(self, ops, mark):
        lib, B = self.lib, self.B
        if not self._conv_trainable(ops[0]) and not any(self.requires.get(o["inp"]) for o in ops):
            return
        if not self._conv_trainable(ops[0]):
            raise NotImplementedError("backward through a frozen conv that sits above trainable layers")
        live_bn = bool(self._bn_trainable(ops[0]))
        if live_bn:
            grp = self.bn_groups[ops[0]["out"]]
            pb = grp.problem
            for i, op in enumerate(ops):
                s = pb.seg[i]
                s.dz = self.grad[op["out"]].data_ptr()
                if op.get("residual") and self.requires.get(op["residual"]):
                    dres, first = self._grad_target(op["residual"], mark, balanced=False)
                    s.dres, s.dres_accumulate = dres.data_ptr(), 0 if first else 1
            self.bwd_steps.append(self._bn_bwd_step(grp, self.bn_bwd_ws.get(id(pb), grp.ws)))
            dy_of = {op["out"]: grp.dys[i] for i, op in enumerate(ops)}
        else:
            dy_of = {}
            for op in ops:
                if op["out_dtype"] == "f32":
                    shp = list(self.t[op["out"]].shape)
                    shp[3] = (shp[3] + 63) // 64 * 64
                    dyb = torch.zeros(shp, dtype=self.h16, device=self.dev)
                    dy_of[op["out"]] = dyb
                else:
                    dyb = torch.empty_like(self.t[op["out"]])
                    dy_of[op["out"]] = dyb
                    a = (self.grad[op["out"]].data_ptr(), self.t[op["out"]].data_ptr(), dyb.data_ptr(),
                         dyb.numel(), _C.ACT_IDS[op["act"]])
                    self.bwd_steps.append(lambda st, a=a: _C.check(lib.rn_act_bwd(*a, st), "rn_act_bwd"))
            self._keep += list(dy_of.values())
        self.dy_of.update(dy_of)
        by_conv = {}
        for op in ops:
            by_conv.setdefault(op["conv"], []).append(op)
        for cname, cops in by_conv.items():
            c = self.g.convs[cname]
            kvar = c.get("kvar", cname + "/kernel")
            p = _C.WgradProblem()
            p.opts = self.launch_opts
            p.R = p.S = c["k"]
            p.stride_h = p.stride_w = c["stride"]
            p.pad_top = p.pad_left = cops[0]["pad"]
            p.num_segments = len(cops)
            for i, op in enumerate(cops):
                x, dy = self._src(op["inp"]), dy_of[op["out"]]
                s = p.seg[i]
                s.x, s.dy = x.data_ptr(), dy.data_ptr()
                s.N, s.H, s.W, s.Cin, s.Ho, s.Wo, s.Cout = B, x.shape[1], x.shape[2], c["cin"], dy.shape[1], dy.shape[2], c["cout"]
                s.dy_pix_stride = dy.shape[3]
            if self._wgrad_cap and not p.opts.wgrad_target_blocks:
                kid = lib.rn_wgrad_kernel_id(ctypes.byref(p))
                p.opts.wgrad_target_blocks = self._wgrad_cap[0] if kid in (1, 2) else self._wgrad_cap[1]
                self._wgrad_capped.append((p, int(p.opts.wgrad_target_blocks)))
            ws = self._wgrad_workspace([p], lambda: lib.rn_wgrad_workspace_bytes(ctypes.byref(p)))
            dw = self._pview(kvar, self.G)
            self._keep += [p, ws]
            self.wgrad_launches.append(("wgrad:" + cname, p))
            flw = sum(2 * B * p.seg[i].Ho * p.seg[i].Wo * c["k"] * c["k"] * c["cin"] * c["cout"] for i in range(len(cops)))
            step = self._wgrad_step(lib.rn_conv2d_nhwc_wgrad, (ctypes.byref(p), dw.data_ptr(), 0.0, ws.data_ptr(), ws.numel()),
                                    "rn_conv2d_nhwc_wgrad", flw, self._wgrad_bytes(p),
                                    self._wgrad_kernel_name(p) + " + wgrad_reduce_kernel", "wgrad:" + cname, [kvar])
            step.wgrad_item = (p, dw, ws, flw)
            self.bwd_steps.append(step)
            if c["bias"]:
                pb2 = _C.BnProblem()
                pb2.num_segments, pb2.act, pb2.bessel, pb2.eps, pb2.momentum, pb2.count_scale = len(cops), 0, 0, 0.0, 0.0, 1.0
                cw = dy_of[cops[0]["out"]].shape[3]
                bs = torch.zeros((len(cops), 2, cw), dtype=torch.float32, device=self.dev)
                for i, op in enumerate(cops):
                    dy = dy_of[op["out"]]
                    s = pb2.seg[i]
                    s.y, s.sums = dy.data_ptr(), bs[i].data_ptr()
                    s.P, s.C = dy.shape[0] * dy.shape[1] * dy.shape[2], cw
                fused_cs = False
                if live_bn:
                    seg_of = [ops.index(op) for op in cops]
                    chunks = [lib.rn_bn_bwd_colsum_chunks(ctypes.byref(pb), j) for j in seg_of]
                    if all(ch > 0 for ch in chunks):
                        fused_cs = True
                        for i, ch in enumerate(chunks):
                            pb2.seg[i].ext_chunks = ch
                ws2 = torch.zeros((max(lib.rn_bn_workspace_bytes(ctypes.byref(pb2)), 256),), dtype=torch.uint8,
                                  device=self.dev)
                if fused_cs:
                    for i, j in enumerate(seg_of):
                        pb.seg[j].dy_colsum_partial = ws2.data_ptr() + lib.rn_bn_partial_offset_bytes(ctypes.byref(pb2), i)
                db = self._pview(cname + "/bias", self.G)
                self._keep += [pb2, bs, ws2]

                def bias_grad(st, pr=ctypes.byref(pb2), ws2=ws2, bs=bs, db=db, n=c["cout"], rows=len(cops), stride=2 * cw):
                    _C.check(lib.rn_bn_stats(pr, _C.ptr(ws2), ws2.numel(), st), "bias colsum")
                    _C.check(lib.rn_reduce_rows_f32(_C.ptr(bs), rows, stride, n, 0.0, _C.ptr(db), st), "bias grad")
                self.bwd_steps.append(self._side(bias_grad, writes=[cname + "/bias"]))
        packs = {}
        for sub in self._distinct_inputs([op for op in ops if self.requires.get(op["inp"])]):
            self._plan_dgrad_launch(sub, dy_of, mark, packs)

    def _plan_dw_backward(self, ops, mark):
        lib, B = self.lib, self.B
        if self._bn_trainable(ops[0]):
            grp = self.bn_groups[ops[0]["out"]]
            for i, op in enumerate(ops):
                grp.problem.seg[i].dz = self.grad[op["out"]].data_ptr()
            self.bwd_steps.append(self._bn_bwd_step(grp, grp.ws))
            dy_of = {op["out"]: grp.dys[i] for i, op in enumerate(ops)}
        else:
            dy_of = {op["out"]: self.grad[op["out"]] for op in ops}
        by_layer = {}
        for op in ops:
            by_layer.setdefault(op["dw"], []).append(op)
        for dname, dops in by_layer.items():
            d = self.g.dws[dname]
            p = _C.DwProblem()
            p.k, p.stride, p.pad_top, p.pad_left, p.act = d["k"], d["stride"], dops[0]["pad_top"], dops[0]["pad_left"], 0
            p.num_segments = len(dops)
            for i, op in enumerate(dops):
                x, dy = self._src(op["inp"]), dy_of[op["out"]]
                s = p.seg[i]
                s.x, s.y = x.data_ptr(), dy.data_ptr()
                s.N, s.H, s.W, s.C, s.Ho, s.Wo = B, x.shape[1], x.shape[2], d["C"], dy.shape[1], dy.shape[2]
            ws = torch.empty((max(lib.rn_depthwise_wgrad_workspace_bytes(ctypes.byref(p)), 256),), dtype=torch.uint8,
                             device=self.dev)
            self._keep += [p, ws]
            self.dw_wgrad_launches.append(("dw_wgrad:" + dname, p))
            a = (ctypes.byref(p), self._pview(d["kvar"], self.G).data_ptr(), ws.data_ptr(), ws.numel())
            self.bwd_steps.append(self._side(lambda st, a=a: _C.check(lib.rn_depthwise_conv2d_nhwc_wgrad(*a, st),
                                                                     "dw wgrad"), writes=[d["kvar"]]))
        flips = {}
        for sub in self._distinct_inputs([op for op in ops if self.requires.get(op["inp"])]):
            d0 = self.g.dws[sub[0]["dw"]]
            k, stride = d0["k"], d0["stride"]
            if stride not in (1, 2):
                raise NotImplementedError("stride > 2")
            p = _C.DwProblem()
            p.k, p.stride, p.act, p.num_segments = k, 1, 0, len(sub)
            p.pad_top, p.pad_left = k - 1 - sub[0]["pad_top"], k - 1 - sub[0]["pad_left"]
            ups = []
            for i, op in enumerate(sub):
                d = self.g.dws[op["dw"]]
                if op["dw"] not in flips:
                    buf = torch.empty((k * k, d["C"]), dtype=self.h16, device=self.dev)
                    flips[op["dw"]] = buf
                    off, _ = self.p_off[d["kvar"]]
                    self.dw_flip_packs.append((self.P.data_ptr() + 4 * off, k, d["C"], buf))
                src = dy_of[op["out"]]
                x = self._src(op["inp"])
                H, W = x.shape[1], x.shape[2]
                if stride == 2:
                    src, up_args = self._zero_upsampled(src, H, W)
                    ups.append(up_args)
                gbuf, first = self._grad_target(op["inp"], mark)
                s = p.seg[i]
                s.x, s.w, s.y = src.data_ptr(), flips[op["dw"]].data_ptr(), gbuf.data_ptr()
                s.scale, s.shift = None, None
                s.residual = None if first else gbuf.data_ptr()
                s.N, s.H, s.W, s.C, s.Ho, s.Wo = B, H, W, d["C"], H, W
            self._keep.append(p)
            self.dw_launches.append(("dw_dgrad:" + "+".join(o["out"] for o in sub), "dgrad", p, ups))

            def dgrad(st, p=p, ups=ups):
                for u in ups:
                    _C.check(lib.rn_upsample_zero2x(*u, st), "rn_upsample_zero2x")
                _C.check(lib.rn_depthwise_conv2d_nhwc_fwd(ctypes.byref(p), st), "dw dgrad")
            self.bwd_steps.append(dgrad)

    def _bn_bwd_fusable(self, name):
        if not self.fuse_bn_bwd or name in self.bal_src or len(self.readers.get(name, [])) != 1:
            return None
        hit = self._bn_of_tensor.get(name)
        if hit is None:
            return None
        pb, i, o, nseg = hit
        if nseg != 1 and not self.fuse_bn_bwd_groups:
            return None
        if (o["op"] != "conv" or o.get("act") != "relu" or o.get("residual") or
                o.get("survival") is not None or not self._bn_trainable(o) or pb.seg[i].sample_scale):
# ... 16 lines not shown
            pb = pend["pb"]
            if pend.get("dead") or pend.get("done") or sorted(pend["seg"]) != list(range(pb.num_segments)):
                continue
            pend["done"] = True
            for j, (cp, ci, _) in pend["seg"].items():
                pb.seg[j].ext_chunks_bwd = lib.rn_conv_bn_row_blocks(ctypes.byref(cp), ci)
            wsb = torch.zeros((max(lib.rn_bn_workspace_bytes(ctypes.byref(pb)), 256),), dtype=torch.uint8, device=self.dev)
            self.bn_bwd_ws[key] = wsb
            for j, (cp, ci, name) in pend["seg"].items():
                sg = cp.seg[ci]
                sg.bn_partial = wsb.data_ptr() + lib.rn_bn_bwd_partial_offset_bytes(ctypes.byref(pb), j)
                sg.bn_bwd_y = self.raw[name].data_ptr()
                sg.bn_bwd_fwd = pb.seg[j].fwd
                self.bn_bwd_fused.append(name)
                y_bytes = 2 * int(pb.seg[j].P) * int(pb.seg[j].C)
                if cp is p:
                    added += y_bytes
                else:
                    fl0, by0 = self._algo[id(cp)]
                    self._algo[id(cp)] = (fl0, by0 + y_bytes)
        return added

    def _plan_dgrad_launch(self, need, dy_of, mark, packs):
        lib, B = self.lib, self.B
        c0 = self.g.convs[need[0]["conv"]]
        k, stride, pad = c0["k"], c0["stride"], need[0]["pad"]
        if stride not in (1, 2):
            raise NotImplementedError("stride > 2")
        lowres = k == 1 and stride == 2 and pad == 0
        subpixel = (k == 3 and stride == 2 and pad == 1
                    and all(self._src(o["inp"]).shape[1] % 2 == 0 and self._src(o["inp"]).shape[2] % 2 == 0
                            and self.g.convs[o["conv"]]["cin"] % 8 == 0 for o in need))
        p = _C.attach_splitk_workspace(_C.ConvProblem(), self.splitk_ws)
        p.opts = self.launch_opts
        p.R = p.S = 2 if subpixel else k
        p.stride_h = p.stride_w = 1
        p.pad_top = p.pad_left = 0 if subpixel else k - 1 - pad
        p.act, p.out_dtype, p.num_segments = _C.RN_ACT_NONE, _C.RN_DT_BF16, len(need)
        ups, post, firsts = [], [], []
        post_op = ((lib.rn_depth_to_space2x, "rn_depth_to_space2x") if subpixel else
                   (lib.rn_scatter_add2x, "rn_scatter_add2x") if lowres else None)
        fl = by = 0
        for i, op in enumerate(need):
            c = self.g.convs[op["conv"]]
            cin = c["cin"]
            dy = dy_of[op["out"]]
            cw = dy.shape[3]
            cwp = lib.rn_conv_cin_pad(cw)
            if op["conv"] not in packs:
                shape = (lib.rn_conv_cout_pad(4 * cin), 2, 2, cwp) if subpixel else (lib.rn_conv_cout_pad(cin), k, k, cwp)
                packs[op["conv"]] = torch.empty(shape, dtype=self.h16, device=self.dev)
                off, _ = self.p_off[c.get("kvar", op["conv"] + "/kernel")]
                self.dgrad_packs.append((self.P.data_ptr() + 4 * off, k, cin, c["cout"], cwp, packs[op["conv"]],
                                         1 if subpixel else 0))
            x = self._src(op["inp"])
            H, W = x.shape[1], x.shape[2]
            gbuf, first = self._grad_target(op["inp"], mark)
            firsts.append(first)
            src, dst, cout, res = dy, gbuf, cin, None
            if subpixel:
                cout = 4 * cin
                dst = torch.empty((B, dy.shape[1], dy.shape[2], cout), dtype=self.h16, device=self.dev)
                post.append((dst.data_ptr(), gbuf.data_ptr(), B, dy.shape[1], dy.shape[2], cin, 0 if first else 1))
            elif lowres:
                dst = torch.empty((B, dy.shape[1], dy.shape[2], cin), dtype=self.h16, device=self.dev)
                post.append((dst.data_ptr(), gbuf.data_ptr(), B, dy.shape[1], dy.shape[2], cin, H, W, 0 if first else 1))
            else:
                if stride == 2:
                    src, up_args = self._zero_upsampled(dy, H, W)
                    ups.append(up_args)
                res = None if first else gbuf.data_ptr()
            if dst is not gbuf:
                self._keep.append(dst)
            s = p.seg[i]
            s.x, s.w, s.y = src.data_ptr(), packs[op["conv"]].data_ptr(), dst.data_ptr()
            s.scale, s.shift, s.residual = None, None, res
            s.N, s.H, s.W, s.Cin, s.pix_stride = B, src.shape[1], src.shape[2], cw, cw
            s.Ho, s.Wo, s.Cout = dst.shape[1], dst.shape[2], cout
            Ho, Wo = self.tensors[op["out"]][:2]
            fl += 2 * B * Ho * Wo * k * k * cin * c["cout"]
            by += 2 * B * Ho * Wo * c["cout"] + 2 * B * H * W * cin * (2 if res else 1) + 2 * k * k * cin * c["cout"]
        if post_op is None and stride == 1 and all(firsts):
            by += self._fuse_bn_bwd(p, need)
        self._algo[id(p)] = (fl, by)
        self._keep.append(p)
        self.conv_launches.append(("dgrad:" + (need[0].get("group") or need[0]["out"]), p))

        def dgrad(st, p=p, ups=ups, post=post):
            for u in ups:
                _C.check(lib.rn_upsample_zero2x(*u, st), "rn_upsample_zero2x")
            self._launch_conv(p, st, "dgrad")
            for a in post:
                _C.check(post_op[0](*a, st), post_op[1])
        self.bwd_steps.append(dgrad)

    def refresh_dgrad_weights(self, st):
        lib = self.lib
        if self.dgrad_packs:
            _C.check(lib.rn_pack_conv_weight_dgrad_batch(self._dgrad_pack_items, len(self.dgrad_packs), st),
                     "pack dgrad")
        for (mptr, k, C, buf) in self.dw_flip_packs:
            _C.check(lib.rn_pack_depthwise_weight_flip(mptr, k, C, buf.data_ptr(), st), "pack dw flip")

    def draw_drop_connect(self):
        u = torch.rand(self.dc_all.shape, generator=self.dc_generator, device=self.dev, dtype=torch.float32)
        torch.div(torch.floor(u.add_(self.dc_p)), self.dc_p, out=self.dc_all)

    def forward(self, images, draw=True):
        st = _C.current_stream()
        if draw and self.dc_masks:
            self.draw_drop_connect()
        own = self.t["images"]
        if (images.device == own.device and images.dtype == own.dtype and images.shape == own.shape
                and images.is_contiguous()):
            self._images_ref = images
            self._images_ptr = images.data_ptr()
        else:
            own.copy_(images, non_blocking=True)
            self._images_ptr = own.data_ptr()
        for fn in self.fwd_steps:
            fn(st)
        return self.outputs

    @staticmethod
    def _side(fn, writes=()):
        fn.side = True
        fn.writes = list(writes)
        return fn

    def _ensure_side_stream(self):
        if self._side_stream is None:
            probes, agree = [], None
            if self.dp_active and self.sync_bn and self.native_comm is None:
                import torch.distributed as dist
                if dist.is_available() and dist.is_initialized() and dist.get_backend(self.pg) == "nccl":
                    tiny = torch.zeros((64,), dtype=torch.float32, device=self.dev)
                    dist.all_reduce(tiny, group=self.pg)
                    probes.append(lambda tiny=tiny: dist.all_reduce(tiny, group=self.pg))

                    def agree(ok, dist=dist):
                        v = torch.tensor([1.0 if ok else 0.0], device=self.dev)
                        dist.all_reduce(v, op=dist.ReduceOp.MIN, group=self.pg)
                        return bool(v.item() == 1.0)
            self._side_stream, self.side_stream_probed = _C.concurrent_stream(
                self.lib, self.dev, [torch.cuda.current_stream(self.dev)], probes=probes, agree=agree)
            self._side_events = [torch.cuda.Event() for _ in self.bwd_steps]
        return self._side_stream

    def _prepack_dgrad_weights(self):
        if not self.side_stream_on:
            return
        side = self._ensure_side_stream()
        side.wait_stream(torch.cuda.current_stream(self.dev))
        with torch.cuda.stream(side):
            self.refresh_dgrad_weights(ctypes.c_void_p(side.cuda_stream))
        self._dgrad_prepacked = True

    def loss_grad_buffers(self):
        return self._loss_dy

    def backward(self, loss_grads):
        lib, st = self.lib, _C.current_stream()
        if loss_grads is not None:
            for key, okey in (("class-predictions", "class-predictions"), ("box-predictions", "box-predictions")):
                for lv, name in self.g.outputs[okey].items():
                    gsrc = loss_grads[key][lv]
# ... 311 lines not shown
```

Before: 1116 images/s.

## Add fused depth-to-space dgrad epilogue, batched bias grads, tiled dgrad weight pack

Adds an optional depth-to-space output mode to the big 1x1 conv kernel so sub-pixel dgrad results are scattered directly into the final layout, skipping a separate post-op pass. Adds a batched bias-gradient path that merges many per-layer colsum and reduce launches into two kernels. Rewrites the dgrad weight pack kernel to use a shared-memory transposed tile so writes are coalesced. The D2S and bias-batch paths are gated behind environment flags that default off, so by default only the pack kernel change runs. That kernel runs once per step and is small.

```diff
diff --git a/include/rnet_hip.h b/include/rnet_hip.h
--- a/include/rnet_hip.h
+++ b/include/rnet_hip.h
@@ -122,7 +122,10 @@
   int32_t w_pair;
   const void* bn_bwd_y;
   const float* bn_bwd_fwd;
+  int32_t out_mode;
+  int32_t pad_;
 } rn_conv_segment;
+#define RN_CONV_OUT_D2S 1
 
 typedef struct {
   int32_t R, S, stride_h, stride_w, pad_top, pad_left;
@@ -251,6 +254,16 @@
 int rn_bn_bwd_apply(const rn_bn_problem* problem, void* stream);
 int rn_bn_bwd_colsum_chunks(const rn_bn_problem* problem, int segment);
 
+typedef struct rn_bias_batch {
+  void* dev_args;
+  int32_t n, cblocks, segs, parts, cols;
+} rn_bias_batch;
+size_t rn_bias_grad_batch_bytes(int n);
+int rn_bias_grad_batch_init(const rn_bn_problem* const* problems , void* const* ws, const size_t* ws_bytes,
+                            float* const* db, const int* db_cols, int n, void* dev_args, size_t dev_bytes,
+                            rn_bias_batch* out);
+int rn_bias_grad_batch(const rn_bias_batch* batch, void* stream);
+
 int rn_maxpool2d_nhwc_bwd(const void* x, const void* dy, void* dx, int N, int H, int W, int C, int k, int stride,
                           int pad_top, int pad_left, int Ho, int Wo, int accumulate, void* stream);
 int rn_fpn_topdown_bwd_level(const void* dout, const void* din_finer, const void* out, void* din, int N, int H,
diff --git a/retinanet-tensorflow2.x_amd/csrc/rn_conv.hip b/retinanet-tensorflow2.x_amd/csrc/rn_conv.hip
--- a/retinanet-tensorflow2.x_amd/csrc/rn_conv.hip
+++ b/retinanet-tensorflow2.x_amd/csrc/rn_conv.hip
@@ -847,6 +847,18 @@
     }
     RN_CHECK_ARG((s.bn_bwd_y != nullptr) == (p->seg[0].bn_bwd_y != nullptr),
                  "rn_conv2d_nhwc_fwd: bn_bwd_y must be set on all segments or none");
+    if (s.out_mode) {
+      RN_CHECK_ARG(s.out_mode == RN_CONV_OUT_D2S, "rn_conv2d_nhwc_fwd: segment %d: out_mode=%d", i, s.out_mode);
+      RN_CHECK_ARG(kid == 1 && bal_rows == 0 && p->out_dtype == RN_DT_BF16 && p->act == RN_ACT_NONE && !s.scale && !s.shift &&
+                       !s.bias && !s.residual && !s.bn_partial && !s.bn_bwd_y && !s.w_pair,
+                   "rn_conv2d_nhwc_fwd: segment %d: depth-to-space output needs a plain bf16 launch (no scale / shift / bias / "
+                   "residual / activation / bn_partial) on the 256-row 1x1 kernel (rn_conv_kernel_id() == 1)", i);
+      RN_CHECK_ARG(s.Cout % 4 == 0 && (s.Cout / 4) % 64 == 0,
+                   "rn_conv2d_nhwc_fwd: segment %d: depth-to-space output needs Cout = 4 * C, C a multiple of 64 (Cout=%d)", i, s.Cout);
+      RN_CHECK_ARG(M < (1ll << 22),
+                   "rn_conv2d_nhwc_fwd: segment %d: depth-to-space output needs fewer than 2^22 output pixels", i);
+    }
+    RN_CHECK_ARG(s.out_mode == p->seg[0].out_mode, "rn_conv2d_nhwc_fwd: out_mode must be set on all segments or none");
     d.bias = s.bias;
     d.N = s.N; d.H = s.H; d.W = s.W; d.Cin = s.Cin; d.pix_stride = s.pix_stride;
     d.Ho = s.Ho; d.Wo = s.Wo; d.Cout = seg_cols(s);
@@ -896,6 +908,7 @@
     for (int i = 0; i < a.nseg; ++i)
       if (a.seg[i].M >= (1 << 22)) a.pad_ = 0;
     if (deal) a.pad_ |= 2;
+    if (p->seg[0].out_mode == RN_CONV_OUT_D2S) a.pad_ |= 4;
     return rn_launch_conv_big(a, f32, p->opts, st);
   }
   a.pad_ = 1;
diff --git a/retinanet-tensorflow2.x_amd/csrc/rn_conv_big.hip b/retinanet-tensorflow2.x_amd/csrc/rn_conv_big.hip
--- a/retinanet-tensorflow2.x_amd/csrc/rn_conv_big.hip
+++ b/retinanet-tensorflow2.x_amd/csrc/rn_conv_big.hip
@@ -7,7 +7,7 @@
 constexpr int RING_BYTES = STAGES * STAGE_BYTES, PATCH_BYTES = 4096;
 constexpr int LDS_BYTES = RING_BYTES + NW * PATCH_BYTES;
 
-template <bool OUT_F32, bool HAS_RES, bool BN_BWD = false>
+template <bool OUT_F32, bool HAS_RES, bool BN_BWD = false, bool D2S = false>
 __global__ void __launch_bounds__(512) conv_big_kernel(const ConvArgs args) {
   extern __shared__ __attribute__((aligned(16))) char smem[];
   const int total = args.total_tiles;
@@ -184,8 +184,8 @@
   } while (0)
 
   auto epilogue = [&]() __attribute__((always_inline)) {
-    big_epilogue<OUT_F32, HAS_RES, BN_BWD>(acc, args, c_si, c_m0, c_n0, wave, smem + RING_BYTES + wave * PATCH_BYTES,
-                                           BigEpiSrc(), c_mend, c_chunk0);
+    big_epilogue<OUT_F32, HAS_RES, BN_BWD, false, 2, D2S>(acc, args, c_si, c_m0, c_n0, wave,
+                                                          smem + RING_BYTES + wave * PATCH_BYTES, BigEpiSrc(), c_mend, c_chunk0);
   };
 
   BIG_SETUP_ISSUE();
@@ -244,13 +244,17 @@
                                      hipFuncAttributeMaxDynamicSharedMemorySize, LDS_BYTES));
     RN_CHECK_HIP(hipFuncSetAttribute((const void*)conv_big_kernel<false, false, true>,
                                      hipFuncAttributeMaxDynamicSharedMemorySize, LDS_BYTES));
+    RN_CHECK_HIP(hipFuncSetAttribute((const void*)conv_big_kernel<false, false, false, true>,
+                                     hipFuncAttributeMaxDynamicSharedMemorySize, LDS_BYTES));
     RN_ATTRS_DONE(attr_set);
   }
   const int grid = rn_persistent_grid(a.total_tiles, rn_num_cus(), opts);
   bool has_res = false;
   for (int i = 0; i < a.nseg; ++i) has_res = has_res || a.seg[i].residual != nullptr;
   const dim3 g3(grid), b3(512);
-  if (a.seg[0].bn_y) {
+  if (a.pad_ & 4) {
+    hipLaunchKernelGGL((conv_big_kernel<false, false, false, true>), g3, b3, LDS_BYTES, st, a);
+  } else if (a.seg[0].bn_y) {
     hipLaunchKernelGGL((conv_big_kernel<false, false, true>), g3, b3, LDS_BYTES, st, a);
   } else if (out_f32) {
     if (has_res) hipLaunchKernelGGL((conv_big_kernel<true, true>), g3, b3, LDS_BYTES, st, a);
diff --git a/retinanet-tensorflow2.x_amd/csrc/rn_conv_big_epi.h b/retinanet-tensorflow2.x_amd/csrc/rn_conv_big_epi.h
--- a/retinanet-tensorflow2.x_amd/csrc/rn_conv_big_epi.h
+++ b/retinanet-tensorflow2.x_amd/csrc/rn_conv_big_epi.h
@@ -134,11 +134,12 @@
     }
 }
 
-template <bool OUT_F32, bool HAS_RES, bool BN_BWD = false, bool FROM_WS = false, int WM = 2>
+template <bool OUT_F32, bool HAS_RES, bool BN_BWD = false, bool FROM_WS = false, int WM = 2, bool D2S = false>
 __device__ __forceinline__ void big_epilogue(f32x16_t (&acc)[4][2], const ConvArgs& args, int c_si, int c_m0,
                                              int c_n0, int wave, char* patch, const BigEpiSrc src = BigEpiSrc(),
                                              int m_end = -1, int chunk0 = -1) {
   static_assert(!(BN_BWD && (OUT_F32 || HAS_RES)), "BN_BWD: plain bf16 launches only");
+  static_assert(!(D2S && (OUT_F32 || HAS_RES || BN_BWD || FROM_WS)), "D2S: plain bf16 launches of whole tiles only");
   constexpr bool LOADS = HAS_RES || BN_BWD;
   const int wave_m = wave / (8 / WM), wave_n = wave % (8 / WM);
   const ConvSegDev& sg = args.seg[c_si];
@@ -197,6 +198,11 @@
     for (int q = 0; q < 8; ++q) st0[q] = st1[q] = 0.0f;
     char* const ybase = (char*)sg.y + ((long long)(mw0 + rrow) * Cout + nr) * 2;
     const long long row_bytes = (long long)Cout * 2;
+    const int d2s_C = Cout >> 2, d2s_ph = D2S ? nw0 / d2s_C : 0, d2s_Wo = sg.Wo;
+    const float d2s_rWo = D2S ? rn_rcp((float)d2s_Wo) : 0.0f;
+    const long long d2s_row_bytes = (long long)d2s_C * 2;
+    char* const d2s_base = (char*)sg.y + ((long long)(d2s_ph >> 1) * 2 * d2s_Wo + (d2s_ph & 1)) * d2s_row_bytes +
+                           (long long)(nr - d2s_ph * d2s_C) * 2;
     const int act = args.act;
     const bool clamp_lo = act == RN_ACT_RELU || act == RN_ACT_RELU6, clamp_hi = act == RN_ACT_RELU6;
     const bool affine = !BN_BWD && (sg.scale != nullptr || sg.shift != nullptr);
@@ -271,7 +277,12 @@
               ov.x = pk_min_i16(pk_max_i16(ov.x, lo2), hi2); ov.y = pk_min_i16(pk_max_i16(ov.y, lo2), hi2);
               ov.z = pk_min_i16(pk_max_i16(ov.z, lo2), hi2); ov.w = pk_min_i16(pk_max_i16(ov.w, lo2), hi2);
             }
-            if (!(EPI_ABLATE & 16) || ov.x == 0x12345678u) *(uint4*)(ybase + (long long)(i * 32 + pass * 8) * row_bytes) = ov;
+            if constexpr (D2S) {
+              const int t = rn_fdiv(m, d2s_Wo, d2s_rWo);
+              *(uint4*)(d2s_base + (4ll * t * d2s_Wo + 2 * (m - t * d2s_Wo)) * d2s_row_bytes) = ov;
+            } else {
+              if (!(EPI_ABLATE & 16) || ov.x == 0x12345678u) *(uint4*)(ybase + (long long)(i * 32 + pass * 8) * row_bytes) = ov;
+            }
             if (STATS == 1 || (STATS == 2 && stats)) {
               const float w[8] = {bf_lo(ov.x), bf_hi(ov.x), bf_lo(ov.y), bf_hi(ov.y),
                                   bf_lo(ov.z), bf_hi(ov.z), bf_lo(ov.w), bf_hi(ov.w)};
@@ -299,6 +310,8 @@
     typedef std::integral_constant<int, 2> runtime_t;
     if constexpr (BN_BWD) {
       blocks(std::true_type{}, on_t{}, off_t{}, off_t{});
+    } else if constexpr (D2S) {
+      blocks(std::true_type{}, off_t{}, off_t{}, off_t{});
     } else if (plain) {
       if (stats) blocks(std::true_type{}, on_t{}, off_t{}, off_t{});
       else blocks(std::true_type{}, off_t{}, off_t{}, off_t{});
diff --git a/retinanet-tensorflow2.x_amd/csrc/rn_core.hip b/retinanet-tensorflow2.x_amd/csrc/rn_core.hip
--- a/retinanet-tensorflow2.x_amd/csrc/rn_core.hip
+++ b/retinanet-tensorflow2.x_amd/csrc/rn_core.hip
@@ -13,7 +13,7 @@
 
 extern "C" const char* rn_last_error(void) { return g_rn_err; }
 
-extern "C" int rn_abi_version(void) { return 8; }
+extern "C" int rn_abi_version(void) { return 9; }
 
 extern "C" int rn_storage_dtype(void) {
 #ifdef RN_F16
diff --git a/retinanet-tensorflow2.x_amd/csrc/rn_optim.hip b/retinanet-tensorflow2.x_amd/csrc/rn_optim.hip
--- a/retinanet-tensorflow2.x_amd/csrc/rn_optim.hip
+++ b/retinanet-tensorflow2.x_amd/csrc/rn_optim.hip
@@ -316,38 +316,52 @@
   return w[(((long long)co * 3 + r) * 3 + s) * Cin + ci];
 }
 
+constexpr int PACK_TILE = 64;
+__device__ __forceinline__ int pack_dgrad_rows(const rn_dgrad_pack& it) {
+  const int n = it.pad_ == 1 ? 4 * it.Cin : it.Cin;
+  return n <= 64 ? 64 : ((n + 127) / 128) * 128;
+}
+__host__ __device__ __forceinline__ long long pack_dgrad_tiles(int rows, int taps, int Cout_pad) {
+  return (long long)(rows / PACK_TILE) * taps * ((Cout_pad + PACK_TILE - 1) / PACK_TILE);
+}
 __global__ void __launch_bounds__(256) pack_dgrad_batch_kernel(const DgradPackArgs a) {
+  __shared__ float tile[PACK_TILE][PACK_TILE + 1];
   const rn_dgrad_pack& it = a.item[blockIdx.y];
-  if (it.pad_ == 1) {
-    const int Cin = it.Cin, Cout = it.Cout, Cout_pad = it.Cout_pad;
-    const int rows = 4 * Cin <= 64 ? 64 : ((4 * Cin + 127) / 128) * 128;
-    const long long total = (long long)rows * 4 * Cout_pad;
-    uint16_t* __restrict__ out = (uint16_t*)it.w_packed;
-    for (long long i = blockIdx.x * (long long)blockDim.x + threadIdx.x; i < total;
-         i += (long long)gridDim.x * blockDim.x) {
-      const int co = (int)(i % Cout_pad);
-      const long long t = i / Cout_pad;
-      const int v = (int)(t & 1), u = (int)((t >> 1) & 1), n = (int)(t >> 2);
-      out[i] = rn_f32_to_bf16(dgrad_s2_weight(it.w_ohwi, Cin, Cout, n, u, v, co));
-    }
-    return;
-  }
+  const bool sub = it.pad_ == 1;
   const int R = it.R, S = it.S, Cin = it.Cin, Cout = it.Cout, Cout_pad = it.Cout_pad;
-  const int Cin_pad = Cin <= 64 ? 64 : ((Cin + 127) / 128) * 128;
-  const long long total = (long long)Cin_pad * R * S * Cout_pad;
+  const int taps = sub ? 4 : R * S;
+  const int rows = pack_dgrad_rows(it);
+  const int co_tiles = (Cout_pad + PACK_TILE - 1) / PACK_TILE;
+  const long long tiles = pack_dgrad_tiles(rows, taps, Cout_pad);
   const float* __restrict__ w = it.w_ohwi;
   uint16_t* __restrict__ out = (uint16_t*)it.w_packed;
-  for (long long i = blockIdx.x * (long long)blockDim.x + threadIdx.x; i < total;
-       i += (long long)gridDim.x * blockDim.x) {
-    const int co = (int)(i % Cout_pad);
-    long long t = i / Cout_pad;
-    const int s = (int)(t % S);
-    t /= S;
-    const int r = (int)(t % R);
-    const int ci = (int)(t / R);
-    float v = 0.0f;
-    if (ci < Cin && co < Cout) v = w[(((long long)co * R + (R - 1 - r)) * S + (S - 1 - s)) * Cin + ci];
-    out[i] = rn_f32_to_bf16(v);
+  const int lane = threadIdx.x & (PACK_TILE - 1), sub_row = threadIdx.x / PACK_TILE;
+  for (long long t = blockIdx.x; t < tiles; t += gridDim.x) {
+    const int co0 = (int)(t % co_tiles) * PACK_TILE;
+    const long long t2 = t / co_tiles;
+    const int tap = (int)(t2 % taps);
+    const int row0 = (int)(t2 / taps) * PACK_TILE;
+    const int row = row0 + lane;
+#pragma unroll 4
+    for (int j = sub_row; j < PACK_TILE; j += 256 / PACK_TILE) {
+      const int co = co0 + j;
+      float v;
+      if (sub) {
+        v = dgrad_s2_weight(w, Cin, Cout, row, tap >> 1, tap & 1, co);
+      } else {
+        const int r = tap / S, s = tap - r * S;
+        v = (row < Cin && co < Cout) ? w[(((long long)co * R + (R - 1 - r)) * S + (S - 1 - s)) * Cin + row] : 0.0f;
+      }
+      tile[j][lane] = v;
+    }
+    __syncthreads();
+    const int co = co0 + lane;
+    if (co < Cout_pad) {
+#pragma unroll 4
+      for (int j = sub_row; j < PACK_TILE; j += 256 / PACK_TILE)
+        out[((long long)(row0 + j) * taps + tap) * Cout_pad + co] = rn_f32_to_bf16(tile[lane][j]);
+    }
+    __syncthreads();
   }
 }
 extern "C" int rn_pack_conv_weight_dgrad_batch(const rn_dgrad_pack* items, int n, void* stream) {
@@ -363,11 +377,11 @@
       RN_CHECK_ARG(it.pad_ == 0 || (it.pad_ == 1 && it.R == 3 && it.S == 3),
                    "rn_pack_conv_weight_dgrad_batch: item %d: the sub-pixel form is for 3x3 kernels", base + i);
       a.item[i] = it;
-      const long long total = it.pad_ == 1 ? (long long)rn_conv_cout_pad(4 * it.Cin) * 4 * it.Cout_pad
-                                           : (long long)rn_conv_cout_pad(it.Cin) * it.R * it.S * it.Cout_pad;
-      if (total > most) most = total;
-    }
-    const int bx = (int)(rn_cdiv(most, 256) < 256 ? rn_cdiv(most, 256) : 256);
+      const long long tiles = it.pad_ == 1 ? pack_dgrad_tiles(rn_conv_cout_pad(4 * it.Cin), 4, it.Cout_pad)
+                                           : pack_dgrad_tiles(rn_conv_cout_pad(it.Cin), it.R * it.S, it.Cout_pad);
+      if (tiles > most) most = tiles;
+    }
+    const int bx = (int)(most < 256 ? most : 256);
     hipLaunchKernelGGL(pack_dgrad_batch_kernel, dim3(bx, a.n), dim3(256), 0, (hipStream_t)stream, a);
     RN_CHECK_LAUNCH();
   }
diff --git a/retinanet-tensorflow2.x_amd/csrc/rn_train.hip b/retinanet-tensorflow2.x_amd/csrc/rn_train.hip
--- a/retinanet-tensorflow2.x_amd/csrc/rn_train.hip
+++ b/retinanet-tensorflow2.x_amd/csrc/rn_train.hip
@@ -1,4 +1,5 @@
 #include "rn_common.h"
+#include <vector>
 
 #define TR_THREADS 256
 
@@ -232,16 +233,16 @@
 }
 
 template <int CH>
-__global__ void __launch_bounds__(1024) bn_colreduce_final_kernel(const BnArgs a) {
+__device__ __forceinline__ void bn_colreduce_final_body(const BnArgs& a, const int bx, const int seg) {
   constexpr int LANES = 1024 / CH, PER = LANES / 16;
-  const BnSegDev& s = a.seg[blockIdx.y];
+  const BnSegDev& s = a.seg[seg];
   __shared__ double red[2][LANES][CH + 1];
   __shared__ double red2[2][16][CH + 1];
   const int cl = threadIdx.x & (CH - 1), lane = threadIdx.x / CH;
-  const int c = blockIdx.x * CH + cl;
+  const int c = bx * CH + cl;
   double t0 = 0.0, t1 = 0.0;
   if (c < s.C) {
-    const float* p = a.ws + a.ws_off[blockIdx.y];
+    const float* p = a.ws + a.ws_off[seg];
 #pragma unroll 8
     for (int k = lane; k < s.chunks; k += LANES) {
       t0 += (double)p[((long long)k * 2 + 0) * s.C + c];
@@ -262,7 +263,7 @@
   __syncthreads();
   if (threadIdx.x < 2 * CH) {
     const int which = threadIdx.x / CH, ch = threadIdx.x - which * CH;
-    const int cc = blockIdx.x * CH + ch;
+    const int cc = bx * CH + ch;
     if (cc < s.C) {
       double t = 0.0;
 #pragma unroll
@@ -281,21 +282,25 @@
     if (threadIdx.x < CH && c < s.C) bn_finalize_channel(a, s, c, red2[0][0][cl], red2[1][0][cl]);
   }
 }
+template <int CH>
+__global__ void __launch_bounds__(1024) bn_colreduce_final_kernel(const BnArgs a) {
+  bn_colreduce_final_body<CH>(a, blockIdx.x, blockIdx.y);
+}
 
 typedef unsigned bn_u32x2_t __attribute__((ext_vector_type(2)));
-__global__ void __launch_bounds__(1024) bn_colreduce_final_split_kernel(const BnArgs a) {
-  const BnSegDev& s = a.seg[blockIdx.y];
-  const int ks = a.ks[blockIdx.y], part = blockIdx.z;
-  if (part >= ks || (int)blockIdx.x * 16 >= s.C) return;
+__device__ __forceinline__ void bn_colreduce_final_split_body(const BnArgs& a, const int bx, const int seg, const int part) {
+  const BnSegDev& s = a.seg[seg];
+  const int ks = a.ks[seg];
+  if (part >= ks || bx * 16 >= s.C) return;
   __shared__ double red[16][2][16];
   __shared__ unsigned s_old;
   const int col = threadIdx.x & 3, lane = threadIdx.x >> 2, wave = threadIdx.x >> 6;
-  const int c = blockIdx.x * 16 + col * 4;
+  const int c = bx * 16 + col * 4;
   double t[8];
 #pragma unroll
   for (int q = 0; q < 8; ++q) t[q] = 0.0;
   if (c < s.C) {
-    const float* p = a.ws + a.ws_off[blockIdx.y] + c;
+    const float* p = a.ws + a.ws_off[seg] + c;
     const int per = (s.chunks + ks - 1) / ks;
     const int k1 = (part + 1) * per < s.chunks ? (part + 1) * per : s.chunks;
 #pragma unroll 2
@@ -322,7 +327,7 @@
     for (int j = 0; j < 16; ++j) r += red[j][which][ch];
   }
   if (ks > 1) {
-    char* const slots = (char*)a.ws + a.slot_off[blockIdx.y] + (size_t)blockIdx.x * ks * 256;
+    char* const slots = (char*)a.ws + a.slot_off[seg] + (size_t)bx * ks * 256;
     if (threadIdx.x < 64) {
       if (threadIdx.x < 32) {
         const __amdgpu_buffer_rsrc_t rs = __builtin_amdgcn_make_buffer_rsrc((void*)(slots + part * 256), 0, 256, 0x00020000);
@@ -331,7 +336,7 @@
       }
       asm volatile("s_waitcnt vmcnt(0)" ::: "memory");
       if (threadIdx.x == 0) {
-        unsigned* const cnt = (unsigned*)((char*)a.ws + a.cnt_off[blockIdx.y]) + blockIdx.x;
+        unsigned* const cnt = (unsigned*)((char*)a.ws + a.cnt_off[seg]) + bx;
         const unsigned old = __hip_atomic_fetch_add(cnt, 1u, __ATOMIC_RELAXED, __HIP_MEMORY_SCOPE_AGENT);
         if (old == (unsigned)(ks - 1)) __hip_atomic_store(cnt, 0u, __ATOMIC_RELAXED, __HIP_MEMORY_SCOPE_AGENT);
         s_old = old;
@@ -351,7 +356,7 @@
     }
   }
   if (threadIdx.x < 32) {
-    const int cc = blockIdx.x * 16 + ch;
+    const int cc = bx * 16 + ch;
     if (cc < s.C) {
       float* out = a.mode == 0 ? s.sums : s.bsums;
       out[which * s.C + cc] = (float)r;
@@ -364,9 +369,12 @@
   }
   if (a.fuse_finalize) {
     __syncthreads();
-    const int cc = blockIdx.x * 16 + threadIdx.x;
+    const int cc = bx * 16 + threadIdx.x;
     if (threadIdx.x < 16 && cc < s.C) bn_finalize_channel(a, s, cc, red[0][0][threadIdx.x], red[0][1][threadIdx.x]);
   }
+}
+__global__ void __launch_bounds__(1024) bn_colreduce_final_split_kernel(const BnArgs a) {
+  bn_colreduce_final_split_body(a, blockIdx.x, blockIdx.y, blockIdx.z);
 }
 
 __global__ void bn_finalize_kernel(const BnArgs a) {
@@ -622,6 +630,11 @@
   return (size_t)a.ws_off[segment] * sizeof(float);
 }
 
+static bool bn_final_is_split(const BnArgs& a, int max_ks) {
+  static const int final_form = getenv("RNET_BN_FINAL") ? atoi(getenv("RNET_BN_FINAL")) : 0;
+  return max_ks > 1 && final_form != 1 && (((uintptr_t)a.ws) & 15) == 0;
+}
+
 static int bn_colreduce(const rn_bn_problem* p, int mode, void* ws, size_t ws_bytes, hipStream_t st,
                         const char* fn, int fuse_finalize = 0) {
   BnArgs a;
@@ -672,8 +685,7 @@
   }
   int max_ks = 1;
   for (int i = 0; i < a.nseg; ++i) max_ks = a.ks[i] > max_ks ? a.ks[i] : max_ks;
-  static const int final_form = getenv("RNET_BN_FINAL") ? atoi(getenv("RNET_BN_FINAL")) : 0;
-  if (max_ks > 1 && final_form != 1 && (((uintptr_t)a.ws) & 15) == 0)
+  if (bn_final_is_split(a, max_ks))
     hipLaunchKernelGGL(bn_colreduce_final_split_kernel, dim3((max_c + 15) / 16, a.nseg, max_ks), dim3(1024), 0, st, a);
   else
     hipLaunchKernelGGL(bn_colreduce_final_kernel<16>, dim3((max_c + 15) / 16, a.nseg), dim3(1024), 0, st, a);
@@ -827,18 +839,111 @@
   return RN_OK;
 }
 
-__global__ void __launch_bounds__(TR_THREADS)
-reduce_rows_kernel(const float* __restrict__ src, int rows, long long row_stride, int n, float add, float* __restrict__ dst) {
-  const int c = blockIdx.x * blockDim.x + threadIdx.x;
+__device__ __forceinline__ void reduce_rows_body(const float* __restrict__ src, int rows, long long row_stride, int n,
+                                                 float add, float* __restrict__ dst, const int bx) {
+  const int c = bx * blockDim.x + threadIdx.x;
   if (c >= n) return;
   float s = 0.0f;
   for (int r = 0; r < rows; ++r) s += src[r * row_stride + c];
   dst[c] = s + add;
 }
+__global__ void __launch_bounds__(TR_THREADS)
+reduce_rows_kernel(const float* __restrict__ src, int rows, long long row_stride, int n, float add, float* __restrict__ dst) {
+  reduce_rows_body(src, rows, row_stride, n, add, dst, blockIdx.x);
+}
 extern "C" int rn_reduce_rows_f32(const float* src, int rows, int64_t row_stride, int n, float add, float* dst, void* stream) {
   RN_CHECK_ARG(src && dst && rows > 0 && n > 0 && row_stride >= 0, "rn_reduce_rows_f32: bad argument");
   hipLaunchKernelGGL(reduce_rows_kernel, dim3((n + TR_THREADS - 1) / TR_THREADS), dim3(TR_THREADS), 0, (hipStream_t)stream,
                      src, rows, (long long)row_stride, n, add, dst);
+  RN_CHECK_LAUNCH();
+  return RN_OK;
+}
+
+struct BiasBatchLayer {
+  BnArgs a;
+  int split;
+  const float* src;
+  long long row_stride;
+  int rows, n;
+  float* dst;
+};
+__global__ void __launch_bounds__(1024) bias_grad_stage2_batch_kernel(const BiasBatchLayer* __restrict__ layers, int parts) {
+  const int layer = blockIdx.z / parts, part = blockIdx.z - layer * parts;
+  const BiasBatchLayer& L = layers[layer];
+  const int seg = blockIdx.y;
+  if (seg >= L.a.nseg) return;
+  if (L.split) {
+    bn_colreduce_final_split_body(L.a, blockIdx.x, seg, part);
+  } else {
+    if (part > 0 || (int)blockIdx.x * 16 >= L.a.seg[seg].C) return;
+    bn_colreduce_final_body<16>(L.a, blockIdx.x, seg);
+  }
+}
+__global__ void __launch_bounds__(TR_THREADS) bias_grad_levels_batch_kernel(const BiasBatchLayer* __restrict__ layers) {
+  const BiasBatchLayer& L = layers[blockIdx.y];
+  reduce_rows_body(L.src, L.rows, L.row_stride, L.n, 0.0f, L.dst, blockIdx.x);
+}
+
+extern "C" size_t rn_bias_grad_batch_bytes(int n) { return n > 0 ? (size_t)n * sizeof(BiasBatchLayer) : 0; }
+
+extern "C" int rn_bias_grad_batch_init(const rn_bn_problem* const* problems, void* const* ws, const size_t* ws_bytes,
+                                       float* const* db, const int* db_cols, int n, void* dev_args, size_t dev_bytes,
+                                       rn_bias_batch* out) {
+  RN_CHECK_ARG(problems && ws && ws_bytes && db && db_cols && out && n > 0 && n <= 4096,
+               "rn_bias_grad_batch_init: bad argument");
+  if (!dev_args || dev_bytes < rn_bias_grad_batch_bytes(n)) {
+    rn_set_error("rn_bias_grad_batch_init: argument buffer too small (%zu < %zu)", dev_bytes, rn_bias_grad_batch_bytes(n));
+    return RN_ENOMEM;
+  }
+  std::vector<BiasBatchLayer> host((size_t)n);
+  rn_bias_batch b = {dev_args, n, 1, 1, 1, 1};
+  for (int l = 0; l < n; ++l) {
+    BiasBatchLayer& L = host[(size_t)l];
+    const rn_bn_problem* p = problems[l];
+    RN_CHECK_ARG(p && bn_fill(p, L.a, 1, 0) == 0, "rn_bias_grad_batch_init: layer %d: bad problem (C %% 8 == 0, 1..10 segments)", l);
+    if (!ws[l] || ws_bytes[l] < rn_bn_workspace_bytes(p)) {
+      rn_set_error("rn_bias_grad_batch_init: layer %d: workspace too small", l);
+      return RN_ENOMEM;
+    }
+    L.a.mode = 0;
+    L.a.fuse_finalize = 0;
+    L.a.ws = (float*)ws[l];
+    int max_ks = 1;
+    for (int i = 0; i < L.a.nseg; ++i) {
+      const BnSegDev& s = L.a.seg[i];
+      RN_CHECK_ARG(p->seg[i].ext_chunks > 0, "rn_bias_grad_batch_init: layer %d: stage 1 must be external (ext_chunks)", l);
+      RN_CHECK_ARG(s.sums, "rn_bias_grad_batch_init: layer %d: null tensor", l);
+      RN_CHECK_ARG(s.C == L.a.seg[0].C && s.sums - L.a.seg[0].sums == (long long)i * (L.a.seg[1 % L.a.nseg].sums - L.a.seg[0].sums),
+                   "rn_bias_grad_batch_init: layer %d: the segments' sums must be rows of one array", l);
+      if (L.a.ks[i] > max_ks) max_ks = L.a.ks[i];
+      if ((s.C + 15) / 16 > b.cblocks) b.cblocks = (s.C + 15) / 16;
+    }
+    L.split = bn_final_is_split(L.a, max_ks) ? 1 : 0;
+    if (L.split && max_ks > b.parts) b.parts = max_ks;
+    if (L.a.nseg > b.segs) b.segs = L.a.nseg;
+    RN_CHECK_ARG(db[l] && db_cols[l] > 0 && db_cols[l] <= L.a.seg[0].C, "rn_bias_grad_batch_init: layer %d: bad output", l);
+    L.src = L.a.seg[0].sums;
+    L.rows = L.a.nseg;
+    L.row_stride = L.a.nseg > 1 ? (long long)(L.a.seg[1].sums - L.a.seg[0].sums) : 0;
+    L.n = db_cols[l];
+    L.dst = db[l];
+    if (L.n > b.cols) b.cols = L.n;
+  }
+  RN_CHECK_ARG((long long)n * b.parts <= 65535, "rn_bias_grad_batch_init: too many layers");
+  RN_CHECK_HIP(hipMemcpy(dev_args, host.data(), (size_t)n * sizeof(BiasBatchLayer), hipMemcpyHostToDevice));
+  *out = b;
+  return RN_OK;
+}
+
+extern "C" int rn_bias_grad_batch(const rn_bias_batch* b, void* stream) {
+  RN_CHECK_ARG(b && b->dev_args && b->n > 0 && b->cblocks > 0 && b->segs > 0 && b->parts > 0 && b->cols > 0,
+               "rn_bias_grad_batch: bad argument (rn_bias_grad_batch_init fills it)");
+  const BiasBatchLayer* layers = (const BiasBatchLayer*)b->dev_args;
+  hipLaunchKernelGGL(bias_grad_stage2_batch_kernel, dim3(b->cblocks, b->segs, b->n * b->parts), dim3(1024), 0,
+                     (hipStream_t)stream, layers, b->parts);
+  RN_CHECK_LAUNCH();
+  hipLaunchKernelGGL(bias_grad_levels_batch_kernel, dim3((b->cols + TR_THREADS - 1) / TR_THREADS, b->n), dim3(TR_THREADS), 0,
+                     (hipStream_t)stream, layers);
   RN_CHECK_LAUNCH();
   return RN_OK;
 }
diff --git a/retinanet-tensorflow2.x_amd/retinanet/_C.py b/retinanet-tensorflow2.x_amd/retinanet/_C.py
--- a/retinanet-tensorflow2.x_amd/retinanet/_C.py
+++ b/retinanet-tensorflow2.x_amd/retinanet/_C.py
@@ -14,7 +14,8 @@
 RN_OK, RN_EINVAL, RN_ENOMEM, RN_EHIP, RN_ECOMM, RN_EUNSUPPORTED = 0, -1, -2, -3, -4, -5
 RN_ACT_NONE, RN_ACT_RELU, RN_ACT_RELU6, RN_ACT_SWISH = 0, 1, 2, 3
 RN_CONV_MAX_SEGMENTS = 10
-ABI_VERSION = 8
+RN_CONV_OUT_D2S = 1
+ABI_VERSION = 9
 PRED_W_TERMS = int(os.environ.get("RNET_PRED_W_TERMS", "2"))
 ACT_IDS = {None: RN_ACT_NONE, "none": RN_ACT_NONE, "relu": RN_ACT_RELU, "relu6": RN_ACT_RELU6,
            "swish": RN_ACT_SWISH}
@@ -64,7 +65,7 @@
                 ("residual", c_void_p), ("N", c_int32), ("H", c_int32), ("W", c_int32), ("Cin", c_int32),
                 ("pix_stride", c_int32), ("Ho", c_int32), ("Wo", c_int32), ("Cout", c_int32), ("bn_partial", c_void_p),
                 ("bias", c_void_p), ("w_terms", c_int32), ("w_pair", c_int32), ("bn_bwd_y", c_void_p),
-                ("bn_bwd_fwd", c_void_p)]
+                ("bn_bwd_fwd", c_void_p), ("out_mode", c_int32), ("pad_", c_int32)]
 
 
 class ConvProblem(Structure):
@@ -110,6 +111,11 @@
 class BnProblem(Structure):
     _fields_ = [("num_segments", c_int32), ("act", c_int32), ("bessel", c_int32), ("eps", c_float),
                 ("momentum", c_float), ("count_scale", c_float), ("seg", BnSegment * RN_CONV_MAX_SEGMENTS)]
+
+
+class BiasBatch(Structure):
+    _fields_ = [("dev_args", c_void_p), ("n", c_int32), ("cblocks", c_int32), ("segs", c_int32), ("parts", c_int32),
+                ("cols", c_int32)]
 
 
 _PP = POINTER(c_void_p)
@@ -147,6 +153,10 @@
                                  c_void_p, c_void_p, c_void_p, c_void_p, c_void_p, c_void_p, c_size_t, c_void_p]),
     "rn_rowmax_argmax": (c_int, [c_void_p, c_int64, c_int, c_void_p, c_void_p, c_void_p]),
     "rn_conv2d_nhwc_fwd": (c_int, [POINTER(ConvProblem), c_void_p]),
+    "rn_bias_grad_batch_bytes": (c_size_t, [c_int]),
+    "rn_bias_grad_batch_init": (c_int, [POINTER(POINTER(BnProblem)), _PP, POINTER(c_size_t), _PP, POINTER(c_int), c_int,
+                                        c_void_p, c_size_t, POINTER(BiasBatch)]),
+    "rn_bias_grad_batch": (c_int, [POINTER(BiasBatch), c_void_p]),
     "rn_conv_cout_pad": (c_int, [c_int]),
     "rn_conv_tile_rows": (c_int, [POINTER(ConvProblem)]),
     "rn_conv_bn_row_blocks": (c_int, [POINTER(ConvProblem), c_int]),
@@ -358,6 +368,18 @@
     return ctypes.cast(arr, _PP)
 
 
+def new_bias_grad_batch(library, problems, workspaces, outputs, cols):
+    import torch
+    n = len(problems)
+    args = torch.zeros((max(library.rn_bias_grad_batch_bytes(n), 256),), dtype=torch.uint8, device=workspaces[0].device)
+    probs = (POINTER(BnProblem) * n)(*[ctypes.pointer(p) for p in problems])
+    batch = BiasBatch()
+    check(library.rn_bias_grad_batch_init(probs, ptr_array(workspaces), (c_size_t * n)(*[w.numel() for w in workspaces]),
+                                          ptr_array(outputs), (c_int * n)(*[int(c) for c in cols]), n, ptr(args),
+                                          args.numel(), ctypes.byref(batch)), "rn_bias_grad_batch_init")
+    return batch, args
+
+
 def f32_array(values):
     if values is None:
         return None
diff --git a/retinanet-tensorflow2.x_amd/retinanet/model/train_engine.py b/retinanet-tensorflow2.x_amd/retinanet/model/train_engine.py
--- a/retinanet-tensorflow2.x_amd/retinanet/model/train_engine.py
+++ b/retinanet-tensorflow2.x_amd/retinanet/model/train_engine.py
@@ -53,6 +53,8 @@
         self.fuse_bn_bwd = env("RNET_FUSE_BN_BWD", "1") != "0"
         self.fuse_bn_bwd_groups = env("RNET_FUSE_BN_BWD", "1") == "2"
         self.side_stream_on = env("RNET_WGRAD_STREAM", "1") != "0"
+        self._bias_batch_on = env("RNET_BIAS_BATCH", "0") == "1"
+        self._fuse_d2s = env("RNET_FUSE_D2S", "0") == "1"
         cus = env("RNET_WGRAD_CUS", "160,208")
         self._wgrad_cap = tuple(int(v) for v in cus.split(",")) if cus not in ("0", "") else None
         if not self.side_stream_on:
@@ -158,6 +160,7 @@
             self._build_forward()
             self._build_backward()
             self._group_wgrad_steps()
+            self._batch_bias_grads()
             for name, cp in self.conv_launches:
                 marks = {bool(cp.seg[i].bn_bwd_y) for i in range(cp.num_segments)}
                 if name.startswith("dgrad:") and len(marks) != 1:
@@ -1041,6 +1044,24 @@
                 self.wgrad_groups.append(probs)
         self.bwd_steps = [replace.get(i, fn) for i, fn in enumerate(self.bwd_steps) if i not in drop]
 
+    def _batch_bias_grads(self):
+        self.bias_batch = None
+        idxs = [i for i, fn in enumerate(self.bwd_steps) if getattr(fn, "bias_item", None) is not None]
+        if not self._bias_batch_on or self.dp_active or len(idxs) < 2:
+            return
+        items = [self.bwd_steps[i].bias_item for i in idxs]
+        batch, args = _C.new_bias_grad_batch(self.lib, [it[0] for it in items], [it[1] for it in items],
+                                             [it[2] for it in items], [it[3] for it in items])
+        self._keep += [batch, args]
+        self.bias_batch = batch
+
+        def bias_grads(st, b=ctypes.byref(batch)):
+            _C.check(self.lib.rn_bias_grad_batch(b, st), "rn_bias_grad_batch")
+        last = idxs[-1]
+        self.bwd_steps[last] = self._side(bias_grads, writes=[w for i in idxs for w in self.bwd_steps[i].writes])
+        drop = set(idxs[:-1])
+        self.bwd_steps = [fn for i, fn in enumerate(self.bwd_steps) if i not in drop]
+
     def _bn_bwd_step(self, grp, ws, profiled=True):
         lib, pb, prb, bsums = self.lib, grp.problem, ctypes.byref(grp.problem), grp.bsums
         bracket = self._bn_pass if profiled else (lambda kind, pb, fn: fn())
@@ -1161,7 +1182,10 @@
                 def bias_grad(st, pr=ctypes.byref(pb2), ws2=ws2, bs=bs, db=db, n=c["cout"], rows=len(cops), stride=2 * cw):
                     _C.check(lib.rn_bn_stats(pr, _C.ptr(ws2), ws2.numel(), st), "bias colsum")
                     _C.check(lib.rn_reduce_rows_f32(_C.ptr(bs), rows, stride, n, 0.0, _C.ptr(db), st), "bias grad")
-                self.bwd_steps.append(self._side(bias_grad, writes=[cname + "/bias"]))
+                step = self._side(bias_grad, writes=[cname + "/bias"])
+                if fused_cs:
+                    step.bias_item = (pb2, ws2, db, c["cout"])
+                self.bwd_steps.append(step)
         packs = {}
         for sub in self._distinct_inputs([op for op in ops if self.requires.get(op["inp"])]):
             self._plan_dgrad_launch(sub, dy_of, mark, packs)
@@ -1344,6 +1368,12 @@
             by += 2 * B * Ho * Wo * c["cout"] + 2 * B * H * W * cin * (2 if res else 1) + 2 * k * k * cin * c["cout"]
         if post_op is None and stride == 1 and all(firsts):
             by += self._fuse_bn_bwd(p, need)
+        if subpixel and self._fuse_d2s and all(firsts) and all(p.seg[i].Cout % 256 == 0 for i in range(len(need))) \
+                and lib.rn_conv_kernel_id(ctypes.byref(p)) == 1:
+            for i in range(len(need)):
+                self._keep = [t for t in self._keep if not (torch.is_tensor(t) and t.data_ptr() == post[i][0])]
+                p.seg[i].y, p.seg[i].out_mode = post[i][1], _C.RN_CONV_OUT_D2S
+            post = []
         self._algo[id(p)] = (fl, by)
         self._keep.append(p)
         self.conv_launches.append(("dgrad:" + (need[0].get("group") or need[0]["out"]), p))
```

Measured after the change: 1116 images/s. About the same (-0.0%).
